# spiraldb/vortex

Hardware: AMD Instinct MI355X
Metric: decoded GB/s/GPU (device-resident) per encoding; % HBM roofline (higher is better)
Workload: dtype u32

## Files before the change

include/vortex_gpu.h:

```cpp
#ifndef VORTEX_GPU_H
#define VORTEX_GPU_H

#include <stddef.h>
#include <stdint.h>

#ifdef __cplusplus
extern "C" {
#endif

#define VXG_ABI_VERSION 9

typedef enum vxg_status {
    VXG_OK = 0,
    VXG_ERR_OUT_OF_BOUNDS = 1,
    VXG_ERR_COMPUTE = 2,
    VXG_ERR_INVALID_ARGUMENT = 3,
    VXG_ERR_INVALID_SERDE = 4,
    VXG_ERR_NOT_IMPLEMENTED = 5,
    VXG_ERR_MISMATCHED_TYPES = 6,
    VXG_ERR_ASSERTION_FAILED = 7,
    VXG_ERR_HIP = 8,
    VXG_ERR_OUT_OF_MEMORY = 9
} vxg_status;

enum {
    VXG_ENC_BOOL = 2, VXG_ENC_PRIMITIVE = 3, VXG_ENC_STRUCT = 4, VXG_ENC_VARBIN = 5,
    VXG_ENC_VARBINVIEW = 6, VXG_ENC_SPARSE = 8, VXG_ENC_CONSTANT = 9, VXG_ENC_CHUNKED = 10,
    VXG_ENC_ALP = 17, VXG_ENC_BYTE_BOOL = 18, VXG_ENC_DICT = 20, VXG_ENC_FL_BITPACKED = 21,
    VXG_ENC_FL_DELTA = 22, VXG_ENC_FL_FOR = 23, VXG_ENC_FSST = 24, VXG_ENC_ROARING_BOOL = 25, VXG_ENC_RUN_END = 27,
    VXG_ENC_RUN_END_BOOL = 28, VXG_ENC_ZIGZAG = 29, VXG_ENC_ALP_RD = 30
};

enum {
    VXG_U8 = 0, VXG_U16 = 1, VXG_U32 = 2, VXG_U64 = 3, VXG_I8 = 4, VXG_I16 = 5, VXG_I32 = 6,
    VXG_I64 = 7, VXG_F16 = 8, VXG_F32 = 9, VXG_F64 = 10
};

enum { VXG_DTYPE_NULL = 0, VXG_DTYPE_BOOL = 1, VXG_DTYPE_PRIMITIVE = 2, VXG_DTYPE_UTF8 = 3,
       VXG_DTYPE_BINARY = 4 };

enum { VXG_VALIDITY_NON_NULLABLE = 0, VXG_VALIDITY_ALL_VALID = 1, VXG_VALIDITY_ALL_INVALID = 2,
       VXG_VALIDITY_ARRAY = 3 };

typedef struct vxg_buffer {
    const void* ptr;
    uint64_t len;
} vxg_buffer;

typedef union vxg_meta {
    struct { uint8_t bit_width; uint8_t has_patches; uint16_t offset; } bitpacked;
    struct { uint64_t reference; uint8_t shift; } for_;
    struct { uint64_t deltas_len; uint16_t offset; } delta;
    struct { uint8_t e; uint8_t f; uint8_t has_patches; } alp;
    struct { uint8_t right_bit_width; uint8_t dict_len; uint8_t left_parts_ptype;
             uint8_t has_exceptions; uint16_t dict[8]; } alprd;
    struct { uint8_t codes_ptype; uint64_t values_len; } dict;
    struct { uint64_t symbols_len; uint8_t codes_nullable; uint8_t uncompressed_lengths_ptype; } fsst;
    struct { uint8_t ends_ptype; uint64_t num_runs; uint64_t offset; } runend;
    struct { uint64_t indices_offset; uint64_t indices_len; uint8_t fill_is_null; uint8_t fill[16]; } sparse;
    struct { uint8_t is_null; uint8_t scalar[16]; } constant;
    struct { uint64_t nchunks; } chunked;
    struct { uint8_t offsets_ptype; uint64_t bytes_len; } varbin;
    struct { uint8_t first_byte_bit_offset; } boolean;
    struct { uint8_t start; uint8_t ends_ptype; uint64_t num_runs; uint64_t offset; } runendbool;
    struct { uint32_t n_buffers; } varbinview;
    uint64_t raw[5];
} vxg_meta;

typedef struct vxg_array {
    uint16_t encoding;
    uint8_t dtype;
    uint8_t ptype;
    uint8_t nullable;
    uint8_t validity;
    uint16_t reserved;
    uint64_t len;
    vxg_meta meta;
    uint32_t n_buffers;
    uint32_t n_children;
    const vxg_buffer* buffers;
    const struct vxg_array* children;
} vxg_array;

typedef struct vxg_data_buffer {
    uint64_t offset;
    uint64_t len;
} vxg_data_buffer;

typedef struct vxg_canonical {
    uint16_t kind;
    uint8_t ptype;
    uint8_t dtype;
    uint32_t reserved;
    uint64_t len;
    void* values;
    uint64_t values_bytes;
    void* views;
    void* data;
    uint64_t data_bytes;
    void* validity;
    uint32_t n_data_buffers;
    uint32_t data_buffers_cap;
    vxg_data_buffer* data_buffers;
} vxg_canonical;

typedef struct vxg_ctx vxg_ctx;

int vxg_abi_version(void);
vxg_status vxg_open(int device, vxg_ctx** out);
vxg_status vxg_close(vxg_ctx* ctx);
const char* vxg_last_error(void);
vxg_status vxg_alloc(vxg_ctx* ctx, uint64_t bytes, void** dptr);
vxg_status vxg_free(vxg_ctx* ctx, void* dptr);
vxg_status vxg_host_alloc(vxg_ctx* ctx, uint64_t bytes, void** hptr);
vxg_status vxg_host_free(vxg_ctx* ctx, void* hptr);
vxg_status vxg_memcpy_h2d(vxg_ctx* ctx, void* dst, const void* src, uint64_t bytes, void* stream);
vxg_status vxg_memcpy_d2h(vxg_ctx* ctx, void* dst, const void* src, uint64_t bytes, void* stream);
vxg_status vxg_memcpy_d2d(vxg_ctx* ctx, void* dst, const void* src, uint64_t bytes, void* stream);
vxg_status vxg_stream_sync(vxg_ctx* ctx, void* stream);

typedef enum vxg_option {
    VXG_OPT_K1W_MIN_GROUPS = 1,
    VXG_OPT_K1W_BPW = 2,
    VXG_OPT_K1_WAVE = 3
} vxg_option;
vxg_status vxg_set_option(vxg_ctx* ctx, int option, int64_t value);
vxg_status vxg_get_option(vxg_ctx* ctx, int option, int64_t* value);

typedef struct vxg_launch_stats {
    uint64_t k1w_launches;
    uint64_t k1w_last_groups;
    uint32_t k1w_last_bpw;
    uint32_t k1w_last_bpw_max;
    uint32_t k1w_min_bpw;
    uint32_t k1w_max_bpw;
} vxg_launch_stats;
vxg_status vxg_get_launch_stats(vxg_ctx* ctx, vxg_launch_stats* out, int reset);

vxg_status vxg_canonical_size(vxg_ctx* ctx, const vxg_array* a, uint64_t* values_bytes,
                              uint64_t* data_bytes);
vxg_status vxg_canonicalize(vxg_ctx* ctx, const vxg_array* a, vxg_canonical* out, void* stream);

vxg_status vxg_canonical_layout(vxg_ctx* ctx, const vxg_array* a, uint64_t* values_bytes,
                                uint64_t* data_bytes, vxg_data_buffer* bufs, uint32_t cap,
                                uint32_t* n_bufs);

typedef struct vxg_plan vxg_plan;
enum { VXG_PLAN_MEASURE = 1 };
vxg_status vxg_plan_create(vxg_ctx* ctx, const vxg_array* arrays, vxg_canonical* outs, uint32_t n,
                           vxg_plan** plan);
vxg_status vxg_plan_create_ex(vxg_ctx* ctx, const vxg_array* arrays, vxg_canonical* outs, uint32_t n,
                              uint32_t flags, vxg_plan** plan);
vxg_status vxg_plan_launch(vxg_plan* plan, void* stream);
vxg_status vxg_plan_destroy(vxg_plan* plan);

typedef struct vxg_plan_info {
    uint32_t batched;
    uint32_t branches;
    uint32_t direct_nodes;
    uint32_t n_candidates;
    uint32_t candidate_batched[2];
    float candidate_ms[2];
    float create_ms;
    uint32_t selection;
    uint32_t candidate_cost[2];
    uint32_t reserved;
} vxg_plan_info;
vxg_status vxg_plan_get_info(const vxg_plan* plan, vxg_plan_info* info);

typedef enum vxg_plan_selection {
    VXG_PLAN_SEL_SINGLE = 0,
    VXG_PLAN_SEL_FASTER = 1,
    VXG_PLAN_SEL_TIE_COST = 2,
    VXG_PLAN_SEL_UNMEASURED = 3
} vxg_plan_selection;
uint32_t vxg_plan_select(const float* ms, const uint32_t* cost, uint32_t n, uint32_t* selection);


vxg_status vxg_bitunpack(vxg_ctx* ctx, int ptype, unsigned bit_width, unsigned offset,
                         uint64_t len, const void* packed, uint64_t packed_bytes, void* out,
                         void* stream);

vxg_status vxg_bitunpack_for(vxg_ctx* ctx, int ptype, unsigned bit_width, unsigned offset,
                             uint64_t len, const void* packed, uint64_t packed_bytes,
                             uint64_t reference, unsigned shift, int zigzag, void* out,
                             void* stream);

vxg_status vxg_bitunpack_alp(vxg_ctx* ctx, int float_ptype, unsigned bit_width, unsigned offset,
                             uint64_t len, const void* packed, uint64_t packed_bytes,
                             uint64_t for_reference, unsigned for_shift, unsigned e, unsigned f,
                             void* out, void* stream);

vxg_status vxg_bitunpack_dict(vxg_ctx* ctx, int codes_ptype, unsigned bit_width,
                              unsigned offset, uint64_t len, const void* packed,
                              uint64_t packed_bytes, const void* dict_values,
                              uint64_t dict_len, unsigned value_width, void* out, void* stream);

vxg_status vxg_patch(vxg_ctx* ctx, int ptype, void* out, uint64_t out_len, int indices_ptype,
                     const void* indices, uint64_t indices_offset, const void* values,
                     uint64_t n_patches, void* stream);

vxg_status vxg_for_decode(vxg_ctx* ctx, int ptype, const void* in, uint64_t n,
                          uint64_t reference, unsigned shift, void* out, void* stream);

vxg_status vxg_zigzag_decode(vxg_ctx* ctx, int out_ptype, const void* in, uint64_t n, void* out,
                             void* stream);

// ... 104 lines not shown
```

rust/vortex-gpu/src/ffi.rs:

```rust
#![allow(non_camel_case_types, non_upper_case_globals, dead_code)]

use std::os::raw::{c_char, c_int, c_uint, c_void};

pub const VXG_ABI_VERSION: c_int = 9;
pub type vxg_status = c_int;
pub const VXG_OK: vxg_status = 0;
pub const VXG_ERR_OUT_OF_BOUNDS: vxg_status = 1;
pub const VXG_ERR_COMPUTE: vxg_status = 2;
pub const VXG_ERR_INVALID_ARGUMENT: vxg_status = 3;
pub const VXG_ERR_INVALID_SERDE: vxg_status = 4;
pub const VXG_ERR_NOT_IMPLEMENTED: vxg_status = 5;
pub const VXG_ERR_MISMATCHED_TYPES: vxg_status = 6;
pub const VXG_ERR_ASSERTION_FAILED: vxg_status = 7;
pub const VXG_ERR_HIP: vxg_status = 8;
pub const VXG_ERR_OUT_OF_MEMORY: vxg_status = 9;
pub const VXG_ENC_BOOL: c_int = 2;
pub const VXG_ENC_PRIMITIVE: c_int = 3;
pub const VXG_ENC_STRUCT: c_int = 4;
pub const VXG_ENC_VARBIN: c_int = 5;
pub const VXG_ENC_VARBINVIEW: c_int = 6;
pub const VXG_ENC_SPARSE: c_int = 8;
pub const VXG_ENC_CONSTANT: c_int = 9;
pub const VXG_ENC_CHUNKED: c_int = 10;
pub const VXG_ENC_ALP: c_int = 17;
pub const VXG_ENC_BYTE_BOOL: c_int = 18;
pub const VXG_ENC_DICT: c_int = 20;
pub const VXG_ENC_FL_BITPACKED: c_int = 21;
pub const VXG_ENC_FL_DELTA: c_int = 22;
pub const VXG_ENC_FL_FOR: c_int = 23;
pub const VXG_ENC_FSST: c_int = 24;
pub const VXG_ENC_ROARING_BOOL: c_int = 25;
pub const VXG_ENC_RUN_END: c_int = 27;
pub const VXG_ENC_RUN_END_BOOL: c_int = 28;
pub const VXG_ENC_ZIGZAG: c_int = 29;
pub const VXG_ENC_ALP_RD: c_int = 30;
pub const VXG_U8: c_int = 0;
pub const VXG_U16: c_int = 1;
pub const VXG_U32: c_int = 2;
pub const VXG_U64: c_int = 3;
pub const VXG_I8: c_int = 4;
pub const VXG_I16: c_int = 5;
pub const VXG_I32: c_int = 6;
pub const VXG_I64: c_int = 7;
pub const VXG_F16: c_int = 8;
pub const VXG_F32: c_int = 9;
pub const VXG_F64: c_int = 10;
pub const VXG_DTYPE_NULL: c_int = 0;
pub const VXG_DTYPE_BOOL: c_int = 1;
pub const VXG_DTYPE_PRIMITIVE: c_int = 2;
pub const VXG_DTYPE_UTF8: c_int = 3;
pub const VXG_DTYPE_BINARY: c_int = 4;
pub const VXG_VALIDITY_NON_NULLABLE: c_int = 0;
pub const VXG_VALIDITY_ALL_VALID: c_int = 1;
pub const VXG_VALIDITY_ALL_INVALID: c_int = 2;
pub const VXG_VALIDITY_ARRAY: c_int = 3;

#[repr(C)]
#[derive(Copy, Clone, Debug)]
pub struct vxg_buffer {
    pub ptr: *const c_void,
    pub len: u64,
}

#[repr(C)]
#[derive(Copy, Clone, Debug)]
pub struct vxg_meta_bitpacked {
    pub bit_width: u8,
    pub has_patches: u8,
    pub offset: u16,
}

#[repr(C)]
#[derive(Copy, Clone, Debug)]
pub struct vxg_meta_for_ {
    pub reference: u64,
    pub shift: u8,
}

#[repr(C)]
#[derive(Copy, Clone, Debug)]
pub struct vxg_meta_delta {
    pub deltas_len: u64,
    pub offset: u16,
}

#[repr(C)]
#[derive(Copy, Clone, Debug)]
// ... 78 lines not shown
    pub ends_ptype: u8,
    pub num_runs: u64,
    pub offset: u64,
}

#[repr(C)]
#[derive(Copy, Clone, Debug)]
pub struct vxg_meta_varbinview {
    pub n_buffers: u32,
}

#[repr(C)]
#[derive(Copy, Clone)]
pub union vxg_meta {
    pub bitpacked: vxg_meta_bitpacked,
    pub for_: vxg_meta_for_,
    pub delta: vxg_meta_delta,
    pub alp: vxg_meta_alp,
    pub alprd: vxg_meta_alprd,
    pub dict: vxg_meta_dict,
    pub fsst: vxg_meta_fsst,
    pub runend: vxg_meta_runend,
    pub sparse: vxg_meta_sparse,
    pub constant: vxg_meta_constant,
    pub chunked: vxg_meta_chunked,
    pub varbin: vxg_meta_varbin,
    pub boolean: vxg_meta_boolean,
    pub runendbool: vxg_meta_runendbool,
    pub varbinview: vxg_meta_varbinview,
    pub raw: [u64; 5],
}

#[repr(C)]
#[derive(Copy, Clone, Debug)]
pub struct vxg_array {
    pub encoding: u16,
    pub dtype: u8,
    pub ptype: u8,
    pub nullable: u8,
    pub validity: u8,
    pub reserved: u16,
    pub len: u64,
    pub meta: vxg_meta,
    pub n_buffers: u32,
    pub n_children: u32,
    pub buffers: *const vxg_buffer,
    pub children: *const vxg_array,
}

#[repr(C)]
#[derive(Copy, Clone, Debug)]
pub struct vxg_data_buffer {
    pub offset: u64,
    pub len: u64,
}

#[repr(C)]
#[derive(Copy, Clone, Debug)]
pub struct vxg_canonical {
    pub kind: u16,
    pub ptype: u8,
    pub dtype: u8,
    pub reserved: u32,
    pub len: u64,
    pub values: *mut c_void,
    pub values_bytes: u64,
    pub views: *mut c_void,
    pub data: *mut c_void,
    pub data_bytes: u64,
    pub validity: *mut c_void,
    pub n_data_buffers: u32,
    pub data_buffers_cap: u32,
    pub data_buffers: *mut vxg_data_buffer,
}

#[repr(C)]
pub struct vxg_ctx {
    _private: [u8; 0],
}
pub type vxg_option = c_int;
pub const VXG_OPT_K1W_MIN_GROUPS: vxg_option = 1;
pub const VXG_OPT_K1W_BPW: vxg_option = 2;
pub const VXG_OPT_K1_WAVE: vxg_option = 3;

#[repr(C)]
#[derive(Copy, Clone, Debug)]
pub struct vxg_launch_stats {
    pub k1w_launches: u64,
    pub k1w_last_groups: u64,
    pub k1w_last_bpw: u32,
    pub k1w_last_bpw_max: u32,
    pub k1w_min_bpw: u32,
    pub k1w_max_bpw: u32,
}

#[repr(C)]
pub struct vxg_plan {
    _private: [u8; 0],
}
pub const VXG_PLAN_MEASURE: c_int = 1;

#[repr(C)]
#[derive(Copy, Clone, Debug)]
pub struct vxg_plan_info {
    pub batched: u32,
    pub branches: u32,
    pub direct_nodes: u32,
    pub n_candidates: u32,
    pub candidate_batched: [u32; 2],
    pub candidate_ms: [f32; 2],
    pub create_ms: f32,
    pub selection: u32,
    pub candidate_cost: [u32; 2],
    pub reserved: u32,
}
pub type vxg_plan_selection = c_int;
pub const VXG_PLAN_SEL_SINGLE: vxg_plan_selection = 0;
pub const VXG_PLAN_SEL_FASTER: vxg_plan_selection = 1;
pub const VXG_PLAN_SEL_TIE_COST: vxg_plan_selection = 2;
pub const VXG_PLAN_SEL_UNMEASURED: vxg_plan_selection = 3;
pub type vxg_cmp_op = c_int;
pub const VXG_CMP_EQ: vxg_cmp_op = 0;
pub const VXG_CMP_NOT_EQ: vxg_cmp_op = 1;
pub const VXG_CMP_GT: vxg_cmp_op = 2;
pub const VXG_CMP_GTE: vxg_cmp_op = 3;
pub const VXG_CMP_LT: vxg_cmp_op = 4;
pub const VXG_CMP_LTE: vxg_cmp_op = 5;
pub const VXG_CMP_NULL_AS_FALSE: c_int = 1;

#[repr(C)]
#[derive(Copy, Clone, Debug)]
pub struct vxg_compare_info {
    pub fused_launches: u32,
    pub fused_chunks: u32,
    pub fallback_arrays: u32,
    pub patch_launches: u32,
}

#[repr(C)]
#[derive(Copy, Clone, Debug)]
pub struct vxg_int_stats {
    pub n: u64,
    pub min_bits: u64,
    pub max_bits: u64,
    pub trailing_zeros: u32,
    pub reserved: u32,
    pub bit_width_freq: [u64; 65],
}

#[repr(C)]
#[derive(Copy, Clone, Debug)]
pub struct vxg_dict_chunk {
    pub packed: *const c_void,
    pub dict_values: *const c_void,
    pub out: *mut c_void,
    pub n_blocks: u64,
    pub len: u64,
    pub dict_len: u64,
}

#[repr(C)]
pub struct vxg_file {
    _private: [u8; 0],
}

#[repr(C)]
// ... 87 lines not shown
```

vortex_amd/_lib.py:

```python
from __future__ import annotations

import ctypes as C
import os
from pathlib import Path

_HERE = Path(__file__).resolve().parent
GPU_LIB_PATH = Path(os.environ["VXG_GPU_LIB"]) if os.environ.get("VXG_GPU_LIB") else _HERE / "libvortex_gpu.so"
ENC_LIB_PATH = _HERE / "libvortex_enc.so"

ENC = dict(BOOL=2, PRIMITIVE=3, STRUCT=4, VARBIN=5, VARBINVIEW=6, SPARSE=8, CONSTANT=9,
           CHUNKED=10, ALP=17, BYTE_BOOL=18, DICT=20, FL_BITPACKED=21, FL_DELTA=22, FL_FOR=23,
           FSST=24, ROARING_BOOL=25, RUN_END=27, RUN_END_BOOL=28, ZIGZAG=29, ALP_RD=30)
PTYPES = ["u8", "u16", "u32", "u64", "i8", "i16", "i32", "i64", "f16", "f32", "f64"]
PTYPE = {n: i for i, n in enumerate(PTYPES)}
DTYPE = dict(NULL=0, BOOL=1, PRIMITIVE=2, UTF8=3, BINARY=4)
VALIDITY = dict(NON_NULLABLE=0, ALL_VALID=1, ALL_INVALID=2, ARRAY=3)
ABI_VERSION = 9
STATUS = {0: "OK", 1: "OutOfBounds", 2: "ComputeError", 3: "InvalidArgument", 4: "InvalidSerde",
          5: "NotImplemented", 6: "MismatchedTypes", 7: "AssertionFailed", 8: "HipError",
          9: "OutOfMemory"}


class VortexGpuError(RuntimeError):

    def __init__(self, status: int, msg: str):
        super().__init__(f"{STATUS.get(status, status)}: {msg}")
        self.status = status
        self.kind = STATUS.get(status, str(status))


class VxgBuffer(C.Structure):
    _fields_ = [("ptr", C.c_void_p), ("len", C.c_uint64)]


class _MBitPacked(C.Structure):
    _fields_ = [("bit_width", C.c_uint8), ("has_patches", C.c_uint8), ("offset", C.c_uint16)]


class _MFoR(C.Structure):
    _fields_ = [("reference", C.c_uint64), ("shift", C.c_uint8)]


class _MDelta(C.Structure):
    _fields_ = [("deltas_len", C.c_uint64), ("offset", C.c_uint16)]


class _MAlp(C.Structure):
    _fields_ = [("e", C.c_uint8), ("f", C.c_uint8), ("has_patches", C.c_uint8)]


class _MAlpRd(C.Structure):
    _fields_ = [("right_bit_width", C.c_uint8), ("dict_len", C.c_uint8),
                ("left_parts_ptype", C.c_uint8), ("has_exceptions", C.c_uint8),
                ("dict", C.c_uint16 * 8)]


class _MDict(C.Structure):
    _fields_ = [("codes_ptype", C.c_uint8), ("values_len", C.c_uint64)]


class _MFsst(C.Structure):
    _fields_ = [("symbols_len", C.c_uint64), ("codes_nullable", C.c_uint8),
                ("uncompressed_lengths_ptype", C.c_uint8)]


class _MRunEnd(C.Structure):
    _fields_ = [("ends_ptype", C.c_uint8), ("num_runs", C.c_uint64), ("offset", C.c_uint64)]


class _MSparse(C.Structure):
    _fields_ = [("indices_offset", C.c_uint64), ("indices_len", C.c_uint64),
                ("fill_is_null", C.c_uint8), ("fill", C.c_uint8 * 16)]


class _MConstant(C.Structure):
    _fields_ = [("is_null", C.c_uint8), ("scalar", C.c_uint8 * 16)]


class _MChunked(C.Structure):
    _fields_ = [("nchunks", C.c_uint64)]


class _MVarBin(C.Structure):
    _fields_ = [("offsets_ptype", C.c_uint8), ("bytes_len", C.c_uint64)]


class _MBool(C.Structure):
    _fields_ = [("first_byte_bit_offset", C.c_uint8)]


class _MRunEndBool(C.Structure):
    _fields_ = [("start", C.c_uint8), ("ends_ptype", C.c_uint8), ("num_runs", C.c_uint64),
                ("offset", C.c_uint64)]


class _MVarBinView(C.Structure):
    _fields_ = [("n_buffers", C.c_uint32)]


class VxgMeta(C.Union):
    _fields_ = [("bitpacked", _MBitPacked), ("for_", _MFoR), ("delta", _MDelta), ("alp", _MAlp),
                ("alprd", _MAlpRd), ("dict", _MDict), ("fsst", _MFsst), ("runend", _MRunEnd),
                ("sparse", _MSparse), ("constant", _MConstant), ("chunked", _MChunked),
                ("varbin", _MVarBin), ("boolean", _MBool), ("runendbool", _MRunEndBool),
                ("varbinview", _MVarBinView), ("raw", C.c_uint64 * 5)]


class VxgArray(C.Structure):
    pass


VxgArray._fields_ = [("encoding", C.c_uint16), ("dtype", C.c_uint8), ("ptype", C.c_uint8),
                     ("nullable", C.c_uint8), ("validity", C.c_uint8), ("reserved", C.c_uint16),
                     ("len", C.c_uint64), ("meta", VxgMeta), ("n_buffers", C.c_uint32),
                     ("n_children", C.c_uint32), ("buffers", C.POINTER(VxgBuffer)),
                     ("children", C.POINTER(VxgArray))]


class VxgDataBuffer(C.Structure):
    _fields_ = [("offset", C.c_uint64), ("len", C.c_uint64)]


class VxgCanonical(C.Structure):
    _fields_ = [("kind", C.c_uint16), ("ptype", C.c_uint8), ("dtype", C.c_uint8),
                ("reserved", C.c_uint32), ("len", C.c_uint64), ("values", C.c_void_p),
                ("values_bytes", C.c_uint64), ("views", C.c_void_p), ("data", C.c_void_p),
                ("data_bytes", C.c_uint64), ("validity", C.c_void_p),
                ("n_data_buffers", C.c_uint32), ("data_buffers_cap", C.c_uint32),
                ("data_buffers", C.POINTER(VxgDataBuffer))]


PLAN_MEASURE = 1


class VxgPlanInfo(C.Structure):
    _fields_ = [("batched", C.c_uint32), ("branches", C.c_uint32), ("direct_nodes", C.c_uint32),
                ("n_candidates", C.c_uint32), ("candidate_batched", C.c_uint32 * 2),
                ("candidate_ms", C.c_float * 2), ("create_ms", C.c_float), ("selection", C.c_uint32),
                ("candidate_cost", C.c_uint32 * 2), ("reserved", C.c_uint32)]


PLAN_SELECTION = {0: "single", 1: "faster", 2: "tie_fewer_nodes", 3: "unmeasured"}


OPT_K1W_MIN_GROUPS, OPT_K1W_BPW, OPT_K1_WAVE = 1, 2, 3


class VxgLaunchStats(C.Structure):
    _fields_ = [("k1w_launches", C.c_uint64), ("k1w_last_groups", C.c_uint64), ("k1w_last_bpw", C.c_uint32),
                ("k1w_last_bpw_max", C.c_uint32), ("k1w_min_bpw", C.c_uint32), ("k1w_max_bpw", C.c_uint32)]


CMP_OP = {"==": 0, "!=": 1, ">": 2, ">=": 3, "<": 4, "<=": 5}
CMP_NULL_AS_FALSE = 1


class VxgCompareInfo(C.Structure):
    _fields_ = [("fused_launches", C.c_uint32), ("fused_chunks", C.c_uint32), ("fallback_arrays", C.c_uint32),
                ("patch_launches", C.c_uint32)]


class VxgIntStats(C.Structure):
    _fields_ = [("n", C.c_uint64), ("min_bits", C.c_uint64), ("max_bits", C.c_uint64), ("trailing_zeros", C.c_uint32),
                ("reserved", C.c_uint32), ("bit_width_freq", C.c_uint64 * 65)]


class VxgDictChunk(C.Structure):
    _fields_ = [("packed", C.c_void_p), ("dict_values", C.c_void_p), ("out", C.c_void_p),
                ("n_blocks", C.c_uint64), ("len", C.c_uint64), ("dict_len", C.c_uint64)]


assert C.sizeof(VxgMeta) == 40, C.sizeof(VxgMeta)
assert C.sizeof(VxgArray) == 80, C.sizeof(VxgArray)

VP, U64, U32, INT, UINT = C.c_void_p, C.c_uint64, C.c_uint32, C.c_int, C.c_uint
ST = C.c_int

GPU_SIGNATURES = {
    "vxg_abi_version": (C.c_int, []),
    "vxg_open": (ST, [INT, C.POINTER(VP)]),
    "vxg_close": (ST, [VP]),
    "vxg_last_error": (C.c_char_p, []),
    "vxg_alloc": (ST, [VP, U64, C.POINTER(VP)]),
    "vxg_free": (ST, [VP, VP]),
    "vxg_host_alloc": (ST, [VP, U64, C.POINTER(VP)]),
    "vxg_host_free": (ST, [VP, VP]),
    "vxg_memcpy_h2d": (ST, [VP, VP, VP, U64, VP]),
    "vxg_memcpy_d2h": (ST, [VP, VP, VP, U64, VP]),
    "vxg_memcpy_d2d": (ST, [VP, VP, VP, U64, VP]),
    "vxg_stream_sync": (ST, [VP, VP]),
    "vxg_set_option": (ST, [VP, INT, C.c_int64]),
    "vxg_get_option": (ST, [VP, INT, C.POINTER(C.c_int64)]),
    "vxg_get_launch_stats": (ST, [VP, C.POINTER(VxgLaunchStats), INT]),
    "vxg_canonical_size": (ST, [VP, C.POINTER(VxgArray), C.POINTER(U64), C.POINTER(U64)]),
    "vxg_canonicalize": (ST, [VP, C.POINTER(VxgArray), C.POINTER(VxgCanonical), VP]),
    "vxg_plan_create": (ST, [VP, C.POINTER(VxgArray), C.POINTER(VxgCanonical), U32, C.POINTER(VP)]),
    "vxg_plan_create_ex": (ST, [VP, C.POINTER(VxgArray), C.POINTER(VxgCanonical), U32, U32, C.POINTER(VP)]),
    "vxg_plan_get_info": (ST, [VP, C.c_void_p]),
    "vxg_plan_select": (U32, [C.POINTER(C.c_float), C.POINTER(U32), U32, C.POINTER(U32)]),
    "vxg_plan_launch": (ST, [VP, VP]),
    "vxg_plan_destroy": (ST, [VP]),
    "vxg_canonical_layout": (ST, [VP, C.POINTER(VxgArray), C.POINTER(U64), C.POINTER(U64),
                                  C.POINTER(VxgDataBuffer), U32, C.POINTER(U32)]),
    "vxg_bitunpack": (ST, [VP, INT, UINT, UINT, U64, VP, U64, VP, VP]),
    "vxg_bitunpack_for": (ST, [VP, INT, UINT, UINT, U64, VP, U64, U64, UINT, INT, VP, VP]),
    "vxg_bitunpack_alp": (ST, [VP, INT, UINT, UINT, U64, VP, U64, U64, UINT, UINT, UINT, VP, VP]),
    "vxg_bitunpack_dict": (ST, [VP, INT, UINT, UINT, U64, VP, U64, VP, U64, UINT, VP, VP]),
    "vxg_bitunpack_dict_chunks": (ST, [VP, INT, UINT, UINT, C.POINTER(VxgDictChunk), U32, VP]),
    "vxg_patch": (ST, [VP, INT, VP, U64, INT, VP, U64, VP, U64, VP]),
    "vxg_for_decode": (ST, [VP, INT, VP, U64, U64, UINT, VP, VP]),
    "vxg_zigzag_decode": (ST, [VP, INT, VP, U64, VP, VP]),
    "vxg_alp_decode": (ST, [VP, INT, VP, U64, UINT, UINT, VP, VP]),
    "vxg_alprd_decode": (ST, [VP, INT, VP, VP, UINT, UINT, VP, U64, VP, VP, U64, VP, VP]),
    "vxg_take": (ST, [VP, UINT, VP, U64, INT, VP, U64, VP, VP]),
    "vxg_delta_decode": (ST, [VP, INT, VP, U64, VP, U64, U64, U64, VP, VP]),
    "vxg_runend_decode": (ST, [VP, UINT, VP, INT, VP, U64, U64, U64, VP, VP]),
    "vxg_runend_bool_decode": (ST, [VP, INT, VP, U64, U64, INT, U64, VP, U64, VP]),
    "vxg_bytebool_to_bits": (ST, [VP, VP, U64, VP, U64, VP]),
    "vxg_take_array": (ST, [VP, VP, INT, VP, U64, VP, VP]),
    "vxg_filter_array": (ST, [VP, VP, VP, VP, VP]),
    "vxg_compare_scalar": (ST, [VP, VP, INT, VP, U32, VP, C.POINTER(VxgCompareInfo), VP]),
    "vxg_fsst_scratch_bytes": (U64, [U64]),
    "vxg_fsst_decode": (ST, [VP, VP, VP, UINT, VP, INT, VP, INT, VP, U64, VP, VP, VP, VP, VP]),
    "vxg_fill": (ST, [VP, UINT, VP, U64, VP, VP]),
    "vxg_compute_int_stats": (ST, [VP, INT, VP, U64, C.POINTER(VxgIntStats), VP]),
    "vxg_bitpack": (ST, [VP, INT, UINT, VP, U64, VP, U64, VP]),
    "vxg_for_encode": (ST, [VP, INT, VP, U64, U64, UINT, VP, VP]),
    "vxg_for_bitpack": (ST, [VP, INT, U64, UINT, UINT, VP, U64, VP, U64, VP]),
# ... 89 lines not shown
```

vortex_amd/arrays.py:

```python
from __future__ import annotations

import ctypes as C
from dataclasses import dataclass, field
from typing import Any, Optional, Sequence

import numpy as np

from . import _lib
from ._lib import DTYPE, ENC, PTYPE, PTYPES, VALIDITY, VortexGpuError

NP_OF_PTYPE = {"u8": np.uint8, "u16": np.uint16, "u32": np.uint32, "u64": np.uint64,
               "i8": np.int8, "i16": np.int16, "i32": np.int32, "i64": np.int64,
               "f16": np.float16, "f32": np.float32, "f64": np.float64}
PTYPE_OF_NP = {np.dtype(v): k for k, v in NP_OF_PTYPE.items()}


def ptype_width(p: str) -> int:
    return np.dtype(NP_OF_PTYPE[p]).itemsize


def unsigned_of(p: str) -> str:
    return "u" + p[1:] if p[0] == "i" else p


# ... 351 lines not shown
        m.sparse.indices_len = md["indices_len"]
        m.sparse.fill_is_null = int(md["fill_is_null"])
        for i, b in enumerate(md["fill"][:16]):
            m.sparse.fill[i] = b
    elif e == ENC["CONSTANT"]:
        m.constant.is_null = int(md["is_null"])
        for i, b in enumerate(md["scalar"][:16]):
            m.constant.scalar[i] = b
    elif e == ENC["CHUNKED"]:
        m.chunked.nchunks = md["nchunks"]
    elif e == ENC["VARBIN"]:
        m.varbin.offsets_ptype, m.varbin.bytes_len = md["offsets_ptype"], md["bytes_len"]
    elif e == ENC["BOOL"]:
        m.boolean.first_byte_bit_offset = md.get("first_byte_bit_offset", 0)
    elif e == ENC["RUN_END_BOOL"]:
        m.runendbool.start, m.runendbool.ends_ptype = int(md["start"]), md["ends_ptype"]
        m.runendbool.num_runs, m.runendbool.offset = md["num_runs"], md["offset"]
    elif e == ENC["VARBINVIEW"]:
        m.varbinview.n_buffers = md["n_buffers"]


def _buf_ptr(b) -> tuple[int, int]:
    import torch
    if not isinstance(b, torch.Tensor) or not b.is_cuda:
        raise VortexError(3, "array buffers must be device tensors: call Array.to(device) first")
    return b.data_ptr(), b.numel() * b.element_size()


def flatten(a: Array, keep: list) -> _lib.VxgArray:
    node = _lib.VxgArray()
    node.encoding = a.encoding
    node.dtype = a.dtype
    node.ptype = PTYPE[a.ptype]
    node.nullable = int(a.nullable)
    node.validity = a.validity
    node.len = a.len
    _fill_meta(node.meta, a)
    if a.buffers:
        bufs = (_lib.VxgBuffer * len(a.buffers))()
        for i, b in enumerate(a.buffers):
            bufs[i].ptr, bufs[i].len = _buf_ptr(b)
            keep.append(b)
        keep.append(bufs)
        node.buffers = C.cast(bufs, C.POINTER(_lib.VxgBuffer))
        node.n_buffers = len(a.buffers)
    if a.children:
        kids = (_lib.VxgArray * len(a.children))()
        for i, c in enumerate(a.children):
            kids[i] = flatten(c, keep)
        keep.append(kids)
        node.children = C.cast(kids, C.POINTER(_lib.VxgArray))
        node.n_children = len(a.children)
    return node


class Context:

    def __init__(self, device: int = 0):
        self.lib = _lib.gpu_lib()
        self.device = device
        h = C.c_void_p()
        _lib.check(self.lib.vxg_open(device, C.byref(h)))
        self.handle = h

    def close(self):
        if self.handle:
            self.lib.vxg_close(self.handle)
            self.handle = None

    def __del__(self):
        try:
            self.close()
        except Exception:
            pass

    def stream_ptr(self):
        import torch
        return C.c_void_p(torch.cuda.current_stream(self.device).cuda_stream)

    def sync(self):
        _lib.check(self.lib.vxg_stream_sync(self.handle, self.stream_ptr()))

    _OPTIONS = {"k1w_min_groups": _lib.OPT_K1W_MIN_GROUPS, "k1w_bpw": _lib.OPT_K1W_BPW,
                "k1_wave": _lib.OPT_K1_WAVE}

    def set_option(self, name: str, value: int):
        _lib.check(self.lib.vxg_set_option(self.handle, self._OPTIONS[name], int(value)))

    def get_option(self, name: str) -> int:
        v = C.c_int64()
        _lib.check(self.lib.vxg_get_option(self.handle, self._OPTIONS[name], C.byref(v)))
        return v.value

    def launch_stats(self, reset: bool = False) -> dict:
        st = _lib.VxgLaunchStats()
        _lib.check(self.lib.vxg_get_launch_stats(self.handle, C.byref(st), int(reset)))
        return {f: getattr(st, f) for f, _ in st._fields_}


@dataclass
class Canonical:
    kind: str
    len: int
    ptype: str
    values: Any = None
    views: Any = None
    data: Any = None
    validity: Any = None
    data_buffers: Any = None
    binary: bool = False
    info: Any = None

    def to_arrow(self):
        import pyarrow as pa
        validity = None if self.validity is None else pa.py_buffer(self.validity.cpu().numpy()[: (self.len + 7) // 8].copy())
        nulls = -1 if validity is not None else 0
        if self.kind == "primitive":
            t = {"u8": pa.uint8(), "u16": pa.uint16(), "u32": pa.uint32(), "u64": pa.uint64(), "i8": pa.int8(),
                 "i16": pa.int16(), "i32": pa.int32(), "i64": pa.int64(), "f16": pa.float16(), "f32": pa.float32(),
                 "f64": pa.float64()}[self.ptype]
            return pa.Array.from_buffers(t, self.len, [validity, pa.py_buffer(self.values.cpu().numpy().copy())],
                                         null_count=nulls)
        if self.kind == "bool":
            bits = self.values.cpu().numpy()[: (self.len + 7) // 8].copy()
            return pa.Array.from_buffers(pa.bool_(), self.len, [validity, pa.py_buffer(bits)], null_count=nulls)
        data = self.data.cpu().numpy()
        bufs = [pa.py_buffer(data[o: o + n].copy()) for o, n in self.data_buffers]
        views = pa.py_buffer(self.views.cpu().numpy()[: 16 * self.len].copy())
        return pa.Array.from_buffers(pa.binary_view() if self.binary else pa.string_view(), self.len,
                                     [validity, views] + bufs, null_count=nulls)

    def numpy(self):
        if self.kind == "primitive":
            return self.values.cpu().numpy().view(NP_OF_PTYPE[self.ptype])
        if self.kind == "bool":
            return np.unpackbits(self.values.cpu().numpy(), bitorder="little")[: self.len].astype(bool)
        return self.views.cpu().numpy().reshape(-1, 16), self.data.cpu().numpy()

    def buffers(self):
        d = self.data.cpu().numpy()
        return [d[o: o + n] for o, n in self.data_buffers]

    def validity_mask(self):
        if self.validity is None:
            return None
        bits = self.validity.cpu().numpy()
        return np.unpackbits(bits, bitorder="little")[: self.len].astype(bool)


def _kind(a: Array) -> str:
    return {DTYPE["PRIMITIVE"]: "primitive", DTYPE["BOOL"]: "bool"}.get(a.dtype, "varbinview")


def canonicalize(a: Array, ctx: Context, out_values=None, sync: bool = True) -> Canonical:
    import torch
    keep: list = []
    node = flatten(a, keep)
    dev = torch.device("cuda", ctx.device)
    vb, db, nb = C.c_uint64(), C.c_uint64(), C.c_uint32()
    cap = 256
    while True:
        table = (_lib.VxgDataBuffer * cap)()
        st = ctx.lib.vxg_canonical_layout(ctx.handle, C.byref(node), C.byref(vb), C.byref(db), table, cap,
                                          C.byref(nb))
        if st == 3 and cap < (1 << 24):
            cap *= 16
            continue
# ... 245 lines not shown
```

vortex_amd/csrc/capi.hip:

```cpp
#include <hip/hip_runtime.h>

#include <algorithm>
#include <memory>
#include <chrono>
#include <cstdio>
#include <cstdlib>
#include <cstring>
#include <mutex>
#include <string>
#include <tuple>
#include <vector>

#include "compare.hpp"
#include "encode_gpu.hpp"
#include "filter.hpp"
#include "k1g.hpp"
#include "take.hpp"
#include "vxg_internal.hpp"

struct vxg_ctx {
    vxg::Ctx c;
};

static_assert(sizeof(vxg::ChunkTable) <= 4096, "ChunkTable exceeds the kernarg limit");
static_assert(sizeof(vxg::FsstTable) <= 4096, "FsstTable exceeds the kernarg limit");
static_assert(sizeof(vxg::RunEndTable) <= 4096, "RunEndTable exceeds the kernarg limit");
static_assert(sizeof(vxg::VarBinTable) <= 4096, "VarBinTable exceeds the kernarg limit");
static_assert(sizeof(vxg::CmpTable) + 32 <= 4096, "CmpTable and the compare arguments exceed the kernarg limit");

namespace vxg {

const float kF10f[11] = {1.0f, 10.0f, 100.0f, 1000.0f, 10000.0f, 100000.0f, 1000000.0f,
                         10000000.0f, 100000000.0f, 1000000000.0f, 10000000000.0f};
const float kIF10f[11] = {1.0f, 0.1f, 0.01f, 0.001f, 0.0001f, 0.00001f, 0.000001f,
                          0.0000001f, 0.00000001f, 0.000000001f, 0.0000000001f};
const double kF10d[24] = {
    1.0, 10.0, 100.0, 1000.0, 10000.0, 100000.0, 1000000.0, 10000000.0, 100000000.0,
    1000000000.0, 10000000000.0, 100000000000.0, 1000000000000.0, 10000000000000.0,
    100000000000000.0, 1000000000000000.0, 10000000000000000.0, 100000000000000000.0,
    1000000000000000000.0, 10000000000000000000.0, 100000000000000000000.0,
    1000000000000000000000.0, 10000000000000000000000.0, 100000000000000000000000.0};
const double kIF10d[24] = {
    1.0, 0.1, 0.01, 0.001, 0.0001, 0.00001, 0.000001, 0.0000001, 0.00000001, 0.000000001,
    0.0000000001, 0.00000000001, 0.000000000001, 0.0000000000001, 0.00000000000001,
    0.000000000000001, 0.0000000000000001, 0.00000000000000001, 0.000000000000000001,
    0.0000000000000000001, 0.00000000000000000001, 0.000000000000000000001,
    0.0000000000000000000001, 0.00000000000000000000001};

static thread_local std::string g_last_error;

vxg_status set_error(vxg_status s, const std::string& msg) {
    if (s != VXG_OK) g_last_error = msg;
    return s;
}

vxg_status hip_check(hipError_t e, const char* what) {
    if (e == hipSuccess) return VXG_OK;
    return set_error(e == hipErrorOutOfMemory ? VXG_ERR_OUT_OF_MEMORY : VXG_ERR_HIP,
                     std::string(what) + ": " + hipGetErrorString(e));
}

static bool dict_rows_enabled() {
    static const bool on = [] {
        const char* e = std::getenv("VXG_DICT_ROWS");
        return !(e && e[0] == '0');
    }();
    return on;
}

static bool plan_vb_k1g() {
    const char* e = std::getenv("VXG_PLAN_VB_K1G");
    return !(e && e[0] == '0');
}

static bool fused_patches_enabled() {
    const char* e = std::getenv("VXG_FUSED_PATCHES");
    return !(e && e[0] == '0');
}

thread_local bool g_k1w_wrote_patches = false;
thread_local Ctx* g_cur_ctx = nullptr;

Options default_options() {
    static const Options d = [] {
        Options o;
        if (const char* e = std::getenv("VXG_K1W_MIN_GROUPS")) o.k1w_min_groups = int64_t(std::strtoll(e, nullptr, 10));
        return o;
    }();
    return d;
}

void note_k1w_launch(uint32_t bpw, uint32_t bpw_max, uint64_t groups) {
    if (!g_cur_ctx) return;
    std::lock_guard<std::mutex> lk(g_cur_ctx->mu);
    LaunchStats& st = g_cur_ctx->st;
    st.k1w_min_bpw = st.k1w_launches == 0 ? bpw : std::min(st.k1w_min_bpw, bpw);
    st.k1w_max_bpw = st.k1w_launches == 0 ? bpw : std::max(st.k1w_max_bpw, bpw);
    st.k1w_launches++;
    st.k1w_last_bpw = bpw;
    st.k1w_last_bpw_max = bpw_max;
    st.k1w_last_groups = groups;
}

bool k1_takes_wave(int T, int W, Epi epi, uint64_t groups32) {
    const int mode = k1_wave_mode();
    const bool split = (T == 32 || T == 64) && W > 0 && groups32 < split_below_groups();
    return groups32 > 0 && (mode == 2 || (mode == 1 && !split && epi != Epi::Dict));
}

vxg_status launch_fl_unpack(int T, int W, Epi epi, int vw, const ChunkTable& t, uint64_t g, hipStream_t s) {
    if (W < 0 || W > T) return set_error(VXG_ERR_INVALID_ARGUMENT, "bit width out of range");
    switch (epi) {
    case Epi::Plain:
    case Epi::For:
    case Epi::ForZigZag:
        switch (T) {
        case 8: return fl_plain_8(W, epi, t, g, s);
        case 16: return fl_plain_16(W, epi, t, g, s);
        case 32: return fl_plain_32(W, epi, t, g, s);
        case 64: return fl_plain_64(W, epi, t, g, s);
        }
        return set_error(VXG_ERR_INVALID_ARGUMENT, "bad FastLanes width");
    case Epi::AlpF32:
    case Epi::AlpF64:
        return fl_alp(T, W, epi, t, g, s);
    case Epi::Dict:
        if (W > kDictFusedMaxW) return VXG_ERR_NOT_IMPLEMENTED;
        if (vw == 16 && dict_rows_enabled()) return launch_dict_rows(T, W, vw, t, s);
        switch (vw) {
        case 1: return fl_dict_1(T, W, t, g, s);
        case 2: return fl_dict_2(T, W, t, g, s);
        case 4: return fl_dict_4(T, W, t, g, s);
        case 8: return fl_dict_8(T, W, t, g, s);
        case 16: return fl_dict_16(T, W, t, g, s);
        }
        return set_error(VXG_ERR_INVALID_ARGUMENT, "bad dictionary value width");
    }
    return VXG_ERR_INVALID_ARGUMENT;
}

}

using namespace vxg;

namespace {

#define VXG_TRY_S(expr)                       \
    do {                                      \
        vxg_status _s = (expr);               \
        if (_s != VXG_OK) return _s;          \
    } while (0)

struct K1Job {
    int T, W;
    Epi epi;
    int vw;
    ChunkDev d;
    bool vb = false;
    VarBinChunk vbc{};
};

bool same_kernel(const K1Job& a, const K1Job& b) {
    return a.T == b.T && a.W == b.W && a.epi == b.epi && a.vw == b.vw && a.vb == b.vb;
}

static uint64_t k1g_max_bytes() {
    static const uint64_t v = [] {
        const char* e = std::getenv("VXG_K1G_MAX_BYTES");
        return e ? uint64_t(std::strtoull(e, nullptr, 10)) : uint64_t(20) << 20;
    }();
    return v;
}

static int k1_out_width(const K1Job& j) {
    return j.epi == Epi::Dict ? j.vw : (j.epi == Epi::AlpF32 ? 4 : (j.epi == Epi::AlpF64 ? 8 : j.T / 8));
}

vxg_status launch_k1_jobs(std::vector<K1Job>& jobs, uint32_t* err, hipStream_t s, DevTables* dt = nullptr,
                          bool generic_small = false,
                          const std::vector<std::pair<int, RunEndChunk>>* gen_runs = nullptr,
                          const PatchCol* patch = nullptr, const FsstFused* fuse = nullptr) {
    std::stable_sort(jobs.begin(), jobs.end(), [](const K1Job& a, const K1Job& b) {
        return std::make_tuple(a.T, a.W, int(a.epi), a.vw, a.vb) < std::make_tuple(b.T, b.W, int(b.epi), b.vw, b.vb);
    });
    std::vector<const K1Job*> gen;
    const char* kf = std::getenv("VXG_PLAN_K1G_FIRST");
    const bool k1g_first = generic_small && dt && kf && kf[0] == '1';
    std::vector<std::pair<size_t, size_t>> deferred;
    auto launch_group = [&](size_t i, size_t j) -> vxg_status {
        size_t live = 0;
        for (size_t k = i; k < j; k++) live += jobs[k].d.n_blocks != 0;
        ChunkTable tab{};
        tab.err = err;
        if (patch && jobs.size() == 1) tab.patch = *patch;
        ChunkDev* cs = tab.c;
        if (live > size_t(kArgChunks)) {
            if (live > 0xFFFFFFFFull) return set_error(VXG_ERR_INVALID_ARGUMENT, "too many chunks");
            VXG_TRY_S(dt->table(live, &tab.host, &tab.ext));
            cs = tab.host;
        }
        uint64_t groups = 0;
        for (size_t k = i; k < j; k++) {
            if (jobs[k].d.n_blocks == 0) continue;
            ChunkDev& c = cs[tab.n++];
            c = jobs[k].d;
            c.first_group = groups;
            groups += (c.n_blocks + 31) / 32;
        }
        if (groups > 0xFFFFFFFFull) return set_error(VXG_ERR_INVALID_ARGUMENT, "array too long for one launch");
        if (tab.n) return launch_fl_unpack(jobs[i].T, jobs[i].W, jobs[i].epi, jobs[i].vw, tab, groups, s);
        return VXG_OK;
    };
    size_t i = 0;
    while (i < jobs.size()) {
        size_t j = i, live = 0;
        uint64_t out_bytes = 0;
        while (j < jobs.size() && (dt || j - i < size_t(kArgChunks)) && same_kernel(jobs[i], jobs[j])) {
            live += jobs[j].d.n_blocks != 0;
            out_bytes += jobs[j].d.len * uint64_t(k1_out_width(jobs[j]));
            j++;
        }
        if (jobs[i].vb || (dt && generic_small && out_bytes < k1g_max_bytes() &&
                           gen_kind(jobs[i].T, int(jobs[i].epi), jobs[i].vw) >= 0)) {
            if (!dt) return set_error(VXG_ERR_INVALID_ARGUMENT, "VarBin-dictionary K1 jobs need a plan");
            for (size_t k = i; k < j; k++)
                if (jobs[k].d.n_blocks) gen.push_back(&jobs[k]);
            i = j;
            continue;
        }
        (void)live;
        if (k1g_first) deferred.emplace_back(i, j);
        else VXG_TRY_S(launch_group(i, j));
        i = j;
    }
    const size_t n_runs = gen_runs ? gen_runs->size() : 0;
    if (!gen.empty() || n_runs || (fuse && fuse->valid)) {
        if (!dt) return set_error(VXG_ERR_INVALID_ARGUMENT, "internal: K1g launch outside a plan");
        if (gen.size() + n_runs > 0xFFFFFFFFull) return set_error(VXG_ERR_INVALID_ARGUMENT, "too many chunks");
        GenChunk* host;
        const GenChunk* ext;
        VXG_TRY_S(dt->table(gen.size() + n_runs, &host, &ext));
        uint64_t groups = 0;
        bool dict_lds = true;
        uint32_t packed_bytes = 0, dict_bytes = 0, runs_bytes = 0;
        const bool vb_alone = n_runs == 0 && !(fuse && fuse->valid) &&
                              std::all_of(gen.begin(), gen.end(), [](const K1Job* jp) { return jp->vb; });
        uint64_t gen_blocks = 0;
        for (const K1Job* jp : gen) gen_blocks += jp->d.n_blocks;
        const uint32_t bpw_cap = gen_bpw_cap(gen_blocks);
        for (size_t k = 0; k < gen.size(); k++) {
            const K1Job& jb = *gen[k];
            GenChunk& g = host[k];
            g.d = jb.d;
            g.kind = uint32_t(gen_kind(jb.T, int(jb.epi), jb.vw, jb.vb));
            g.W = uint32_t(jb.W);
            g.bpw = jb.vb ? gen_vb_bpw(jb.T, jb.W, vb_alone, bpw_cap) : gen_bpw(jb.T, jb.W, bpw_cap);
            g.d.first_group = groups;
            groups += (jb.d.n_blocks + g.bpw - 1) / g.bpw;
            packed_bytes = std::max(packed_bytes, g.bpw * 128u * uint32_t(jb.W));
            if (jb.vb) {
                dict_bytes = std::max(dict_bytes, gen_vb_stage_bytes(jb.d.dict_len, jb.vbc.bytes));
                g.vb_src = jb.vbc.src;
                g.vb_offs = jb.vbc.offsets;
                g.vb_offs_width = jb.vbc.offs_width;
                g.vb_dst = jb.vbc.dst;
                g.vb_bytes = jb.vbc.bytes;
                g.vb_bidx = jb.vbc.bidx;
            } else if (jb.epi == Epi::Dict) {
                dict_lds = dict_lds && jb.d.dict_len * uint64_t(jb.vw) <= uint64_t(kDictLdsBytes) &&
                           (reinterpret_cast<uintptr_t>(jb.d.dict) & 15) == 0;
            }
        }
        if (dict_lds)
            for (const K1Job* jp : gen)
                if (jp->epi == Epi::Dict && !jp->vb)
                    dict_bytes = std::max(dict_bytes, uint32_t((jp->d.dict_len * uint64_t(jp->vw) + 15) & ~15ull));
        for (size_t k = 0; k < n_runs; k++) {
            const auto& [w, r] = (*gen_runs)[k];
            GenChunk& g = host[gen.size() + k];
            g.kind = uint32_t(gen_runs_kind(w));
            g.re = r;
            g.d.first_group = groups;
            g.d.n_blocks = r.n_runs;
            groups += (r.n_runs + kRunEndRunsPerGroup - 1) / kRunEndRunsPerGroup;
            runs_bytes = std::max(runs_bytes, gen_runs_lds_bytes(w));
        }
        std::vector<uint64_t> cnt(gen.size() + n_runs);
        for (size_t k = 0; k < cnt.size(); k++)
            cnt[k] = (k + 1 < cnt.size() ? host[k + 1].d.first_group : groups) - host[k].d.first_group;
        uint64_t gpe = common_groups(cnt.data(), cnt.size());
        const char* pe = std::getenv("VXG_K1G_PAD");
        if (!gpe && cnt.size() > 1 && !(pe && pe[0] == '0')) {
            const uint64_t m = *std::max_element(cnt.begin(), cnt.end());
            if (m * cnt.size() - groups <= groups / 10) {
                for (size_t k = 0; k < cnt.size(); k++) host[k].d.first_group = k * m;
                groups = m * cnt.size();
                gpe = m;
            }
        }
        VXG_TRY_S(launch_k1_generic(ext, uint32_t(gen.size() + n_runs), groups, dict_lds, packed_bytes, dict_bytes,
                                    runs_bytes, err, s, gpe, fuse));
    }
    for (const auto& [a, b] : deferred) VXG_TRY_S(launch_group(a, b));
    return VXG_OK;
}

#define VXG_TRY(expr)                         \
    do {                                      \
        vxg_status _s = (expr);               \
        if (_s != VXG_OK) return _s;          \
    } while (0)

inline hipStream_t S(void* s) { return static_cast<hipStream_t>(s); }

vxg_status use_device(vxg_ctx* ctx) {
    if (!ctx) return set_error(VXG_ERR_INVALID_ARGUMENT, "null vxg_ctx");
    g_cur_ctx = &ctx->c;
    return hip_check(hipSetDevice(ctx->c.device), "hipSetDevice");
}

vxg_status make_k1_job(int T, unsigned W, unsigned offset, uint64_t len, const void* packed, uint64_t packed_bytes,
                       Epi epi, int vw, const UnpackArgs& a, void* out, K1Job& j) {
    if (offset > 1023) return set_error(VXG_ERR_INVALID_ARGUMENT, "Offset must be less than full block, i.e. 1024");
    if (W > unsigned(T)) return set_error(VXG_ERR_INVALID_ARGUMENT, "Unsupported bit width");
    const uint64_t nblk = (len + offset + 1023) / 1024;
    if (W > 0 && packed_bytes != nblk * 128ull * W)
        return set_error(VXG_ERR_INVALID_ARGUMENT, "Expected " + std::to_string(nblk * 128ull * W) +
                                                       " packed bytes, got " + std::to_string(packed_bytes));
    if (W > 0 && (reinterpret_cast<uintptr_t>(packed) & 15))
        return set_error(VXG_ERR_INVALID_ARGUMENT, "packed buffer must be 16-byte aligned");
    const int ow = epi == Epi::Dict ? vw : (epi == Epi::AlpF32 ? 4 : (epi == Epi::AlpF64 ? 8 : T / 8));
    if (reinterpret_cast<uintptr_t>(out) % uint64_t(ow))
        return set_error(VXG_ERR_INVALID_ARGUMENT, "output buffer must be aligned to the value width");
    if (epi == Epi::Dict && W > unsigned(kDictFusedMaxW)) return VXG_ERR_NOT_IMPLEMENTED;
    if (epi == Epi::Dict && a.dict_len == 0 && len > 0)
        return set_error(VXG_ERR_OUT_OF_BOUNDS, "take: index out of bounds");
    j.T = T;
    j.W = int(W);
    j.epi = epi;
    j.vw = epi == Epi::Dict ? vw : 0;
    j.d = ChunkDev{};
    j.d.packed = static_cast<const uint8_t*>(packed);
    j.d.out = out;
    j.d.n_blocks = len ? nblk : 0;
    j.d.len = len;
    j.d.reference = a.reference;
    j.d.alp_a = a.alp_a;
    j.d.alp_b = a.alp_b;
    j.d.dict = a.dict;
    j.d.dict_len = a.dict_len;
    j.d.offset = offset;
    j.d.shift = a.shift;
    return VXG_OK;
}

vxg_status bitunpack_common(vxg_ctx* ctx, int T, unsigned W, unsigned offset, uint64_t len,
                            const void* packed, uint64_t packed_bytes, Epi epi, int vw,
                            UnpackArgs a, void* out, void* stream) {
    std::vector<K1Job> jobs(1);
    VXG_TRY(make_k1_job(T, W, offset, len, packed, packed_bytes, epi, vw, a, out, jobs[0]));
    return launch_k1_jobs(jobs, ctx->c.err_word, S(stream));
}

vxg_status launch_runs(std::vector<RunEndChunk> runs, int w, uint32_t* err, hipStream_t s, DevTables* dt) {
    runs.erase(std::remove_if(runs.begin(), runs.end(), [](const RunEndChunk& r) { return r.len == 0; }), runs.end());
    std::vector<RunEndChunk> short_runs, long_runs;
    for (const RunEndChunk& r : runs) (r.len <= kRunEndShortRun * r.n_runs ? short_runs : long_runs).push_back(r);
    for (int pass = 0; pass < 2; pass++) {
        std::vector<RunEndChunk>& rs = pass == 0 ? short_runs : long_runs;
        const size_t per = dt && rs.size() > size_t(kRunEndArgChunks) ? rs.size() : size_t(kRunEndArgChunks);
        for (size_t i = 0; i < rs.size(); i += per) {
            RunEndTable tab{};
            tab.err = err;
            RunEndChunk* cs = tab.c;
            RunEndChunk* host = nullptr;
            if (per > size_t(kRunEndArgChunks)) {
                VXG_TRY_S(dt->table(rs.size(), &host, &tab.ext));
                cs = host;
            }
            uint64_t groups = 0;
            for (size_t k = i; k < rs.size() && k - i < per; k++) {
                RunEndChunk& r = cs[tab.n++];
                r = rs[k];
                r.first_group = groups;
                groups += pass == 0 ? (r.n_runs + kRunEndRunsPerGroup - 1) / kRunEndRunsPerGroup
                                    : (r.len + kRunEndSpan - 1) / kRunEndSpan;
            }
            VXG_TRY_S(pass == 0 ? launch_runend_runs(w, tab, groups, s) : launch_runend_chunks(w, tab, groups, s));
        }
    }
    return VXG_OK;
}

struct PlanBatch {
    struct Run {
        int w;
        RunEndChunk c;
        bool indep;
    };
    std::vector<VarBinChunk> dicts;
    std::vector<K1Job> jobs;
    std::vector<Run> runs;
    std::vector<FsstChunk> fssts;
    bool empty() const { return dicts.empty() && jobs.empty() && runs.empty() && fssts.empty(); }
};

static bool plan_fuse_enabled() {
    const char* e = std::getenv("VXG_PLAN_FUSE");
    return !(e && e[0] == '0');
}

vxg_status launch_varbin_dicts(const std::vector<VarBinChunk>& dicts, uint32_t* err, hipStream_t s, DevTables* dt) {
    const size_t per = dt && dicts.size() > size_t(kVarBinArgChunks) ? dicts.size() : size_t(kVarBinArgChunks);
    for (size_t i = 0; i < dicts.size(); i += per) {
        VarBinTable tab{};
        tab.err = err;
        VarBinChunk* cs = tab.c;
        if (per > size_t(kVarBinArgChunks)) {
            VarBinChunk* host;
            VXG_TRY_S(dt->table(dicts.size(), &host, &tab.ext));
            cs = host;
        }
        uint64_t groups = 0;
        for (size_t j = i; j < dicts.size() && j - i < per; j++) {
            VarBinChunk& d = cs[tab.n++];
            d = dicts[j];
            d.first_group = groups;
            groups += d.n ? (d.n + 255) / 256 : 1;
        }
        VXG_TRY_S(launch_varbin_chunks(tab, groups, s));
    }
    return VXG_OK;
}

vxg_status flush_plan_batch(PlanBatch& b, uint32_t* err, hipStream_t s, DevTables* dt) {
    FsstFused ff;
    if (!b.fssts.empty()) {
        void* scratch = nullptr;
        VXG_TRY_S(hip_check(hipMalloc(&scratch, (fsst_batch_scratch_bytes(b.fssts.data(), b.fssts.size()) + 15) & ~15ull),
                            "hipMalloc (plan FSST scratch)"));
        dt->allocs.push_back(scratch);
        VXG_TRY_S(launch_fsst_batch(b.fssts, scratch, err, s, dt, plan_fuse_enabled() ? &ff : nullptr));
    }
    VXG_TRY_S(launch_varbin_dicts(b.dicts, err, s, dt));
    std::vector<std::pair<int, RunEndChunk>> gen_runs;
    std::vector<PlanBatch::Run> rest;
    for (const PlanBatch::Run& r : b.runs) {
        if (r.c.len == 0) continue;
        if (r.indep && r.c.len <= kRunEndShortRun * r.c.n_runs && gen_runs_kind(r.w) >= 0) gen_runs.emplace_back(r.w, r.c);
        else rest.push_back(r);
    }
    VXG_TRY_S(launch_k1_jobs(b.jobs, err, s, dt, true, &gen_runs, nullptr, &ff));
    std::vector<int> widths;
    for (const auto& r : rest) widths.push_back(r.w);
    std::sort(widths.begin(), widths.end());
    widths.erase(std::unique(widths.begin(), widths.end()), widths.end());
    for (int w : widths) {
        std::vector<RunEndChunk> rs;
        for (const auto& r : rest)
            if (r.w == w) rs.push_back(r.c);
        VXG_TRY_S(launch_runs(rs, w, err, s, dt));
    }
    return VXG_OK;
}

class Planner {
  public:
    Planner(vxg_ctx* ctx, hipStream_t s, DevTables* plan = nullptr, PlanBatch* batch = nullptr)
        : ctx_(ctx), s_(s), plan_(plan), batch_(batch) {}
    ~Planner() {
        for (void* p : temps_) (void)hipFreeAsync(p, s_);
    }

    vxg_status canonical(const vxg_array& a, vxg_canonical& out);
    vxg_status take(const vxg_array& a, const void* idx, int iw, bool isg, uint64_t n, vxg_canonical& out);
    vxg_status filter(const vxg_array& a, const vxg_array& pred, vxg_canonical& out);
    vxg_status compare(const vxg_array& a, int op, uint64_t scalar_bits, uint32_t flags, vxg_canonical& out,
                       vxg_compare_info& info);
    vxg_status canonical_size(const vxg_array& a, uint64_t& vb, uint64_t& db);
    vxg_status string_layout(const vxg_array& a, std::vector<vxg_data_buffer>& bufs, uint64_t& extent);
    static vxg_status string_buffer_count(const vxg_array& a, uint32_t& n);

  private:
    vxg_ctx* ctx_;
    hipStream_t s_;
    std::vector<void*> temps_;
    DevTables* plan_ = nullptr;
    PlanBatch* batch_ = nullptr;
    const vxg_array* root_ = nullptr;
    bool defer(const vxg_array& a) const { return batch_ && &a == root_; }
    struct PatchJob {
        const vxg_array* sp;
        int T;
        Epi epi;
        int vw;
        UnpackArgs a;
        void* dst;
        uint64_t out_len;
    };
    std::vector<K1Job>* k1_batch_ = nullptr;
    std::vector<PatchJob>* patch_batch_ = nullptr;
    const PatchCol* fused_patch_ = nullptr;
    std::vector<FsstChunk>* fsst_batch_ = nullptr;
    bool k1_fusable(const vxg_array& c) const;

    vxg_status temp(uint64_t bytes, void** p) {
        if (bytes == 0) bytes = 16;
        if (plan_) {
            VXG_TRY(hip_check(hipMalloc(p, (bytes + 15) & ~15ull), "hipMalloc (plan temporary)"));
            plan_->allocs.push_back(*p);
            return VXG_OK;
        }
        VXG_TRY(hip_check(hipMallocAsync(p, (bytes + 15) & ~15ull, s_), "hipMallocAsync"));
        temps_.push_back(*p);
        return VXG_OK;
    }

    static bool is_primitive_dtype(const vxg_array& a) { return a.dtype == VXG_DTYPE_PRIMITIVE; }
    static int width(const vxg_array& a) { return ptype_width(a.ptype); }

    const vxg_buffer* buf(const vxg_array& a, uint32_t i) const {
        return i < a.n_buffers ? &a.buffers[i] : nullptr;
    }
    const vxg_array* child(const vxg_array& a, uint32_t i) const {
        return i < a.n_children ? &a.children[i] : nullptr;
    }

    vxg_status decode_into(const vxg_array& a, void* dst);
    vxg_status view_primitive(const vxg_array& a, const void** p);
    vxg_status int_column(const vxg_array& a, IntCol& c);
    vxg_status packed_column(const vxg_array& a, IntCol& c, bool* packed);
    vxg_status runend_column(const vxg_array& a, bool in_place, IntCol& c);

    vxg_status decode_bitpacked(const vxg_array& bp, Epi epi, int vw, UnpackArgs a, void* dst);
    bool patch_fusable(const vxg_array& sparse, int value_width) const;
    vxg_status sparse_patch_col(const vxg_array& sparse, PatchCol& pc);
    vxg_status apply_sparse_patches(const vxg_array& sparse, int T, Epi epi, int vw, const UnpackArgs& a,
                                    void* dst, uint64_t out_len);
    vxg_status decode_alp(const vxg_array& a, void* dst);
    vxg_status decode_dict_primitive(const vxg_array& a, void* dst);
    vxg_status decode_chunked_primitive(const vxg_array& a, void* dst);
    vxg_status decode_alprd(const vxg_array& a, void* dst);
    vxg_status decode_sparse_values(const vxg_array& a, void* dst);

    vxg_status take_values(const vxg_array& a, const void* idx, int iw, bool isg, uint64_t n, void* dst);
    vxg_status take_patches(const vxg_array& sp, TakePatches& p);
    struct CmpFused {
        const vxg_array* arr;
        const vxg_array* bp;
        const vxg_array* outer;
        int T, ck;
        Epi epi;
        EpiParams ep;
        CmpChunk d;
        bool excl;
    };
    vxg_status compare_shape(const vxg_array& a, uint64_t out_bit, CmpFused& f, bool* fused);
    vxg_status launch_compare_group(std::vector<CmpFused*>& group, void* out, uint64_t scalar_bits, int op);
    vxg_status validity_into(const vxg_array& a, void** bitmap);
    vxg_status bools_into(const vxg_array& a, void* bits, uint64_t off);
    vxg_status validity_source(const vxg_array& a, const vxg_array** node, int* kind);
    vxg_status string_canonical(const vxg_array& a, vxg_canonical& out);
    vxg_status string_lens(const vxg_array& a, std::vector<uint64_t>& lens,
                           std::vector<std::pair<size_t, const vxg_array*>>& fsst) const;
    vxg_status strings_into(const vxg_array& a, uint8_t* views, uint8_t* data, const vxg_data_buffer* bufs,
                            uint32_t bidx, const uint8_t* validity);
};

vxg_status Planner::view_primitive(const vxg_array& a, const void** p) {
    if (a.encoding == VXG_ENC_PRIMITIVE) {
// ... 31 lines not shown
vxg_status Planner::packed_column(const vxg_array& a, IntCol& c, bool* packed) {
    *packed = false;
    c = IntCol{};
    c.width = width(a);
    c.sgn = ptype_is_signed(a.ptype);
    const vxg_array* bp = nullptr;
    if (a.encoding == VXG_ENC_FL_FOR && child(a, 0) && child(a, 0)->encoding == VXG_ENC_FL_BITPACKED) {
        bp = child(a, 0);
        c.reference = a.meta.for_.reference;
        c.shift = a.meta.for_.shift;
    } else if (a.encoding == VXG_ENC_FL_BITPACKED) {
        bp = &a;
    }
    if (bp && !bp->meta.bitpacked.has_patches && width(*bp) == c.width && (c.width == 4 || c.width == 8) &&
        bp->len == a.len) {
        const vxg_buffer* pk = buf(*bp, 0);
        const unsigned W = bp->meta.bitpacked.bit_width, off = bp->meta.bitpacked.offset;
        const uint64_t nblk = (bp->len + off + 1023) / 1024;
        if (off > 1023) return set_error(VXG_ERR_INVALID_ARGUMENT, "Offset must be less than full block, i.e. 1024");
        if (W > unsigned(8 * c.width)) return set_error(VXG_ERR_INVALID_ARGUMENT, "Unsupported bit width");
        const uint64_t have = pk ? pk->len : 0;
        if (W > 0 && have != nblk * 128ull * W)
            return set_error(VXG_ERR_INVALID_ARGUMENT, "Expected " + std::to_string(nblk * 128ull * W) +
                                                           " packed bytes, got " + std::to_string(have));
        c.packed = true;
        c.p = pk ? pk->ptr : nullptr;
        c.W = W;
        c.offset = off;
        *packed = true;
    }
    return VXG_OK;
}

vxg_status Planner::apply_sparse_patches(const vxg_array& sp, int T, Epi epi, int vw, const UnpackArgs& a,
                                         void* dst, uint64_t out_len) {
    if (sp.encoding != VXG_ENC_SPARSE)
        return set_error(VXG_ERR_INVALID_ARGUMENT, "Can't patch with a non-Sparse array");
    const vxg_array* idx = child(sp, 0);
    const vxg_array* val = child(sp, 1);
    if (!idx || !val) return set_error(VXG_ERR_INVALID_ARGUMENT, "Sparse patches need indices and values");
    if (idx->len != val->len) return set_error(VXG_ERR_INVALID_ARGUMENT, "Sparse indices/values length mismatch");
    PatchCol pc;
    VXG_TRY(int_column(*idx, pc.idx));
    VXG_TRY(view_primitive(*val, &pc.vals));
    return launch_patch(vw, pc.idx, epi, T, dst, out_len, sp.meta.sparse.indices_offset, pc.vals, idx->len, a, s_);
}

bool Planner::patch_fusable(const vxg_array& sp, int value_width) const {
    const vxg_array* idx = child(sp, 0);
    const vxg_array* val = child(sp, 1);
    return sp.encoding == VXG_ENC_SPARSE && idx && val && idx->len == val->len && idx->len > 0 &&
           width(*val) == value_width && width(*idx) == 8 && ptype_is_int(idx->ptype);
}

vxg_status Planner::sparse_patch_col(const vxg_array& sp, PatchCol& pc) {
    const vxg_array* idx = child(sp, 0);
    VXG_TRY(int_column(*idx, pc.idx));
    VXG_TRY(view_primitive(*child(sp, 1), &pc.vals));
    pc.n = idx->len;
    pc.idx_off = sp.meta.sparse.indices_offset;
    return VXG_OK;
}

vxg_status Planner::decode_bitpacked(const vxg_array& bp, Epi epi, int vw, UnpackArgs a, void* dst) {
    const int T = 8 * width(bp);
    if (!ptype_is_int(bp.ptype)) return set_error(VXG_ERR_MISMATCHED_TYPES, "BitPacked needs an integer ptype");
    const vxg_buffer* packed = buf(bp, 0);
    const unsigned W = bp.meta.bitpacked.bit_width;
    a.err = ctx_->c.err_word;
    K1Job j;
    VXG_TRY(make_k1_job(T, W, bp.meta.bitpacked.offset, bp.len, packed ? packed->ptr : nullptr,
                        packed ? packed->len : 0, epi, vw, a, dst, j));
    const vxg_array* p = nullptr;
    if (bp.meta.bitpacked.has_patches) {
        p = child(bp, 0);
        if (!p) return set_error(VXG_ERR_INVALID_ARGUMENT, "BitPackedArray: patches child missing");
    }
    if (k1_batch_) {
        k1_batch_->push_back(j);
        if (p) patch_batch_->push_back(PatchJob{p, T, epi, vw, a, dst, bp.len});
        return VXG_OK;
    }
    std::vector<K1Job> one{j};
    VXG_TRY(launch_k1_jobs(one, ctx_->c.err_word, s_, plan_, false, nullptr, fused_patch_));
    if (p) VXG_TRY(apply_sparse_patches(*p, T, epi, vw, a, dst, bp.len));
    return VXG_OK;
}

vxg_status Planner::decode_alp(const vxg_array& a, void* dst) {
    const vxg_array* enc = child(a, 0);
    if (!enc) return set_error(VXG_ERR_INVALID_ARGUMENT, "ALPArray: encoded child missing");
    const bool f32 = a.ptype == VXG_F32;
    if (!f32 && a.ptype != VXG_F64) return set_error(VXG_ERR_MISMATCHED_TYPES, "ALP can only encode f32 and f64");
    const unsigned e = a.meta.alp.e, f = a.meta.alp.f;
    if ((f32 && (e > 10 || f > 10)) || (!f32 && (e > 23 || f > 23)))
        return set_error(VXG_ERR_INVALID_ARGUMENT, "ALP exponents out of range");
    UnpackArgs ua{};
    ua.alp_a = f32 ? double(kF10f[f]) : kF10d[f];
    ua.alp_b = f32 ? double(kIF10f[e]) : kIF10d[e];
    const Epi epi = f32 ? Epi::AlpF32 : Epi::AlpF64;
    const vxg_array* bp = nullptr;
    if (enc->encoding == VXG_ENC_FL_FOR && child(*enc, 0) &&
        child(*enc, 0)->encoding == VXG_ENC_FL_BITPACKED) {
        ua.reference = enc->meta.for_.reference;
        ua.shift = enc->meta.for_.shift;
        bp = child(*enc, 0);
    } else if (enc->encoding == VXG_ENC_FL_BITPACKED) {
        bp = enc;
    }
    bool fused = false;
    if (bp && width(*bp) == (f32 ? 4 : 8)) {
        PatchCol pc{};
        const vxg_array* p = a.meta.alp.has_patches ? child(a, 1) : nullptr;
        if (p && !k1_batch_ && !patch_batch_ && !bp->meta.bitpacked.has_patches && bp->len == a.len &&
            patch_fusable(*p, f32 ? 4 : 8) && fused_patches_enabled()) {
            const uint64_t nblk = (bp->len + bp->meta.bitpacked.offset + 1023) / 1024;
            if (k1_takes_wave(f32 ? 32 : 64, int(bp->meta.bitpacked.bit_width), epi, (nblk + 31) / 32)) {
                VXG_TRY(sparse_patch_col(*p, pc));
                fused = !pc.idx.packed || pc.idx.W > 0;
            }
        }
        fused_patch_ = fused ? &pc : nullptr;
        g_k1w_wrote_patches = false;
        const vxg_status st = decode_bitpacked(*bp, epi, 0, ua, dst);
        fused_patch_ = nullptr;
        VXG_TRY(st);
        fused = fused && g_k1w_wrote_patches;
    } else {
        const void* penc;
        VXG_TRY(view_primitive(*enc, &penc));
        VXG_TRY(launch_alp(a.ptype, penc, a.len, ua.alp_a, ua.alp_b, dst, s_));
    }
    if (a.meta.alp.has_patches && !fused) {
        const vxg_array* p = child(a, 1);
        if (!p) return set_error(VXG_ERR_INVALID_ARGUMENT, "ALPArray: patches child missing");
        UnpackArgs plain{};
        plain.err = ctx_->c.err_word;
        if (patch_batch_) {
            patch_batch_->push_back(PatchJob{p, f32 ? 32 : 64, Epi::Plain, 0, plain, dst, a.len});
            return VXG_OK;
        }
        VXG_TRY(apply_sparse_patches(*p, f32 ? 32 : 64, Epi::Plain, 0, plain, dst, a.len));
    }
    return VXG_OK;
}

vxg_status Planner::decode_dict_primitive(const vxg_array& a, void* dst) {
    const vxg_array* values = child(a, 0);
    const vxg_array* codes = child(a, 1);
    if (!values || !codes) return set_error(VXG_ERR_INVALID_ARGUMENT, "DictArray needs values and codes");
    if (!ptype_is_unsigned(codes->ptype) || codes->nullable)
        return set_error(VXG_ERR_MISMATCHED_TYPES, "Dict codes must be non-nullable unsigned int");
    const void* pv;
    VXG_TRY(view_primitive(*values, &pv));
    const int vw = width(*values);
    if (codes->encoding == VXG_ENC_FL_BITPACKED && codes->meta.bitpacked.bit_width <= kDictFusedMaxW) {
        UnpackArgs ua{};
        ua.dict = pv;
        ua.dict_len = values->len;
        return decode_bitpacked(*codes, Epi::Dict, vw, ua, dst);
    }
    const void* pc;
    VXG_TRY(view_primitive(*codes, &pc));
    return launch_take(vw, pv, values->len, width(*codes), false, pc, a.len, dst, ctx_->c.err_word, s_);
}

bool Planner::k1_fusable(const vxg_array& c) const {
// ... 42 lines not shown
    std::vector<uint8_t> is_inplace(2 * n, 0);
    uint64_t tmp_bytes = 0;
    for (uint64_t i = 0; i < n; i++) {
        const vxg_array& c = a.children[i + 1];
        if (!batch_runend(c)) continue;
        const vxg_array* e = child(c, 0);
        const vxg_array* v = child(c, 1);
        const bool short_runs = c.len <= kRunEndShortRun * e->len;
        const vxg_array* xs[2] = {e, v};
        for (int k = 0; k < 2; k++) {
            bool pk = false;
            if (short_runs && ptype_is_int(xs[k]->ptype)) VXG_TRY(packed_column(*xs[k], inplace[2 * i + k], &pk));
            is_inplace[2 * i + k] = pk;
            if (!pk && xs[k]->encoding != VXG_ENC_PRIMITIVE) tmp_bytes += (xs[k]->len * width(*xs[k]) + 15) & ~15ull;
        }
    }
    uint8_t* tmp = nullptr;
    if (tmp_bytes) {
        void* t;
        VXG_TRY(temp(tmp_bytes, &t));
        tmp = static_cast<uint8_t*>(t);
    }
    auto level0 = [&](const vxg_array& x, const void** p) -> vxg_status {
        if (x.encoding == VXG_ENC_PRIMITIVE) return view_primitive(x, p);
        *p = tmp;
        tmp += (x.len * width(x) + 15) & ~15ull;
        k1_batch_ = &jobs;
        patch_batch_ = &patches;
        const vxg_status st = decode_into(x, const_cast<void*>(*p));
        k1_batch_ = nullptr;
        patch_batch_ = nullptr;
        return st;
    };
    uint64_t off = 0;
    for (uint64_t i = 0; i < n; i++) {
        const vxg_array& c = a.children[i + 1];
        if (c.ptype != a.ptype || c.dtype != a.dtype)
            return set_error(VXG_ERR_MISMATCHED_TYPES, "Chunks must have the ChunkedArray's dtype");
        uint8_t* slice = static_cast<uint8_t*>(dst) + off * w;
        if (k1_fusable(c)) {
            k1_batch_ = &jobs;
            patch_batch_ = &patches;
            const vxg_status st = decode_into(c, slice);
            k1_batch_ = nullptr;
            patch_batch_ = nullptr;
            VXG_TRY(st);
        } else if (batch_runend(c)) {
            const vxg_array& e = *child(c, 0);
            const vxg_array& v = *child(c, 1);
            RunEndChunk r{};
            IntCol* cols[2] = {&r.ends, &r.values};
            const vxg_array* xs[2] = {&e, &v};
            for (int k = 0; k < 2; k++) {
                if (is_inplace[2 * i + k]) {
                    *cols[k] = inplace[2 * i + k];
                } else {
                    cols[k]->width = width(*xs[k]);
                    cols[k]->sgn = ptype_is_signed(xs[k]->ptype);
                    VXG_TRY(level0(*xs[k], &cols[k]->p));
                }
            }
            r.out = slice;
            r.n_runs = e.len;
            r.offset = c.meta.runend.offset;
            r.len = c.len;
            runs.push_back(r);
            runs_indep.push_back(uint8_t((is_inplace[2 * i] || e.encoding == VXG_ENC_PRIMITIVE) &&
                                         (is_inplace[2 * i + 1] || v.encoding == VXG_ENC_PRIMITIVE)));
        } else if ((reinterpret_cast<uintptr_t>(slice) & 15) == 0) {
            VXG_TRY(decode_into(c, slice));
        } else {
            const void* p;
            VXG_TRY(view_primitive(c, &p));
            VXG_TRY(launch_copy_bytes(slice, p, c.len * w, s_));
        }
        off += c.len;
    }
    if (off != a.len) return set_error(VXG_ERR_INVALID_ARGUMENT, "Chunked len != sum of chunk lens");
    if (defer(a) && patches.empty()) {
        batch_->jobs.insert(batch_->jobs.end(), jobs.begin(), jobs.end());
        for (size_t k = 0; k < runs.size(); k++) batch_->runs.push_back(PlanBatch::Run{w, runs[k], runs_indep[k] != 0});
        return VXG_OK;
    }
    VXG_TRY(launch_k1_jobs(jobs, ctx_->c.err_word, s_, plan_));
    for (const PatchJob& p : patches) VXG_TRY(apply_sparse_patches(*p.sp, p.T, p.epi, p.vw, p.a, p.dst, p.out_len));
    return launch_runs(runs, w, ctx_->c.err_word, s_, plan_);
}

vxg_status Planner::decode_alprd(const vxg_array& a, void* dst) {
    const vxg_array* left = child(a, 0);
    const vxg_array* right = child(a, 1);
    if (!left || !right) return set_error(VXG_ERR_INVALID_ARGUMENT, "ALPRDArray needs left/right parts");
    if (left->ptype != VXG_U16) return set_error(VXG_ERR_MISMATCHED_TYPES, "ALP-RD left parts must be u16");
    const void *pl, *pr;
    VXG_TRY(view_primitive(*left, &pl));
    VXG_TRY(view_primitive(*right, &pr));
    const void* pos = nullptr;
    const void* exc = nullptr;
    uint64_t n_exc = 0, pos_off = 0;
    int pw = 8;
    bool psg = false;
    if (a.meta.alprd.has_exceptions) {
        const vxg_array* sp = child(a, 2);
        if (!sp || sp->encoding != VXG_ENC_SPARSE)
            return set_error(VXG_ERR_INVALID_ARGUMENT, "left_parts_exceptions must be SparseArray encoded");
        const vxg_array* si = child(*sp, 0);
        const vxg_array* sv = child(*sp, 1);
        VXG_TRY(view_primitive(*si, &pos));
        VXG_TRY(view_primitive(*sv, &exc));
        n_exc = si->len;
        pos_off = sp->meta.sparse.indices_offset;
        pw = width(*si);
        psg = ptype_is_signed(si->ptype);
    }
    return launch_alprd(a.ptype, static_cast<const uint16_t*>(pl), a.meta.alprd.dict, a.meta.alprd.dict_len,
                        a.meta.alprd.right_bit_width, pr, a.len, pos, pw, psg, pos_off,
                        static_cast<const uint16_t*>(exc), n_exc, dst, ctx_->c.err_word, s_);
}

vxg_status Planner::decode_sparse_values(const vxg_array& a, void* dst) {
    uint8_t fill[16] = {0};
    if (!a.meta.sparse.fill_is_null) std::memcpy(fill, a.meta.sparse.fill, 16);
    VXG_TRY(launch_fill(width(a), fill, a.len, dst, s_));
    UnpackArgs plain{};
    plain.err = ctx_->c.err_word;
    return apply_sparse_patches(a, 8 * width(a), Epi::Plain, 0, plain, dst, a.len);
}

vxg_status Planner::decode_into(const vxg_array& a, void* dst) {
    if (!is_primitive_dtype(a)) return set_error(VXG_ERR_MISMATCHED_TYPES, "expected a primitive dtype");
    const int w = width(a);
    if (w == 0) return set_error(VXG_ERR_NOT_IMPLEMENTED, "unsupported ptype");
    switch (a.encoding) {
    case VXG_ENC_PRIMITIVE: {
        const void* p;
        VXG_TRY(view_primitive(a, &p));
        if (p != dst && a.len)
            VXG_TRY(launch_copy_bytes(dst, p, a.len * w, s_));
        return VXG_OK;
    }
    case VXG_ENC_FL_BITPACKED:
        return decode_bitpacked(a, Epi::Plain, 0, UnpackArgs{}, dst);
    case VXG_ENC_FL_FOR: {
        const vxg_array* enc = child(a, 0);
        if (!enc) return set_error(VXG_ERR_INVALID_ARGUMENT, "FoRArray is missing encoded child array");
        if (!ptype_is_int(a.ptype)) return set_error(VXG_ERR_MISMATCHED_TYPES, "FoR needs an integer ptype");
        if (enc->encoding == VXG_ENC_FL_BITPACKED && width(*enc) == w) {
            UnpackArgs ua{};
            ua.reference = a.meta.for_.reference;
            ua.shift = a.meta.for_.shift;
            return decode_bitpacked(*enc, Epi::For, 0, ua, dst);
        }
        VXG_TRY(decode_into(*enc, dst));
        return launch_for(w, dst, a.len, a.meta.for_.reference, a.meta.for_.shift, false, dst, s_);
    }
    case VXG_ENC_ZIGZAG: {
        const vxg_array* enc = child(a, 0);
        if (!enc) return set_error(VXG_ERR_INVALID_ARGUMENT, "ZigZagArray is missing encoded child");
        if (!ptype_is_signed(a.ptype)) return set_error(VXG_ERR_MISMATCHED_TYPES, "ZigZag decodes to signed ints");
        if (enc->encoding == VXG_ENC_FL_BITPACKED && width(*enc) == w)
            return decode_bitpacked(*enc, Epi::ForZigZag, 0, UnpackArgs{}, dst);
        VXG_TRY(decode_into(*enc, dst));
        return launch_zigzag(w, dst, a.len, dst, s_);
    }
    case VXG_ENC_ALP:
        return decode_alp(a, dst);
    case VXG_ENC_ALP_RD:
        return decode_alprd(a, dst);
    case VXG_ENC_DICT:
// ... 753 lines not shown
    if (!fsst.empty()) {
        void* d;
        VXG_TRY(temp(8 * fsst.size(), &d));
        for (size_t k = 0; k < fsst.size(); k++) {
            const vxg_array& ul = *child(*fsst[k].second, 3);
            const void* pul;
            VXG_TRY(view_primitive(ul, &pul));
            VXG_TRY(launch_sum(pul, width(ul), ptype_is_signed(ul.ptype), ul.len, static_cast<uint64_t*>(d) + k, s_));
        }
        std::vector<uint64_t> h(fsst.size());
        VXG_TRY(hip_check(hipMemcpyAsync(h.data(), d, 8 * h.size(), hipMemcpyDeviceToHost, s_), "sum readback"));
        VXG_TRY(hip_check(hipStreamSynchronize(s_), "sum sync"));
        for (size_t k = 0; k < fsst.size(); k++) lens[fsst[k].first] = h[k];
    }
    bufs.resize(lens.size());
    uint64_t off = 0;
    for (size_t b = 0; b < lens.size(); b++) {
        bufs[b] = vxg_data_buffer{off, lens[b]};
        off = (off + lens[b] + 15) & ~15ull;
    }
    extent = lens.empty() ? 0 : bufs.back().offset + bufs.back().len;
    return VXG_OK;
}

vxg_status Planner::strings_into(const vxg_array& a, uint8_t* views, uint8_t* data, const vxg_data_buffer* bufs,
                                 uint32_t bidx, const uint8_t* validity) {
    switch (a.encoding) {
    case VXG_ENC_VARBIN: {
        const vxg_array* offs = child(a, 0);
        const vxg_array* bytes = child(a, 1);
        const void *po, *pb;
        VXG_TRY(view_primitive(*offs, &po));
        VXG_TRY(view_primitive(*bytes, &pb));
        uint8_t* heap = data + bufs[0].offset;
        if (bufs[0].len)
            VXG_TRY(launch_copy_bytes(heap, pb, bufs[0].len, s_));
        return launch_varbin_views(heap, bufs[0].len, width(*offs), po, a.len, validity, bidx, views, ctx_->c.err_word, s_);
    }
    case VXG_ENC_VARBINVIEW: {
        const vxg_array* vw = child(a, 0);
        const void* pv;
        VXG_TRY(view_primitive(*vw, &pv));
        if (vw->len < 16 * a.len) return set_error(VXG_ERR_INVALID_ARGUMENT, "VarBinView views shorter than 16 * len");
        VXG_TRY(launch_views_rebase(static_cast<const uint8_t*>(pv), a.len, bidx, views, s_));
        for (uint32_t b = 0; b < a.meta.varbinview.n_buffers; b++) {
            const void* pb;
            VXG_TRY(view_primitive(a.children[1 + b], &pb));
            if (bufs[b].len)
                VXG_TRY(launch_copy_bytes(data + bufs[b].offset, pb, bufs[b].len, s_));
        }
        return VXG_OK;
    }
    case VXG_ENC_FSST: {
        const vxg_array* sym = child(a, 0);
        const vxg_array* slen = child(a, 1);
        const vxg_array* codes = child(a, 2);
        const vxg_array* ulen = child(a, 3);
        if (!sym || !slen || !codes || !ulen || codes->encoding != VXG_ENC_VARBIN)
            return set_error(VXG_ERR_INVALID_ARGUMENT, "FSSTArray needs symbols, lengths, VarBin codes, lengths");
        const void *psym, *pslen, *pcb;
        VXG_TRY(view_primitive(*sym, &psym));
        VXG_TRY(view_primitive(*slen, &pslen));
        VXG_TRY(view_primitive(*child(*codes, 1), &pcb));
        FsstChunk f{};
        f.symbols = static_cast<const uint64_t*>(psym);
        f.sym_lens = static_cast<const uint8_t*>(pslen);
        f.n_symbols = unsigned(sym->len);
        f.codes = static_cast<const uint8_t*>(pcb);
        VXG_TRY(int_column(*child(*codes, 0), f.offs));
        VXG_TRY(int_column(*ulen, f.lens));
        f.n = a.len;
        f.validity = validity;
        f.heap = data + bufs[0].offset;
        f.heap_len = bufs[0].len;
        f.views = views;
        f.bidx = bidx;
        if (fsst_batch_) {
            fsst_batch_->push_back(f);
            return VXG_OK;
        }
        std::vector<FsstChunk> one{f};
        void* scratch;
        VXG_TRY(temp(fsst_batch_scratch_bytes(one.data(), 1), &scratch));
        return launch_fsst_batch(one, scratch, ctx_->c.err_word, s_, plan_);
    }
    case VXG_ENC_DICT: {
        const vxg_array* values = child(a, 0);
        const vxg_array* codes = child(a, 1);
        if (!values || !codes) return set_error(VXG_ERR_INVALID_ARGUMENT, "DictArray needs values and codes");
        const vxg_array* vn;
        int vk;
        VXG_TRY(validity_source(*values, &vn, &vk));
        void* vbits = nullptr;
        if (vk != 0) {
            VXG_TRY(temp(((values->len + 31) / 32) * 4, &vbits));
            VXG_TRY(validity_into(*values, &vbits));
        }
        void* vviews;
        VXG_TRY(temp(16 * values->len, &vviews));
        VXG_TRY(strings_into(*values, static_cast<uint8_t*>(vviews), data, bufs, bidx,
                             static_cast<const uint8_t*>(vbits)));
        if (codes->encoding == VXG_ENC_FL_BITPACKED && codes->meta.bitpacked.bit_width <= kDictFusedMaxW) {
            UnpackArgs ua{};
            ua.dict = vviews;
            ua.dict_len = values->len;
            return decode_bitpacked(*codes, Epi::Dict, 16, ua, views);
        }
        const void* pc;
        VXG_TRY(view_primitive(*codes, &pc));
        return launch_take(16, vviews, values->len, width(*codes), false, pc, a.len, views, ctx_->c.err_word, s_);
    }
    case VXG_ENC_CHUNKED: {
        const uint64_t n = a.meta.chunked.nchunks;
        if (a.n_children != n + 1) return set_error(VXG_ERR_INVALID_ARGUMENT, "Chunked child count != nchunks + 1");
        auto dict_batchable = [&](const vxg_array& c) {
            if (c.encoding != VXG_ENC_DICT || c.n_children < 2) return false;
            const vxg_array& v = c.children[0];
            const vxg_array& k = c.children[1];
            return v.encoding == VXG_ENC_VARBIN && v.validity != VXG_VALIDITY_ARRAY &&
                   v.validity != VXG_VALIDITY_ALL_INVALID && v.n_children >= 2 &&
                   v.children[0].encoding == VXG_ENC_PRIMITIVE && v.children[1].encoding == VXG_ENC_PRIMITIVE &&
                   k.encoding == VXG_ENC_FL_BITPACKED && ptype_is_unsigned(k.ptype) && !k.nullable &&
                   k.meta.bitpacked.bit_width <= kDictFusedMaxW;
        };
        uint64_t dict_rows = 0;
        for (uint64_t i = 0; i < n; i++)
            if (dict_batchable(a.children[i + 1])) dict_rows += a.children[i + 1].children[0].len;
        uint8_t* dviews = nullptr;
        if (dict_rows) {
            void* t;
            VXG_TRY(temp(16 * dict_rows, &t));
            dviews = static_cast<uint8_t*>(t);
        }
        std::vector<VarBinChunk> dicts;
        std::vector<K1Job> jobs;
        std::vector<PatchJob> patches;
        std::vector<FsstChunk> fssts;
        uint64_t row = 0;
        uint32_t b = 0;
        for (uint64_t i = 0; i < n; i++) {
            const vxg_array& c = a.children[i + 1];
            if (c.dtype != a.dtype) return set_error(VXG_ERR_MISMATCHED_TYPES, "Chunks must have the ChunkedArray's dtype");
            uint32_t k;
            VXG_TRY(string_buffer_count(c, k));
            if (dict_batchable(c)) {
                const vxg_array& v = c.children[0];
                const void *po, *pb;
                VXG_TRY(view_primitive(v.children[0], &po));
                VXG_TRY(view_primitive(v.children[1], &pb));
                VarBinChunk d{};
                d.src = static_cast<const uint8_t*>(pb);
                d.dst = data + bufs[b].offset;
                d.offsets = po;
                d.views = dviews;
                d.bytes = bufs[b].len;
                d.n = v.len;
                d.offs_width = uint32_t(width(v.children[0]));
                d.bidx = bidx + b;
                const vxg_array& codes = c.children[1];
                const bool vb = (defer(a) || (plan_ && plan_vb_k1g())) && v.len <= kGenVarBinDictMax && v.len > 0 &&
                                codes.len > 0 && !codes.meta.bitpacked.has_patches;
                if (!vb) dicts.push_back(d);
                UnpackArgs ua{};
                ua.dict = vb ? nullptr : dviews;
                ua.dict_len = v.len;
                dviews += 16 * v.len;
                k1_batch_ = &jobs;
                patch_batch_ = &patches;
                const size_t nj = jobs.size(), np = patches.size();
                const vxg_status st = decode_bitpacked(c.children[1], Epi::Dict, 16, ua, views + 16 * row);
                k1_batch_ = nullptr;
                patch_batch_ = nullptr;
                VXG_TRY(st);
                if (vb) {
                    if (jobs.size() != nj + 1 || patches.size() != np)
                        return set_error(VXG_ERR_INVALID_ARGUMENT, "internal: VarBin-dictionary job shape");
                    jobs.back().vb = true;
                    jobs.back().vbc = d;
                }
            } else {
                void* cv = nullptr;
                const vxg_array* vn;
                int vk;
                VXG_TRY(validity_source(c, &vn, &vk));
                if (vk != 0) {
                    VXG_TRY(temp(((c.len + 31) / 32) * 4, &cv));
                    VXG_TRY(validity_into(c, &cv));
                }
                if (c.encoding == VXG_ENC_FSST) fsst_batch_ = &fssts;
                const vxg_status st =
                    strings_into(c, views + 16 * row, data, bufs + b, bidx + b, static_cast<const uint8_t*>(cv));
                fsst_batch_ = nullptr;
                VXG_TRY(st);
            }
            row += c.len;
            b += k;
        }
        if (row != a.len) return set_error(VXG_ERR_INVALID_ARGUMENT, "Chunked len != sum of chunk lens");
        if (!fssts.empty() && defer(a)) {
            batch_->fssts.insert(batch_->fssts.end(), fssts.begin(), fssts.end());
        } else if (!fssts.empty()) {
            void* scratch;
            VXG_TRY(temp(fsst_batch_scratch_bytes(fssts.data(), fssts.size()), &scratch));
            VXG_TRY(launch_fsst_batch(fssts, scratch, ctx_->c.err_word, s_, plan_));
        }
        if (defer(a) && patches.empty()) {
            batch_->dicts.insert(batch_->dicts.end(), dicts.begin(), dicts.end());
            batch_->jobs.insert(batch_->jobs.end(), jobs.begin(), jobs.end());
            return VXG_OK;
        }
        VXG_TRY(launch_varbin_dicts(dicts, ctx_->c.err_word, s_, plan_));
        VXG_TRY(launch_k1_jobs(jobs, ctx_->c.err_word, s_, plan_));
        for (const PatchJob& p : patches) VXG_TRY(apply_sparse_patches(*p.sp, p.T, p.epi, p.vw, p.a, p.dst, p.out_len));
        return VXG_OK;
    }
    default:
        return set_error(VXG_ERR_NOT_IMPLEMENTED, "string canonicalize for encoding id " + std::to_string(a.encoding));
    }
}

vxg_status Planner::string_canonical(const vxg_array& a, vxg_canonical& out) {
    out.kind = VXG_ENC_VARBINVIEW;
    out.len = a.len;
    out.dtype = a.dtype;
    uint32_t nb;
    VXG_TRY(string_buffer_count(a, nb));
    std::vector<vxg_data_buffer> bufs;
    if (out.views && out.data) {
        if (nb == 1) {
            bufs.push_back(vxg_data_buffer{0, out.data_bytes});
        } else {
            if (!out.data_buffers || out.n_data_buffers != nb)
                return set_error(VXG_ERR_INVALID_ARGUMENT, "caller-provided data needs the vxg_canonical_layout buffer table (" +
                                                               std::to_string(nb) + " buffers)");
            bufs.assign(out.data_buffers, out.data_buffers + nb);
        }
    } else {
        uint64_t extent;
        VXG_TRY(string_layout(a, bufs, extent));
        if (nb > 1 && (!out.data_buffers || out.data_buffers_cap < nb))
            return set_error(VXG_ERR_INVALID_ARGUMENT, "data_buffers must have room for " + std::to_string(nb) + " buffers");
        if (!out.views) VXG_TRY(hip_check(hipMalloc(&out.views, a.len ? 16 * a.len : 16), "views alloc"));
        if (!out.data) VXG_TRY(hip_check(hipMalloc(&out.data, extent + 16), "data alloc"));
        out.data_bytes = extent;
    }
    out.n_data_buffers = nb;
    if (out.data_buffers && out.data_buffers_cap >= nb && out.data_buffers != bufs.data())
        std::copy(bufs.begin(), bufs.end(), out.data_buffers);
    VXG_TRY(validity_into(a, &out.validity));
    return strings_into(a, static_cast<uint8_t*>(out.views), static_cast<uint8_t*>(out.data), bufs.data(), 0,
                        static_cast<const uint8_t*>(out.validity));
}

vxg_status Planner::canonical_size(const vxg_array& a, uint64_t& vb, uint64_t& db) {
    vb = db = 0;
    if (a.dtype == VXG_DTYPE_PRIMITIVE) {
        vb = a.len * width(a);
        return VXG_OK;
    }
    if (a.dtype == VXG_DTYPE_BOOL) {
        vb = ((a.len + 31) / 32) * 4;
        return VXG_OK;
    }
    if (a.dtype != VXG_DTYPE_UTF8 && a.dtype != VXG_DTYPE_BINARY)
        return set_error(VXG_ERR_NOT_IMPLEMENTED, "canonical size for this dtype");
    vb = a.len * 16;
    std::vector<vxg_data_buffer> bufs;
    return string_layout(a, bufs, db);
}

vxg_status Planner::canonical(const vxg_array& a, vxg_canonical& out) {
    root_ = &a;
    out.len = a.len;
    out.dtype = a.dtype;
    out.ptype = a.ptype;
    if (a.dtype == VXG_DTYPE_UTF8 || a.dtype == VXG_DTYPE_BINARY) return string_canonical(a, out);
    if (a.dtype == VXG_DTYPE_BOOL) {
        out.kind = VXG_ENC_BOOL;
        out.values_bytes = ((a.len + 31) / 32) * 4;
        if (!out.values)
            VXG_TRY(hip_check(hipMalloc(&out.values, out.values_bytes ? out.values_bytes : 4), "bool values alloc"));
        if (out.values_bytes)
            VXG_TRY(launch_copy_bytes(out.values, nullptr, out.values_bytes, s_));
        VXG_TRY(bools_into(a, out.values, 0));
        return validity_into(a, &out.validity);
    }
    if (a.dtype != VXG_DTYPE_PRIMITIVE)
        return set_error(VXG_ERR_NOT_IMPLEMENTED, "canonicalize supports primitive, bool and utf8/binary dtypes");
    out.kind = VXG_ENC_PRIMITIVE;
    out.values_bytes = a.len * width(a);
    if (!out.values)
        VXG_TRY(hip_check(hipMalloc(&out.values, out.values_bytes ? out.values_bytes : 16), "values alloc"));
    VXG_TRY(decode_into(a, out.values));
    return validity_into(a, &out.validity);
}

}

static vxg_status status_of_err_word(uint32_t err) {
    if (err & kErrTakeOOB) return set_error(VXG_ERR_OUT_OF_BOUNDS, "take: index out of bounds");
    if (err & kErrPatchOOB) return set_error(VXG_ERR_OUT_OF_BOUNDS, "patch index out of bounds");
    if (err & kErrPatchOrder) return set_error(VXG_ERR_INVALID_ARGUMENT, "patch indices are not sorted");
    if (err & kErrRunEnd) return set_error(VXG_ERR_INVALID_ARGUMENT, "RunEnd ends do not cover the array");
    if (err & kErrFsst) return set_error(VXG_ERR_INVALID_ARGUMENT, "FSST codes do not decode to uncompressed_lengths");
    if (err & kErrRoaring) return set_error(VXG_ERR_INVALID_SERDE, "RoaringBool buffer is not a croaring Native bitmap");
    if (err & kErrVarBin) return set_error(VXG_ERR_INVALID_ARGUMENT, "VarBin offsets out of range of the bytes");
    if (err & kErrPlanSync)
        return set_error(VXG_ERR_ASSERTION_FAILED, "plan launch: in-grid pre-pass records never published "
                                                   "(overlapping replays of one plan?)");
    return set_error(VXG_ERR_ASSERTION_FAILED, "unknown device error bit");
}

extern "C" {

int vxg_abi_version(void) { return VXG_ABI_VERSION; }

const char* vxg_last_error(void) { return g_last_error.c_str(); }

vxg_status vxg_open(int device, vxg_ctx** out) {
    if (!out) return set_error(VXG_ERR_INVALID_ARGUMENT, "null out");
    int n = 0;
    VXG_TRY(hip_check(hipGetDeviceCount(&n), "hipGetDeviceCount"));
    if (device < 0 || device >= n) return set_error(VXG_ERR_INVALID_ARGUMENT, "no such device");
    VXG_TRY(hip_check(hipSetDevice(device), "hipSetDevice"));
    auto* c = new vxg_ctx();
    c->c.device = device;
    c->c.opt = default_options();
    hipError_t e = hipMalloc(&c->c.err_word, 16);
    if (e == hipSuccess) e = hipMemset(c->c.err_word, 0, 16);
    if (e == hipSuccess) {
        hipMemPool_t pool;
        uint64_t keep = ~0ull;
        if (hipDeviceGetDefaultMemPool(&pool, device) == hipSuccess)
            (void)hipMemPoolSetAttribute(pool, hipMemPoolAttrReleaseThreshold, &keep);
    }
    if (e == hipSuccess) e = fsst_diag_init();
    if (e != hipSuccess) {
        vxg_close(c);
        return hip_check(e, "context setup");
    }
    *out = c;
    return VXG_OK;
}

vxg_status vxg_set_option(vxg_ctx* ctx, int option, int64_t value) {
    if (!ctx) return set_error(VXG_ERR_INVALID_ARGUMENT, "null vxg_ctx");
    Options& o = ctx->c.opt;
    switch (option) {
    case VXG_OPT_K1W_MIN_GROUPS:
        if (value < 0 || value > (int64_t(1) << 31)) return set_error(VXG_ERR_INVALID_ARGUMENT, "K1W_MIN_GROUPS out of range");
        o.k1w_min_groups = value;
        return VXG_OK;
    case VXG_OPT_K1W_BPW:
        if (value < 0 || value > 32) return set_error(VXG_ERR_INVALID_ARGUMENT, "K1W_BPW must be in [0, 32]");
        o.k1w_bpw = value;
        return VXG_OK;
    case VXG_OPT_K1_WAVE:
        if (value < -1 || value > 2) return set_error(VXG_ERR_INVALID_ARGUMENT, "K1_WAVE must be -1, 0, 1 or 2");
        o.k1_wave = value;
        return VXG_OK;
    }
    return set_error(VXG_ERR_INVALID_ARGUMENT, "unknown option " + std::to_string(option));
}

vxg_status vxg_get_option(vxg_ctx* ctx, int option, int64_t* value) {
    if (!ctx || !value) return set_error(VXG_ERR_INVALID_ARGUMENT, "null argument");
    const Options& o = ctx->c.opt;
    switch (option) {
    case VXG_OPT_K1W_MIN_GROUPS: *value = o.k1w_min_groups; return VXG_OK;
    case VXG_OPT_K1W_BPW: *value = o.k1w_bpw; return VXG_OK;
    case VXG_OPT_K1_WAVE: *value = o.k1_wave; return VXG_OK;
    }
    return set_error(VXG_ERR_INVALID_ARGUMENT, "unknown option " + std::to_string(option));
}

vxg_status vxg_get_launch_stats(vxg_ctx* ctx, vxg_launch_stats* out, int reset) {
    if (!ctx || !out) return set_error(VXG_ERR_INVALID_ARGUMENT, "null argument");
    std::lock_guard<std::mutex> lk(ctx->c.mu);
    const LaunchStats& st = ctx->c.st;
    *out = vxg_launch_stats{};
    out->k1w_launches = st.k1w_launches;
    out->k1w_last_groups = st.k1w_last_groups;
    out->k1w_last_bpw = st.k1w_last_bpw;
    out->k1w_min_bpw = st.k1w_min_bpw;
    out->k1w_max_bpw = st.k1w_max_bpw;
    out->k1w_last_bpw_max = st.k1w_last_bpw_max;
    if (reset) ctx->c.st = LaunchStats{};
    return VXG_OK;
}

vxg_status vxg_close(vxg_ctx* ctx) {
    if (!ctx) return VXG_OK;
    if (g_cur_ctx == &ctx->c) g_cur_ctx = nullptr;
    (void)hipSetDevice(ctx->c.device);
    (void)hipDeviceSynchronize();
    if (ctx->c.err_word) (void)hipFree(ctx->c.err_word);
    delete ctx;
    return VXG_OK;
}

vxg_status vxg_alloc(vxg_ctx* ctx, uint64_t bytes, void** dptr) {
    VXG_TRY(use_device(ctx));
    return hip_check(hipMalloc(dptr, bytes ? bytes : 16), "hipMalloc");
}

vxg_status vxg_free(vxg_ctx* ctx, void* dptr) {
    VXG_TRY(use_device(ctx));
    return hip_check(hipFree(dptr), "hipFree");
}

vxg_status vxg_host_alloc(vxg_ctx* ctx, uint64_t bytes, void** hptr) {
    VXG_TRY(use_device(ctx));
    return hip_check(hipHostMalloc(hptr, bytes ? bytes : 16, hipHostMallocDefault), "hipHostMalloc");
}

vxg_status vxg_host_free(vxg_ctx* ctx, void* hptr) {
    VXG_TRY(use_device(ctx));
    return hip_check(hipHostFree(hptr), "hipHostFree");
}

vxg_status vxg_memcpy_h2d(vxg_ctx* ctx, void* dst, const void* src, uint64_t bytes, void* stream) {
    VXG_TRY(use_device(ctx));
    return hip_check(hipMemcpyAsync(dst, src, bytes, hipMemcpyHostToDevice, S(stream)), "h2d");
}

vxg_status vxg_memcpy_d2h(vxg_ctx* ctx, void* dst, const void* src, uint64_t bytes, void* stream) {
    VXG_TRY(use_device(ctx));
    return hip_check(hipMemcpyAsync(dst, src, bytes, hipMemcpyDeviceToHost, S(stream)), "d2h");
}

vxg_status vxg_memcpy_d2d(vxg_ctx* ctx, void* dst, const void* src, uint64_t bytes, void* stream) {
    VXG_TRY(use_device(ctx));
    return hip_check(hipMemcpyAsync(dst, src, bytes, hipMemcpyDeviceToDevice, S(stream)), "d2d");
}

vxg_status vxg_stream_sync(vxg_ctx* ctx, void* stream) {
    VXG_TRY(use_device(ctx));
    VXG_TRY(hip_check(hipStreamSynchronize(S(stream)), "hipStreamSynchronize"));
    uint32_t err = 0;
    VXG_TRY(hip_check(hipMemcpy(&err, ctx->c.err_word, 4, hipMemcpyDeviceToHost), "error word readback"));
    if (err) {
        VXG_TRY(hip_check(hipMemset(ctx->c.err_word, 0, 4), "error word reset"));
        return status_of_err_word(err);
    }
    return VXG_OK;
}

vxg_status vxg_canonical_size(vxg_ctx* ctx, const vxg_array* a, uint64_t* values_bytes, uint64_t* data_bytes) {
    VXG_TRY(use_device(ctx));
    if (!a) return set_error(VXG_ERR_INVALID_ARGUMENT, "null array");
    Planner p(ctx, nullptr);
    uint64_t vb = 0, db = 0;
    VXG_TRY(p.canonical_size(*a, vb, db));
    if (values_bytes) *values_bytes = vb;
    if (data_bytes) *data_bytes = db;
    return VXG_OK;
}

vxg_status vxg_canonical_layout(vxg_ctx* ctx, const vxg_array* a, uint64_t* values_bytes, uint64_t* data_bytes,
                                vxg_data_buffer* bufs, uint32_t cap, uint32_t* n_bufs) {
    VXG_TRY(use_device(ctx));
    if (!a) return set_error(VXG_ERR_INVALID_ARGUMENT, "null array");
    Planner p(ctx, nullptr);
    uint64_t vb = 0, db = 0;
    uint32_t n = 0;
    if (a->dtype == VXG_DTYPE_UTF8 || a->dtype == VXG_DTYPE_BINARY) {
        std::vector<vxg_data_buffer> v;
        VXG_TRY(p.string_layout(*a, v, db));
        vb = 16 * a->len;
        n = uint32_t(v.size());
        if (bufs && cap < n) return set_error(VXG_ERR_INVALID_ARGUMENT, "buffer table too small");
        if (bufs) std::copy(v.begin(), v.end(), bufs);
    } else {
        VXG_TRY(p.canonical_size(*a, vb, db));
    }
    if (values_bytes) *values_bytes = vb;
    if (data_bytes) *data_bytes = db;
    if (n_bufs) *n_bufs = n;
    return VXG_OK;
}

vxg_status vxg_canonicalize(vxg_ctx* ctx, const vxg_array* a, vxg_canonical* out, void* stream) {
    VXG_TRY(use_device(ctx));
    if (!a || !out) return set_error(VXG_ERR_INVALID_ARGUMENT, "null array/out");
    Planner p(ctx, S(stream));
    return p.canonical(*a, *out);
}

}

static uint64_t tree_bytes(const vxg_array& a) {
    uint64_t b = 0;
    for (uint32_t i = 0; i < a.n_buffers; i++) b += a.buffers[i].len;
    for (uint32_t i = 0; i < a.n_children; i++) b += tree_bytes(a.children[i]);
    return b;
}

static uint16_t leading_encoding(const vxg_array& a) {
    return a.encoding == VXG_ENC_CHUNKED && a.n_children ? leading_encoding(a.children[0]) : a.encoding;
}

static uint64_t plan_cost(const vxg_array& a) {
    const bool str = a.dtype == VXG_DTYPE_UTF8 || a.dtype == VXG_DTYPE_BINARY;
    const uint64_t out = a.dtype == VXG_DTYPE_BOOL ? a.len / 8 : a.len * (str ? 16 : ptype_width(a.ptype));
    const uint64_t bytes = tree_bytes(a) + out;
    const uint16_t e = leading_encoding(a);
    const uint64_t pct = e == VXG_ENC_FSST ? 45 : e == VXG_ENC_RUN_END ? 34 : str ? 55 : 70;
    return bytes * 100 / pct;
}

static uint32_t plan_branches_env() {
    static const uint32_t nb = [] {
        const char* e = std::getenv("VXG_PLAN_BRANCHES");
        const long v = e ? std::strtol(e, nullptr, 10) : 0;
        return v >= 1 && v <= 16 ? uint32_t(v) : 0u;
    }();
    return nb;
}

enum class BatchMode { Auto, Off, On, Mixed, Strings };
static BatchMode plan_batch_mode() {
    const char* e = std::getenv("VXG_PLAN_BATCH");
    if (!e || !*e) return BatchMode::Auto;
    if (e[0] == '0') return BatchMode::Off;
    if (e[0] == '1') return BatchMode::On;
    if (e[0] == 'm') return BatchMode::Mixed;
    if (e[0] == 's') return BatchMode::Strings;
    return BatchMode::Auto;
}
static bool dict_string_column(const vxg_array& a) {
    const bool str = a.dtype == VXG_DTYPE_UTF8 || a.dtype == VXG_DTYPE_BINARY;
    if (!str) return false;
    if (a.encoding == VXG_ENC_CHUNKED) {
        for (uint32_t i = 1; i < a.n_children; i++)
            if (a.children[i].encoding != VXG_ENC_DICT) return false;
        return a.n_children > 1;
    }
    return a.encoding == VXG_ENC_DICT;
}
static uint64_t env_bytes(const char* name, uint64_t dflt) {
    const char* e = std::getenv(name);
    return e ? uint64_t(std::strtoull(e, nullptr, 10)) : dflt;
}
static uint64_t plan_batch_max_bytes() { return env_bytes("VXG_PLAN_BATCH_MAX_BYTES", uint64_t(64) << 20); }

static uint64_t canonical_out_bytes(const vxg_array& a) {
    const bool str = a.dtype == VXG_DTYPE_UTF8 || a.dtype == VXG_DTYPE_BINARY;
    return a.dtype == VXG_DTYPE_BOOL ? a.len / 8 : a.len * (str ? 16 : ptype_width(a.ptype));
}

struct FusedNode {
    FsstFusedArgs fa;
    const GenChunk* gtab;
    uint32_t gn, dict_off;
    bool dict_lds;
    uint32_t* err;
    uint64_t gpe;
    void* args[7];
    hipGraphNode_t node = nullptr;
    hipKernelNodeParams p{};
    explicit FusedNode(void** a) {
        fa = *static_cast<const FsstFusedArgs*>(a[0]);
        gtab = *static_cast<const GenChunk* const*>(a[1]);
        gn = *static_cast<const uint32_t*>(a[2]);
        dict_off = *static_cast<const uint32_t*>(a[3]);
        dict_lds = *static_cast<const bool*>(a[4]);
        err = *static_cast<uint32_t* const*>(a[5]);
        gpe = *static_cast<const uint64_t*>(a[6]);
// ... 722 lines not shown
```

vortex_amd/csrc/dict_rows.hip:

```cpp
#include "fl_unpack_impl.hpp"

namespace vxg {

namespace {

constexpr int kRowsThreads = 256;
constexpr int kRowsMaxW = 16;

template <int VW> struct DVal;
template <> struct DVal<8> { using t = uint64_t; };
template <> struct DVal<16> { using t = uint4; };

template <int T, int VW, int BPW, bool LDSD, bool EXT>
__global__ __launch_bounds__(kRowsThreads) void dict_rows_kernel(ChunkTable tab, unsigned W) {
    using E = typename Fl<T>::E;
    using V = typename DVal<VW>::t;
    constexpr unsigned LANES = 1024 / T;
    const uint64_t g = blockIdx.x;
    uint32_t ci;
    if constexpr (EXT) {
        ci = ext_chunk_index(tab.ext, tab.n, g, [](const ChunkDev& d) { return d.first_group; });
    } else {
        uint32_t lo = 0, hi = tab.n;
        while (hi - lo > 1) {
            const uint32_t mid = (lo + hi) >> 1;
            if (tab.c[mid].first_group <= g) lo = mid; else hi = mid;
        }
        ci = lo;
    }
    const ChunkDev& c = EXT ? tab.ext[ci] : tab.c[ci];
    __shared__ __attribute__((aligned(16))) E s_packed[BPW * 128 * kRowsMaxW / sizeof(E)];
    __shared__ __attribute__((aligned(16))) uint8_t s_dict[LDSD ? kDictLdsBytes : 16];
    const unsigned tid = threadIdx.x;
    const uint64_t blk0 = (g - c.first_group) * BPW;
    const unsigned nb = unsigned(c.n_blocks - blk0 < uint64_t(BPW) ? c.n_blocks - blk0 : uint64_t(BPW));
    const unsigned q16 = nb * 8 * W;
    for (unsigned q = tid; q < q16; q += kRowsThreads)
        reinterpret_cast<uint4*>(s_packed)[q] = reinterpret_cast<const uint4*>(c.packed + blk0 * (128ull * W))[q];
    const V* dict = static_cast<const V*>(c.dict);
    if constexpr (LDSD) {
        const unsigned n16 = unsigned((c.dict_len * VW + 15) / 16);
        for (unsigned q = tid; q < n16; q += kRowsThreads)
            reinterpret_cast<uint4*>(s_dict)[q] = static_cast<const uint4*>(c.dict)[q];
        dict = reinterpret_cast<const V*>(s_dict);
    }
    __syncthreads();
    V* __restrict__ out = static_cast<V*>(c.out);
    const RtRows<T> rows(W);
    bool oob = false;
    for (unsigned b = 0; b < nb; b++) {
        const E* __restrict__ pw = s_packed + b * (LANES * W);
        const int64_t base = int64_t((blk0 + b) * 1024) - int64_t(c.offset);
        const bool whole = base >= 0 && uint64_t(base) + 1024 <= c.len;
#pragma unroll
        for (unsigned k = 0; k < 4; k++) {
            const int64_t o = base + int64_t(k * kRowsThreads + tid);
            if (!whole && (o < 0 || uint64_t(o) >= c.len)) continue;
            const uint64_t code = W ? uint64_t(rows.get(pw, k)) : 0;
            const bool bad = code >= c.dict_len;
            oob |= bad;
            nt_store(out + o, dict[bad ? 0 : code]);
        }
    }
    if (oob) __hip_atomic_fetch_or(tab.err, kErrTakeOOB, __ATOMIC_RELAXED, __HIP_MEMORY_SCOPE_AGENT);
}

template <int T, int VW, int BPW, bool LDSD, bool EXT>
vxg_status launch_rows(ChunkTable tab, unsigned W, hipStream_t s) {
    ChunkDev* cs = tab.ext ? tab.host : tab.c;
    uint64_t groups = 0;
    for (uint32_t k = 0; k < tab.n; k++) {
        cs[k].first_group = groups;
        groups += (cs[k].n_blocks + BPW - 1) / BPW;
    }
    if (groups == 0) return VXG_OK;
    if (groups > 0xFFFFFFFFull) return set_error(VXG_ERR_INVALID_ARGUMENT, "array too long for one launch");
    hipLaunchKernelGGL((dict_rows_kernel<T, VW, BPW, LDSD, EXT>), dim3(unsigned(groups)), dim3(kRowsThreads), 0, s,
                       tab, W);
    return hip_check(hipGetLastError(), "dict_rows_kernel launch");
}

template <int T, int VW, int BPW>
vxg_status launch_rows_b(const ChunkTable& tab, unsigned W, bool lds, hipStream_t s) {
    if (tab.ext) return lds ? launch_rows<T, VW, BPW, true, true>(tab, W, s) : launch_rows<T, VW, BPW, false, true>(tab, W, s);
    return lds ? launch_rows<T, VW, BPW, true, false>(tab, W, s) : launch_rows<T, VW, BPW, false, false>(tab, W, s);
}

template <int T, int VW>
vxg_status launch_rows_t(const ChunkTable& tab, unsigned W, hipStream_t s) {
    const ChunkDev* cs = tab.ext ? tab.host : tab.c;
    bool lds = true;
    uint64_t max_dict = 0;
    for (uint32_t k = 0; k < tab.n; k++) {
        lds = lds && cs[k].dict_len * VW <= uint64_t(kDictLdsBytes) && (reinterpret_cast<uintptr_t>(cs[k].dict) & 15) == 0;
        max_dict = cs[k].dict_len * VW > max_dict ? cs[k].dict_len * VW : max_dict;
    }
    if (lds && max_dict > 1024) return launch_rows_b<T, VW, 8>(tab, W, lds, s);
    return launch_rows_b<T, VW, 1>(tab, W, lds, s);
}

}

vxg_status launch_dict_rows(int T, int W, int vw, const ChunkTable& tab, hipStream_t s) {
    if (W < 0 || W > kRowsMaxW || W > T) return VXG_ERR_NOT_IMPLEMENTED;
    const unsigned w = unsigned(W);
#define VXG_ROWS(TT, VV) \
    if (T == TT && vw == VV) return launch_rows_t<TT, VV>(tab, w, s);
    VXG_ROWS(8, 8) VXG_ROWS(16, 8) VXG_ROWS(32, 8) VXG_ROWS(64, 8)
    VXG_ROWS(8, 16) VXG_ROWS(16, 16) VXG_ROWS(32, 16) VXG_ROWS(64, 16)
#undef VXG_ROWS
    return VXG_ERR_NOT_IMPLEMENTED;
}

}
```

vortex_amd/csrc/fl_unpack_impl.hpp:

```cpp
#pragma once

#include <hip/hip_runtime.h>

#include <cstdint>
#include <cstdlib>
#include <type_traits>
#include <utility>

#include "vxg_internal.hpp"
#include "intcol.hpp"

namespace vxg {

template <int T> struct Fl;
template <> struct Fl<8> {
    using E = uint8_t;  using U = uint32_t;
    static constexpr uint32_t rep(uint32_t m) { return m * 0x01010101u; }
};
template <> struct Fl<16> {
    using E = uint16_t; using U = uint32_t;
    static constexpr uint32_t rep(uint32_t m) { return m * 0x00010001u; }
};
template <> struct Fl<32> {
    using E = uint32_t; using U = uint32_t;
// ... 567 lines not shown
                __hip_atomic_fetch_or(err, kErrPatchOOB, __ATOMIC_RELAXED, __HIP_MEMORY_SCOPE_AGENT);
        }
        __builtin_amdgcn_s_waitcnt(0);
        __syncthreads();
        if (s_pscr[0] && s_pscr[1]) {
            if (pin) gstore(out + pkey, pval);
        } else {
            const uint64_t ps = patch_lower_bound(pc, olo, s_pscr + 4);
            const uint64_t pe = patch_lower_bound(pc, ohi, s_pscr + 4);
            bool bad = false;
            for (uint64_t i = ps + threadIdx.x; i < pe; i += 256) {
                const uint64_t key = uint64_t(intcol_get(pc.idx, i)) - pc.idx_off;
                if (key >= olo && key < ohi) gstore(out + key, gload(static_cast<const O*>(pc.vals) + i));
                else bad = true;
            }
            if (bad) __hip_atomic_fetch_or(err, kErrPatchOrder, __ATOMIC_RELAXED, __HIP_MEMORY_SCOPE_AGENT);
        }
    }
}

template <int T, int W, Epi EPI, int VW, bool LDSD, bool EXT>
__global__ __launch_bounds__(256) void fl_unpack_w_kernel(ChunkTable tab) {
    const uint64_t g = blockIdx.x;
    if constexpr (EXT) {
        const ChunkDev& c =
            tab.ext[ext_chunk_index(tab.ext, tab.n, g, [](const ChunkDev& d) { return d.first_group; })];
        unpack_chunk_w<T, W, EPI, VW, LDSD>(c, g, tab.err, PatchCol{}, tab.bpw);
    } else {
        uint32_t lo = 0, hi = tab.n;
        while (hi - lo > 1) {
            const uint32_t mid = (lo + hi) >> 1;
            if (tab.c[mid].first_group <= g) lo = mid; else hi = mid;
        }
        unpack_chunk_w<T, W, EPI, VW, LDSD>(tab.c[lo], g, tab.err, tab.patch, tab.bpw);
    }
}

template <int T, int W, Epi EPI, int VW, bool LDSD = false, int S = 1, bool EXT = false>
__global__ __launch_bounds__(256) void fl_unpack_kernel(ChunkTable tab) {
    const uint64_t g = blockIdx.x;
    if constexpr (EXT) {
        const ChunkDev& c =
            tab.ext[ext_chunk_index(tab.ext, tab.n, g, [](const ChunkDev& d) { return d.first_group; })];
        unpack_chunk<T, W, EPI, VW, LDSD, S>(c, g, tab.err);
    } else {
        uint32_t lo = 0, hi = tab.n;
        while (hi - lo > 1) {
            const uint32_t mid = (lo + hi) >> 1;
            if (tab.c[mid].first_group <= g) lo = mid; else hi = mid;
        }
        unpack_chunk<T, W, EPI, VW, LDSD, S>(tab.c[lo], g, tab.err);
    }
}


inline int k1w_pick_bpw(uint64_t blocks, int bpw_max, int64_t min_groups, int64_t forced) {
    if (forced > 0) return int(forced < bpw_max ? forced : bpw_max);
    if (min_groups <= 0 || blocks >= uint64_t(min_groups) * uint64_t(bpw_max)) return bpw_max;
    const uint64_t b = blocks / uint64_t(min_groups);
    const int bpw = int(b < 4 ? 4 : (b / 4) * 4);
    return bpw > bpw_max ? bpw_max : bpw;
}

template <int T, int W, Epi EPI, int VW, bool LDSD, bool EXT>
vxg_status launch_w(ChunkTable tab, hipStream_t s) {
    constexpr int BPW_MAX = kw_bpw(W, LDSD);
    ChunkDev* cs = tab.ext ? tab.host : tab.c;
    uint64_t blocks = 0;
    for (uint32_t k = 0; k < tab.n; k++) blocks += cs[k].n_blocks;
    const Options o = cur_options();
    const int BPW = k1w_pick_bpw(blocks, BPW_MAX, o.k1w_min_groups, o.k1w_bpw);
    tab.bpw = uint32_t(BPW);
    uint64_t groups = 0, dict_bytes = 0;
    for (uint32_t k = 0; k < tab.n; k++) {
        cs[k].first_group = groups;
        groups += (cs[k].n_blocks + BPW - 1) / BPW;
        const uint64_t db = (cs[k].dict_len * uint64_t(VW > 0 ? VW : 1) + 15) & ~15ull;
        dict_bytes = db > dict_bytes ? db : dict_bytes;
    }
    if (groups == 0) return VXG_OK;
    if (groups > 0xFFFFFFFFull) return set_error(VXG_ERR_INVALID_ARGUMENT, "array too long for one launch");
    const size_t shm = LDSD ? size_t(kw_packed_lds<W, LDSD>()) + size_t(dict_bytes)
                            : size_t(W > 0 ? BPW * 128 * W : 0) + 128;
    hipLaunchKernelGGL((fl_unpack_w_kernel<T, W, EPI, VW, LDSD, EXT>), dim3(unsigned(groups)), dim3(256), shm, s, tab);
    note_k1w_launch(uint32_t(BPW), uint32_t(BPW_MAX), groups);
    if constexpr (!EXT) {
        if (tab.patch.n) g_k1w_wrote_patches = true;
    }
    return hip_check(hipGetLastError(), "fl_unpack_w_kernel launch");
}


template <int T, int W, Epi EPI, int VW, bool LDSD, int S, bool EXT = false>
vxg_status launch_s(ChunkTable tab, hipStream_t s) {
    ChunkDev* cs = tab.ext ? tab.host : tab.c;
    uint64_t groups = 0;
    for (uint32_t k = 0; k < tab.n; k++) {
        cs[k].first_group = groups;
        groups += (cs[k].n_blocks + (32 / S) - 1) / (32 / S);
    }
    if (groups == 0) return VXG_OK;
    if (groups > 0xFFFFFFFFull) return set_error(VXG_ERR_INVALID_ARGUMENT, "array too long for one launch");
    hipLaunchKernelGGL((fl_unpack_kernel<T, W, EPI, VW, LDSD, S, EXT>), dim3(unsigned(groups)), dim3(256), 0, s, tab);
    return hip_check(hipGetLastError(), "fl_unpack_kernel launch");
}

template <int T, int W, Epi EPI, int VW>
vxg_status launch_one(const ChunkTable& tab, uint64_t groups32, hipStream_t s) {
    if (groups32 == 0) return VXG_OK;
    constexpr bool kSplit = (T == 32 || T == 64) && W > 0;
    const bool split = kSplit && groups32 < split_below_groups();
    bool lds = false;
    if constexpr (EPI == Epi::Dict) {
        const ChunkDev* cs = tab.ext ? tab.host : tab.c;
        lds = true;
        for (uint32_t k = 0; k < tab.n; k++)
            lds = lds && cs[k].dict_len * VW <= uint64_t(kDictLdsBytes) &&
                  (reinterpret_cast<uintptr_t>(cs[k].dict) & 15) == 0;
    }
    constexpr uint64_t kExtWaveGroups = 128;
    const int mode = k1_wave_mode();
    const bool big = !split || (tab.ext && groups32 >= kExtWaveGroups);
    const bool wave = mode == 2 || (mode == 1 && big && EPI != Epi::Dict);
    if (tab.ext) {
        if (wave) {
            if constexpr (EPI == Epi::Dict) {
                if (lds) return launch_w<T, W, EPI, VW, true, true>(tab, s);
            }
            return launch_w<T, W, EPI, VW, false, true>(tab, s);
        }
        constexpr int SX = kSplit ? 4 : 1;
        if constexpr (EPI == Epi::Dict) {
            if (lds) return launch_s<T, W, EPI, VW, true, SX, true>(tab, s);
        }
        return launch_s<T, W, EPI, VW, false, SX, true>(tab, s);
    }
    if constexpr (kSplit) {
        if (split && !wave) return lds ? launch_s<T, W, EPI, VW, true, 4>(tab, s) : launch_s<T, W, EPI, VW, false, 4>(tab, s);
    }
    if (wave) {
        if constexpr (EPI == Epi::Dict) {
            if (lds) return launch_w<T, W, EPI, VW, true, false>(tab, s);
        }
        return launch_w<T, W, EPI, VW, false, false>(tab, s);
    }
    if constexpr (EPI == Epi::Dict) {
        if (lds) return launch_s<T, W, EPI, VW, true, 1>(tab, s);
    }
    return launch_s<T, W, EPI, VW, false, 1>(tab, s);
}

template <int T, Epi EPI, int VW, int... Ws>
vxg_status dispatch_w_impl(int W, const ChunkTable& tab, uint64_t groups, hipStream_t s,
                           std::integer_sequence<int, Ws...>) {
    using Fn = vxg_status (*)(const ChunkTable&, uint64_t, hipStream_t);
    static constexpr Fn table[] = {&launch_one<T, Ws, EPI, VW>...};
    if (W < 0 || W >= int(sizeof...(Ws))) return VXG_ERR_NOT_IMPLEMENTED;
    return table[W](tab, groups, s);
}

template <int T, Epi EPI, int VW, int WMAX>
vxg_status dispatch_w(int W, const ChunkTable& tab, uint64_t groups, hipStream_t s) {
    return dispatch_w_impl<T, EPI, VW>(W, tab, groups, s, std::make_integer_sequence<int, WMAX + 1>{});
}

}
```

vortex_amd/csrc/fsst.hip:

```cpp
#include <algorithm>
#include <tuple>

#include "fl_unpack_impl.hpp"
#include "intcol.hpp"
#include "k1g_impl.hpp"

namespace vxg {


namespace {

constexpr int kTile = 256;
constexpr int kTS = kTile;
constexpr int kCodeLds = 6 * 1024;
constexpr int kHeapLds = 10 * 1024;
constexpr int kTPB = 1024 / kTS;
constexpr int kScanTiles = 32 * kTPB;

__device__ __forceinline__ int64_t wave_sum(int64_t x) {
#pragma unroll
    for (int d = 32; d > 0; d >>= 1) x += __shfl_xor(x, d, 64);
    return x;
}

// ... 921 lines not shown
                           int64_t* codes, std::integer_sequence<int, Ws...>) {
    using Fn = void (*)(FsstTable, int64_t*, int64_t*, int64_t*);
    static constexpr Fn table[] = {&fsst_tile_scan_fl32<Ws, false>...};
    static constexpr Fn table_ext[] = {&fsst_tile_scan_fl32<Ws, true>...};
    hipLaunchKernelGGL((t.ext ? table_ext : table)[W], grid, dim3(kScanThreads), 0, s, t, tiles, blocks, codes);
}

template <class F>
bool with_acc(int kind, F&& f) {
    switch (kind) {
    case 1: f(static_cast<PlainCol<1>*>(nullptr)); return true;
    case 2: f(static_cast<PlainCol<2>*>(nullptr)); return true;
    case 4: f(static_cast<PlainCol<4>*>(nullptr)); return true;
    case 8: f(static_cast<PlainCol<8>*>(nullptr)); return true;
    case 32: f(static_cast<PackedCol<32>*>(nullptr)); return true;
    case 64: f(static_cast<PackedCol<64>*>(nullptr)); return true;
    default: return false;
    }
}

}

static size_t fsst_pad_lds() {
    static const size_t v = [] {
        const char* e = std::getenv("VXG_FSST_PAD_LDS");
        const long x = e ? std::strtol(e, nullptr, 10) : 0;
        return size_t(x > 0 && x <= 65536 ? x : 0);
    }();
    return v;
}

hipError_t fsst_diag_init() {
    static const uint32_t m = [] {
        const char* e = std::getenv("VXG_FSST_ABL");
        return e ? uint32_t(std::strtoul(e, nullptr, 10)) : 0u;
    }();
    return m ? hipMemcpyToSymbol(HIP_SYMBOL(g_fsst_abl), &m, sizeof m) : hipSuccess;
}

static bool fused_acc(int oa, int la) { return (oa == 32 && la == 32) || (oa == 4 && la == 4); }

static uint64_t fused_mix_pct() {
    static const uint64_t v = [] {
        const char* e = std::getenv("VXG_FUSED_MIX");
        const long x = e ? std::strtol(e, nullptr, 10) : 100;
        return uint64_t(x >= 0 && x <= 100 ? x : 100);
    }();
    return v;
}

static uint64_t fused_prepass_max_tiles() {
    const char* e = std::getenv("VXG_FUSED_PREPASS_MAX_TILES");
    return e ? uint64_t(std::strtoull(e, nullptr, 10)) : uint64_t(8192);
}
static int64_t fused_delay() {
    static const int64_t v = [] {
        const char* e = std::getenv("VXG_FUSED_DELAY");
        return e ? int64_t(std::strtoull(e, nullptr, 10)) : int64_t(-1);
    }();
    return v;
}

vxg_status launch_fsst_k1g(const FsstFused& fuse, const GenChunk* ext, uint32_t n, uint64_t groups, uint32_t dict_off,
                           bool dict_lds, size_t shm, uint32_t* err, hipStream_t s, uint64_t gpe) {
    if (!fuse.valid || !fused_acc(fuse.oa, fuse.la)) return set_error(VXG_ERR_INVALID_ARGUMENT, "internal: fused FSST group");
    if (n == 0) groups = 0;
    FsstFusedArgs a = fuse.a;
    a.delay = fused_delay() >= 0 ? std::min(uint64_t(fused_delay()), groups) : (a.prepass ? groups : 0);
    a.mix = a.tiles + (groups - a.delay) * fused_mix_pct() / 100;
    const uint64_t grid = a.prepass + a.tiles + groups;
    if (grid == 0) return VXG_OK;
    if (grid > 0xFFFFFFFFull) return set_error(VXG_ERR_INVALID_ARGUMENT, "array too long for one launch");
    shm = std::max<size_t>(shm, kDecLdsBytes + fsst_pad_lds());
    if (fuse.oa == 32)
        hipLaunchKernelGGL((fsst_k1g_kernel<PackedCol<32>, PackedCol<32>>), dim3(unsigned(grid)), dim3(kTile), shm, s, a,
                           ext, n, dict_off, dict_lds, err, gpe);
    else
        hipLaunchKernelGGL((fsst_k1g_kernel<PlainCol<4>, PlainCol<4>>), dim3(unsigned(grid)), dim3(kTile), shm, s, a, ext,
                           n, dict_off, dict_lds, err, gpe);
    return hip_check(hipGetLastError(), "fsst_k1g_kernel launch");
}

vxg_status launch_fsst_batch(std::vector<FsstChunk>& chunks, void* scratch, uint32_t* err, hipStream_t s,
                             DevTables* dt, FsstFused* fuse) {
    if (fuse) fuse->valid = false;
    for (const FsstChunk& c : chunks) {
        if (c.n_symbols > 255) return set_error(VXG_ERR_INVALID_ARGUMENT, "FSST symbol table > 255 entries");
        if ((c.n + kTS - 1) / kTS > 0xFFFFFFFFull) return set_error(VXG_ERR_INVALID_ARGUMENT, "FSST array too long");
        if (acc_kind(c.offs) == 0 || acc_kind(c.lens) == 0 || (c.offs.packed && c.offs.width != 4 && c.offs.width != 8) ||
            (c.lens.packed && c.lens.width != 4 && c.lens.width != 8))
            return set_error(VXG_ERR_MISMATCHED_TYPES, "FSST offsets/lengths must be 1/2/4/8-byte integers "
                                                        "(packed: 32/64-bit)");
    }
    std::stable_sort(chunks.begin(), chunks.end(),
                     [](const FsstChunk& a, const FsstChunk& b) { return fsst_key(a) < fsst_key(b); });
    int64_t* tiles_all = static_cast<int64_t*>(scratch);
    size_t i = 0;
    while (i < chunks.size()) {
        FsstTable tab{};
        uint64_t tiles = 0, scans = 0;
        size_t j = i, live = 0;
        while (j < chunks.size() && (dt || j - i < size_t(kFsstArgChunks)) && fsst_key(chunks[j]) == fsst_key(chunks[i]))
            live += chunks[j++].n != 0;
        const bool fusing = fuse && dt && !fuse->valid && live &&
                            fused_acc(std::get<0>(fsst_key(chunks[i])), std::get<1>(fsst_key(chunks[i])));
        uint64_t group_tiles = 0;
        for (size_t k = i; k < j; k++) group_tiles += (chunks[k].n + kTS - 1) / kTS;
        const bool ingrid = fusing && group_tiles <= fused_prepass_max_tiles();
        const uint64_t scan_tiles = ingrid ? uint64_t(kFusedScanTiles) : uint64_t(kScanTiles);
        FsstChunk* cs = tab.c;
        if (live > size_t(kFsstArgChunks) || fusing) {
            FsstChunk* host;
            const vxg_status st = dt->table(live, &host, &tab.ext);
            if (st != VXG_OK) return st;
            cs = host;
        }
        for (size_t k = i; k < j; k++) {
            if (chunks[k].n == 0) continue;
            FsstChunk& c = cs[tab.n++];
            c = chunks[k];
            const uint64_t nt = (c.n + kTS - 1) / kTS;
            c.first_tile = tiles;
            c.first_scan = scans;
            tiles += nt;
            scans += (nt + scan_tiles - 1) / scan_tiles;
        }
        if (tab.n) {
            const uint32_t* wg_chunk = nullptr;
            if (tab.ext) {
                uint32_t* host_map;
                const vxg_status st = dt->table(tiles, &host_map, &wg_chunk);
                if (st != VXG_OK) return st;
                for (uint32_t k = 0; k < tab.n; k++) {
                    const FsstChunk& c = cs[k];
                    const uint64_t nt = (c.n + kTS - 1) / kTS;
                    for (uint64_t t = 0; t < nt; t++) host_map[c.first_tile + t] = k;
                }
            }
            const auto key = fsst_key(cs[0]);
            if (ingrid) {
                int64_t* rec_host;
                const int64_t* rec;
                uint32_t* scan_host;
                const uint32_t* scan_chunk;
                vxg_status st = dt->table(2 * tiles + scans, &rec_host, &rec);
                if (st == VXG_OK) st = dt->table(scans, &scan_host, &scan_chunk);
                if (st != VXG_OK) return st;
                for (uint32_t k = 0; k < tab.n; k++) {
                    const FsstChunk& c = cs[k];
                    const uint64_t ns = ((c.n + kTS - 1) / kTS + kFusedScanTiles - 1) / kFusedScanTiles;
                    for (uint64_t b = 0; b < ns; b++) scan_host[c.first_scan + b] = k;
                }
                int64_t* r = const_cast<int64_t*>(rec);
                fuse->valid = true;
                fuse->oa = std::get<0>(key);
                fuse->la = std::get<1>(key);
                fuse->a = FsstFusedArgs{tab.ext, r, r + tiles, r + tiles + scans, wg_chunk, tiles, tiles,
                                        scans, 0, scan_chunk, 1};
                i = j;
                continue;
            }
            int64_t* tp = tiles_all;
            int64_t* bt = tiles_all + tiles;
            int64_t* tc = bt + scans;
            tiles_all += 2 * tiles + scans;
            if (std::get<2>(key) >= 0)
                launch_tile_scan_fl32(std::get<2>(key), dim3(unsigned(scans)), s, tab, tp, bt, tc,
                                      std::make_integer_sequence<int, 33>{});
            if (fusing) {
                if (std::get<2>(key) < 0) {
                    bool ok = with_acc(std::get<1>(key), [&](auto* la) {
                        using LA = std::remove_pointer_t<decltype(la)>;
                        hipLaunchKernelGGL((fsst_tile_scan<LA, true>), dim3(unsigned(scans)), dim3(kTile), 0, s, tab, tp,
                                           bt, tc);
                    });
                    if (!ok) return set_error(VXG_ERR_MISMATCHED_TYPES, "FSST accessor");
                }
                fuse->valid = true;
                fuse->oa = std::get<0>(key);
                fuse->la = std::get<1>(key);
                fuse->a = FsstFusedArgs{tab.ext, tp, bt, tc, wg_chunk, tiles, tiles, 0, 0, nullptr, 0};
                const vxg_status st = hip_check(hipGetLastError(), "fsst pre-pass");
                if (st != VXG_OK) return st;
                i = j;
                continue;
            }
            bool ok = true;
            with_acc(std::get<0>(key), [&](auto* oa) {
                ok = with_acc(std::get<1>(key), [&](auto* la) {
                    using OA = std::remove_pointer_t<decltype(oa)>;
                    using LA = std::remove_pointer_t<decltype(la)>;
                    auto go = [&](auto ext) {
                        constexpr bool X = decltype(ext)::value;
                        if (std::get<2>(key) < 0)
                            hipLaunchKernelGGL((fsst_tile_scan<LA, X>), dim3(unsigned(scans)), dim3(kTile), 0, s, tab,
                                               tp, bt, tc);
                        hipLaunchKernelGGL((fsst_decode<OA, LA, X>), dim3(unsigned(tiles)), dim3(kTile), fsst_pad_lds(), s,
                                           tab, tp, bt, tc, err, wg_chunk);
                    };
                    if (tab.ext) go(std::true_type{});
                    else go(std::false_type{});
                });
            });
            if (!ok) return set_error(VXG_ERR_MISMATCHED_TYPES, "FSST accessor");
            const vxg_status st = hip_check(hipGetLastError(), "fsst kernels");
            if (st != VXG_OK) return st;
        }
        i = j;
    }
    return VXG_OK;
}

}
```

vortex_amd/csrc/k1g.hip:

```cpp
#include <algorithm>

#include "k1g_impl.hpp"

namespace vxg {

namespace {

__global__ __launch_bounds__(kGenThreads) void k1_generic_kernel(const GenChunk* __restrict__ tab, uint32_t n,
                                                                 uint32_t dict_off, bool dict_lds, uint32_t* err,
                                                                 uint64_t gpe) {
    extern __shared__ __attribute__((aligned(16))) uint8_t lds[];
    const uint64_t g = blockIdx.x;
    const GenChunk& gc = tab[ext_chunk_index_gpe(tab, n, g, gpe, [](const GenChunk& d) { return d.d.first_group; })];
    gen_dispatch(int(gc.kind), gc, g, lds, dict_off, dict_lds, err);
}

}

int gen_runs_kind(int value_width) {
    switch (value_width) {
    case 1: return 38;
    case 2: return 39;
    case 4: return 40;
    case 8: return 41;
    case 16: return 42;
    default: return -1;
    }
}

int gen_kind(int T, int epi, int vw, bool varbin_dict) {
    const int ti = T == 8 ? 0 : T == 16 ? 1 : T == 32 ? 2 : T == 64 ? 3 : -1;
    if (ti < 0) return -1;
    if (varbin_dict) return Epi(epi) == Epi::Dict && vw == 16 ? 34 + ti : -1;
    switch (Epi(epi)) {
    case Epi::Plain: return 3 * ti;
    case Epi::For: return 3 * ti + 1;
    case Epi::ForZigZag: return 3 * ti + 2;
    case Epi::AlpF32: return T == 32 ? 12 : -1;
    case Epi::AlpF64: return T == 64 ? 13 : -1;
    case Epi::Dict: {
        const int vi = vw == 1 ? 0 : vw == 2 ? 1 : vw == 4 ? 2 : vw == 8 ? 3 : vw == 16 ? 4 : -1;
        return vi < 0 ? -1 : 14 + 5 * ti + vi;
    }
    }
    return -1;
}

static long gen_bpw_env() {
    static const long v = [] {
        const char* e = std::getenv("VXG_K1G_BPW");
        const long x = e ? std::strtol(e, nullptr, 10) : 0;
        return x >= 1 && x <= 32 ? x : 0L;
    }();
    return v;
}

constexpr uint64_t kGenWideMinGroups = 2048;
uint32_t gen_bpw_cap(uint64_t blocks) {
    if (const long v = gen_bpw_env()) return uint32_t(v);
    return blocks / 8 >= kGenWideMinGroups ? 8u : 4u;
}

uint32_t gen_bpw(int T, int W, uint32_t cap) {
    (void)T;
    const uint32_t per = 128u * uint32_t(W > 0 ? W : 1);
    const uint32_t b = kGenPackedLds / per, m = cap ? cap : (gen_bpw_env() ? uint32_t(gen_bpw_env()) : 4u);
    return b > m ? m : (b < 1 ? 1 : b);
}

uint32_t gen_vb_bpw(int T, int W, bool alone, uint32_t cap) {
    static const long v = [] {
        const char* e = std::getenv("VXG_K1G_VB_BPW");
        return e ? std::strtol(e, nullptr, 10) : 0L;
    }();
    const uint32_t b = gen_bpw(T, W, v >= 1 && uint32_t(v) > cap ? uint32_t(v) : cap);
    const uint32_t want = v >= 1 ? uint32_t(v) : (alone ? 1u : b);
    return want < b ? want : b;
}

uint32_t gen_runs_lds_bytes(int value_width) {
    switch (value_width) {
    case 1: return uint32_t(runs_lds_bytes<uint8_t>());
    case 2: return uint32_t(runs_lds_bytes<uint16_t>());
    case 4: return uint32_t(runs_lds_bytes<uint32_t>());
    case 8: return uint32_t(runs_lds_bytes<uint64_t>());
    default: return uint32_t(runs_lds_bytes<uint4>());
    }
}

vxg_status launch_k1_generic(const GenChunk* ext, uint32_t n, uint64_t groups, bool dict_lds, uint32_t packed_bytes,
                             uint32_t dict_bytes, uint32_t runs_bytes, uint32_t* err, hipStream_t s,
                             uint64_t gpe, const FsstFused* fuse) {
    static_assert(kGenVarBinDictMax * 16 <= uint64_t(kDictLdsBytes), "VarBin views must fit the dictionary stage");
    if (n == 0) groups = 0;
    if (groups == 0 && !(fuse && fuse->valid)) return VXG_OK;
    if (groups > 0xFFFFFFFFull) return set_error(VXG_ERR_INVALID_ARGUMENT, "array too long for one launch");
    if (packed_bytes > kGenPackedLds || dict_bytes > uint32_t(kDictLdsBytes))
        return set_error(VXG_ERR_INVALID_ARGUMENT, "K1g stage sizes");
    const uint32_t dict_off = (packed_bytes + 128 + 15) & ~15u;
    const size_t shm = std::max<size_t>({size_t(dict_off) + dict_bytes, size_t(runs_bytes), 16});
    if (fuse && fuse->valid) return launch_fsst_k1g(*fuse, ext, n, groups, dict_off, dict_lds, shm, err, s, gpe);
    hipLaunchKernelGGL(k1_generic_kernel, dim3(unsigned(groups)), dim3(kGenThreads), shm, s, ext, n, dict_off, dict_lds,
                       err, gpe);
    return hip_check(hipGetLastError(), "k1_generic_kernel launch");
}

}
```

vortex_amd/csrc/kernels.hip:

```cpp
#include "fl_unpack_impl.hpp"
#include "intcol.hpp"
#include "runend_runs.hpp"

namespace vxg {

namespace {

constexpr int kBlock = 256;

inline unsigned grid_for(uint64_t n_threads) {
    uint64_t g = (n_threads + kBlock - 1) / kBlock;
    const uint64_t cap = 256ull * 8 * 16;
    if (g > cap) g = cap;
    if (g == 0) g = 1;
    return unsigned(g);
}

__device__ __forceinline__ uint64_t load_uint(const void* p, int width, bool sgn, uint64_t i) {
    switch (width) {
    case 1: return sgn ? uint64_t(int64_t(gload(static_cast<const int8_t*>(p) + i))) : gload(static_cast<const uint8_t*>(p) + i);
    case 2: return sgn ? uint64_t(int64_t(gload(static_cast<const int16_t*>(p) + i))) : gload(static_cast<const uint16_t*>(p) + i);
    case 4: return sgn ? uint64_t(int64_t(gload(static_cast<const int32_t*>(p) + i))) : gload(static_cast<const uint32_t*>(p) + i);
    default: return gload(static_cast<const uint64_t*>(p) + i);
    }
// ... 511 lines not shown
        c = tab.c[lo];
    }
    const V* __restrict__ values = static_cast<const V*>(c.values.p);
    const void* ends = c.ends.p;
    V* __restrict__ out = static_cast<V*>(c.out);
    const int ew = c.ends.width, tid = threadIdx.x;
    const uint64_t j0 = (g - c.first_group) * SPAN;
    const int jn = int(c.len - j0 < uint64_t(SPAN) ? c.len - j0 : uint64_t(SPAN));
    const uint64_t jend = j0 + uint64_t(jn);
    if (tid < 64) {
        const uint64_t r0 = runend_locate(ends, ew, c.offset, c.n_runs, c.len, j0);
        if (tid == 0) s_r0 = r0;
    } else if (tid == 64) {
        s_bad = c.n_runs == 0 || load_uint(ends, ew, false, c.n_runs - 1) - c.offset < c.len;
    }
#pragma unroll
    for (int k = 0; k < PER; k++) s_head[tid + k * kBlock] = 0;
    __syncthreads();
    if (s_bad) {
        if (tid == 0) __hip_atomic_fetch_or(tab.err, kErrRunEnd, __ATOMIC_RELAXED, __HIP_MEMORY_SCOPE_AGENT);
        return;
    }
    const uint64_t r0 = s_r0;
    constexpr int Q = 4;
    for (uint64_t rb = r0;; rb += uint64_t(Q) * kBlock) {
        uint64_t st[Q];
#pragma unroll
        for (int q = 0; q < Q; q++) {
            const uint64_t r = rb + uint64_t(q) * kBlock + uint64_t(tid);
            st[q] = r + 1 < c.n_runs ? load_uint(ends, ew, false, r) - c.offset : ~0ull;
        }
#pragma unroll
        for (int q = 0; q < Q; q++)
            if (st[q] < jend) s_head[st[q] - j0] = uint32_t(rb + uint64_t(q) * kBlock + uint64_t(tid) + 1 - r0);
        if (!__syncthreads_or(st[Q - 1] < jend)) break;
    }
    __syncthreads();
    uint32_t v[PER];
    uint32_t m = 0;
#pragma unroll
    for (int k = 0; k < PER; k++) {
        m = max(m, s_head[tid * PER + k]);
        v[k] = m;
    }
    uint32_t x = m;
#pragma unroll
    for (int d = 1; d < 64; d <<= 1) {
        const uint32_t y = __shfl_up(x, d, 64);
        if ((tid & 63) >= d) x = max(x, y);
    }
    if ((tid & 63) == 63) s_wmax[tid >> 6] = x;
    __syncthreads();
    uint32_t before = __shfl_up(x, 1, 64);
    if ((tid & 63) == 0) before = 0;
#pragma unroll
    for (int w = 0; w < kBlock / 64; w++)
        if (w < (tid >> 6)) before = max(before, s_wmax[w]);
#pragma unroll
    for (int k = 0; k < PER; k++) s_head[tid * PER + k] = max(v[k], before);
    __syncthreads();
    for (int i = tid; i < jn; i += kBlock) nt_store(out + j0 + i, gload(values + r0 + s_head[i]));
}

template <typename V>
__global__ __launch_bounds__(kBlock) void runend_runs_kernel(RunEndTable tab) {
    __shared__ __attribute__((aligned(16))) uint8_t lds[runs_lds_bytes<V>()];
    const uint64_t g = blockIdx.x;
    RunEndChunk c;
    if (tab.ext) {
        c = tab.ext[ext_chunk_index(tab.ext, tab.n, g, [](RunEndChunk const& d) { return d.first_group; })];
    } else {
        uint32_t lo = 0, hi = tab.n;
        while (hi - lo > 1) {
            const uint32_t mid = (lo + hi) >> 1;
            if (tab.c[mid].first_group <= g) lo = mid; else hi = mid;
        }
        c = tab.c[lo];
    }
    runend_runs_body<V>(c, g, tab.err, lds);
}

vxg_status launch_runend_runs(int value_width, const RunEndTable& t, uint64_t groups, hipStream_t s) {
    if (groups == 0) return VXG_OK;
    switch (value_width) {
#define RR_CASE(W)                                                                                                \
    case W:                                                                                                       \
        hipLaunchKernelGGL((runend_runs_kernel<typename UInt<W>::t>), dim3(unsigned(groups)), dim3(kBlock), 0, s, t); \
        break;
        RR_CASE(1) RR_CASE(2) RR_CASE(4) RR_CASE(8) RR_CASE(16)
#undef RR_CASE
    default: return VXG_ERR_INVALID_ARGUMENT;
    }
    return hip_check(hipGetLastError(), "runend_runs_kernel");
}

vxg_status launch_runend_chunks(int value_width, const RunEndTable& t, uint64_t groups, hipStream_t s) {
    if (groups == 0) return VXG_OK;
    switch (value_width) {
#define RE_CASE(W)                                                                                  \
    case W:                                                                                         \
        hipLaunchKernelGGL((runend_chunks_kernel<typename UInt<W>::t>), dim3(unsigned(groups)), dim3(kBlock), 0, s, t); \
        break;
        RE_CASE(1) RE_CASE(2) RE_CASE(4) RE_CASE(8) RE_CASE(16)
#undef RE_CASE
    default: return VXG_ERR_INVALID_ARGUMENT;
    }
    return hip_check(hipGetLastError(), "runend_chunks_kernel");
}

vxg_status launch_runend(int value_width, const RunEndChunk& chunk, uint32_t* err, hipStream_t s) {
    if (chunk.len == 0) return VXG_OK;
    if (chunk.n_runs == 0) return set_error(VXG_ERR_INVALID_ARGUMENT, "RunEnd with len > 0 has no runs");
    RunEndTable t{};
    t.err = err;
    t.n = 1;
    t.c[0] = chunk;
    t.c[0].first_group = 0;
    if (chunk.len <= kRunEndShortRun * chunk.n_runs)
        return launch_runend_runs(value_width, t, (chunk.n_runs + kRunEndRunsPerGroup - 1) / kRunEndRunsPerGroup, s);
    if (chunk.ends.packed || chunk.values.packed)
        return set_error(VXG_ERR_INVALID_ARGUMENT, "long-run RunEnd expansion reads plain ends/values");
    return launch_runend_chunks(value_width, t, (chunk.len + kRunEndSpan - 1) / kRunEndSpan, s);
}

template <typename V>
__global__ __launch_bounds__(kBlock) void fill_kernel(V v, uint64_t n, V* __restrict__ out) {
    const uint64_t stride = uint64_t(gridDim.x) * blockDim.x;
    for (uint64_t i = uint64_t(blockIdx.x) * blockDim.x + threadIdx.x; i < n; i += stride) nt_store(out + i, v);
}

vxg_status launch_fill(int value_width, const uint8_t* scalar16, uint64_t n, void* out, hipStream_t s) {
    if (n == 0) return VXG_OK;
    const unsigned g = grid_for(n);
    switch (value_width) {
#define FILL_CASE(W)                                                                                \
    case W: {                                                                                       \
        typename UInt<W>::t v;                                                                      \
        __builtin_memcpy(&v, scalar16, W);                                                          \
        hipLaunchKernelGGL((fill_kernel<typename UInt<W>::t>), dim3(g), dim3(kBlock), 0, s, v, n,   \
                           static_cast<typename UInt<W>::t*>(out));                                 \
    } break;
        FILL_CASE(1) FILL_CASE(2) FILL_CASE(4) FILL_CASE(8) FILL_CASE(16)
#undef FILL_CASE
    default: return VXG_ERR_INVALID_ARGUMENT;
    }
    return hip_check(hipGetLastError(), "fill_kernel");
}

__device__ __forceinline__ uint32_t abyte(uint32_t hi, uint32_t lo, uint32_t sh) {
    return __builtin_amdgcn_alignbyte(hi, lo, sh);
}
template <int QD>
__device__ __forceinline__ uint4 funnel16(const uint4& lo, const uint4& hi, uint32_t rb) {
    const uint32_t w[8] = {lo.x, lo.y, lo.z, lo.w, hi.x, hi.y, hi.z, hi.w};
    return make_uint4(abyte(w[QD + 1], w[QD], rb), abyte(w[QD + 2], w[QD + 1], rb), abyte(w[QD + 3], w[QD + 2], rb),
                      abyte(w[QD + 4], w[QD + 3], rb));
}

__global__ __launch_bounds__(kBlock) void copy_bytes_kernel(uint8_t* __restrict__ dst, const uint8_t* __restrict__ src,
                                                            uint64_t n, uint64_t head, uint64_t body, uint32_t r) {
    const uint64_t stride = uint64_t(gridDim.x) * blockDim.x;
    const uint64_t t0 = uint64_t(blockIdx.x) * blockDim.x + threadIdx.x;
    uint4* const d16 = reinterpret_cast<uint4*>(dst + head);
    if (!src) {
        for (uint64_t q = t0; q < body; q += stride) gstore(d16 + q, make_uint4(0, 0, 0, 0));
    } else if (r == 0) {
        const uint4* const s16 = reinterpret_cast<const uint4*>(src + head);
        for (uint64_t q = t0; q < body; q += stride) gstore(d16 + q, gload(s16 + q));
    } else {
        const uint4* const s16 = reinterpret_cast<const uint4*>(src + head - r);
        const uint32_t qd = r >> 2, rb = r & 3;
        for (uint64_t q = t0; q < body; q += stride) {
            const uint4 lo = gload(s16 + q), hi = gload(s16 + q + 1);
            uint4 v;
            if (qd == 0) v = funnel16<0>(lo, hi, rb);
            else if (qd == 1) v = funnel16<1>(lo, hi, rb);
            else if (qd == 2) v = funnel16<2>(lo, hi, rb);
            else v = funnel16<3>(lo, hi, rb);
            gstore(d16 + q, v);
        }
// ... 18 lines not shown
}

__device__ __forceinline__ uint4 make_view(const uint8_t* __restrict__ heap, uint64_t start, uint32_t len,
                                          uint32_t bidx) {
    const uint8_t* p = heap + start;
    uint32_t w1 = 0, w2 = 0, w3 = 0;
    if (len <= 12) {
#pragma unroll
        for (int j = 0; j < 12; j++) {
            const uint32_t b = uint32_t(j) < len ? uint32_t(gload(p + j)) : 0u;
            if (j < 4) w1 |= b << (8 * j);
            else if (j < 8) w2 |= b << (8 * (j - 4));
            else w3 |= b << (8 * (j - 8));
        }
    } else {
#pragma unroll
        for (int j = 0; j < 4; j++) w1 |= uint32_t(gload(p + j)) << (8 * j);
        w2 = bidx;
        w3 = uint32_t(start);
    }
    return make_uint4(len, w1, w2, w3);
}

__device__ __forceinline__ uint4 checked_view(const uint8_t* __restrict__ heap, uint64_t heap_len, uint64_t a,
                                              uint64_t e, uint32_t bidx, uint32_t* err) {
    if (a > e || e > heap_len) {
        __hip_atomic_fetch_or(err, kErrVarBin, __ATOMIC_RELAXED, __HIP_MEMORY_SCOPE_AGENT);
        return make_uint4(0, 0, 0, 0);
    }
    return make_view(heap, a, uint32_t(e - a), bidx);
}

__global__ __launch_bounds__(kBlock) void varbin_views_kernel(const uint8_t* __restrict__ heap, uint64_t heap_len,
                                                              const void* offs, int offs_width, uint64_t n,
                                                              const uint8_t* __restrict__ validity,
                                                              uint32_t bidx, uint4* __restrict__ views, uint32_t* err) {
    const uint64_t stride = uint64_t(gridDim.x) * blockDim.x;
    for (uint64_t i = uint64_t(blockIdx.x) * blockDim.x + threadIdx.x; i < n; i += stride) {
        if (validity && !((validity[i >> 3] >> (i & 7)) & 1)) {
            views[i] = make_uint4(0, 0, 0, 0);
            continue;
        }
        const uint64_t a = load_uint(offs, offs_width, offs_width < 8, i);
        const uint64_t b = load_uint(offs, offs_width, offs_width < 8, i + 1);
        views[i] = checked_view(heap, heap_len, a, b, bidx, err);
    }
}

vxg_status launch_varbin_views(const uint8_t* heap, uint64_t heap_len, int offs_width, const void* offsets, uint64_t n,
                               const uint8_t* validity, uint32_t bidx, uint8_t* views, uint32_t* err, hipStream_t s) {
    if (n == 0) return VXG_OK;
    hipLaunchKernelGGL(varbin_views_kernel, dim3(grid_for(n)), dim3(kBlock), 0, s, heap, heap_len, offsets,
                       offs_width, n, validity, bidx, reinterpret_cast<uint4*>(views), err);
    return hip_check(hipGetLastError(), "varbin_views_kernel");
}

__global__ __launch_bounds__(kBlock) void varbin_chunks_kernel(VarBinTable tab) {
    const uint64_t g = blockIdx.x;
    VarBinChunk c;
    if (tab.ext) {
        c = tab.ext[ext_chunk_index(tab.ext, tab.n, g, [](VarBinChunk const& d) { return d.first_group; })];
    } else {
        uint32_t lo = 0, hi = tab.n;
        while (hi - lo > 1) {
            const uint32_t mid = (lo + hi) >> 1;
            if (tab.c[mid].first_group <= g) lo = mid; else hi = mid;
        }
        c = tab.c[lo];
    }
    const uint64_t lg = g - c.first_group;
    const uint64_t ng = (c.n + kBlock - 1) / kBlock > 0 ? (c.n + kBlock - 1) / kBlock : 1;
    const uint64_t per = (c.bytes + ng - 1) / ng;
    for (uint64_t b = lg * per + threadIdx.x; b < c.bytes && b < (lg + 1) * per; b += kBlock) gstore(c.dst + b, gload(c.src + b));
    const uint64_t i = lg * kBlock + threadIdx.x;
    if (i < c.n) {
        const uint64_t a = load_uint(c.offsets, int(c.offs_width), c.offs_width < 8, i);
        const uint64_t e = load_uint(c.offsets, int(c.offs_width), c.offs_width < 8, i + 1);
        gstore(reinterpret_cast<uint4*>(c.views) + i, checked_view(c.src, c.bytes, a, e, c.bidx, tab.err));
    }
}

vxg_status launch_varbin_chunks(const VarBinTable& t, uint64_t groups, hipStream_t s) {
    if (groups == 0) return VXG_OK;
    hipLaunchKernelGGL(varbin_chunks_kernel, dim3(unsigned(groups)), dim3(kBlock), 0, s, t);
    return hip_check(hipGetLastError(), "varbin_chunks_kernel");
}

__global__ __launch_bounds__(kBlock) void views_rebase_kernel(const uint4* __restrict__ src, uint64_t n, uint32_t add,
                                                              uint4* __restrict__ dst) {
    const uint64_t stride = uint64_t(gridDim.x) * blockDim.x;
    for (uint64_t i = uint64_t(blockIdx.x) * blockDim.x + threadIdx.x; i < n; i += stride) {
        uint4 v = src[i];
        if (v.x > 12) v.z += add;
        dst[i] = v;
    }
}

vxg_status launch_views_rebase(const uint8_t* src, uint64_t n, uint32_t add, uint8_t* dst, hipStream_t s) {
    if (n == 0) return VXG_OK;
    hipLaunchKernelGGL(views_rebase_kernel, dim3(grid_for(n)), dim3(kBlock), 0, s,
                       reinterpret_cast<const uint4*>(src), n, add, reinterpret_cast<uint4*>(dst));
    return hip_check(hipGetLastError(), "views_rebase_kernel");
}

__device__ __forceinline__ void put_bits(uint32_t* __restrict__ dst, uint64_t pos, uint32_t word, bool full) {
    const uint64_t w = pos >> 5;
    const int sh = int(pos & 31);
    if (full && sh == 0) {
        dst[w] = word;
        return;
    }
    if (!word) return;
    atomicOr(dst + w, word << sh);
    if (sh) {
        const uint32_t hi = word >> (32 - sh);
        if (hi) atomicOr(dst + w + 1, hi);
    }
}

constexpr int kBoolSpan = 32 * kBlock;
__global__ __launch_bounds__(kBlock) void runend_bool_kernel(const void* __restrict__ ends, int ew, uint64_t n_runs,
                                                             uint64_t offset, int start, uint64_t len,
                                                             uint32_t* __restrict__ dst, uint64_t dst_off,
                                                             uint32_t* __restrict__ err) {
    __shared__ uint32_t s_flip[kBlock];
    __shared__ uint32_t s_wpar[kBlock / 64];
    __shared__ uint64_t s_r0;
    const int tid = threadIdx.x, lane = tid & 63, wave = tid >> 6;
    const uint64_t j0 = uint64_t(blockIdx.x) * kBoolSpan;
    const uint64_t jend = len - j0 < uint64_t(kBoolSpan) ? len : j0 + kBoolSpan;
    s_flip[tid] = 0;
    if (tid < 64) {
        const uint64_t r0 = runend_first_gt(ends, ew, offset, n_runs, j0);
        if (tid == 0) s_r0 = r0;
        if (blockIdx.x == 0 && tid == 0 && load_uint(ends, ew, false, n_runs - 1) - offset < len)
            __hip_atomic_fetch_or(err, kErrRunEnd, __ATOMIC_RELAXED, __HIP_MEMORY_SCOPE_AGENT);
    }
    __syncthreads();
    const uint64_t r0 = s_r0;
    if (r0 >= n_runs) {
        return;
    }
    for (uint64_t r = r0 + tid; r < n_runs; r += kBlock) {
        const uint64_t e = load_uint(ends, ew, false, r) - offset;
        if (e >= jend) break;
        const uint32_t p = uint32_t(e - j0);
        atomicXor(&s_flip[p >> 5], 1u << (p & 31));
    }
    __syncthreads();
    const uint32_t f = s_flip[tid];
    uint32_t x = f;
    x ^= x << 1;
    x ^= x << 2;
    x ^= x << 4;
    x ^= x << 8;
    x ^= x << 16;
    const unsigned long long bal = __ballot(__popc(f) & 1);
    const uint32_t below = uint32_t(__popcll(bal & ((1ull << lane) - 1ull)) & 1);
    if (lane == 0) s_wpar[wave] = uint32_t(__popcll(bal) & 1);
    __syncthreads();
    uint32_t carry = below ^ uint32_t(start != 0) ^ uint32_t(r0 & 1);
    for (int w = 0; w < wave; w++) carry ^= s_wpar[w];
    uint32_t word = x ^ (carry ? 0xFFFFFFFFu : 0u);
    const uint64_t p0 = j0 + uint64_t(tid) * 32;
    if (p0 >= jend) return;
    const uint64_t nb = jend - p0;
// ... 99 lines not shown
```

vortex_amd/csrc/vxg_internal.hpp:

```cpp
#pragma once

#include <hip/hip_runtime.h>

#include <cstdint>
#include <cstdlib>
#include <mutex>
#include <string>
#include <type_traits>
#include <vector>

#include "../../include/vortex_gpu.h"

namespace vxg {

__host__ __device__ constexpr int fl_order(int i) {
    constexpr int o[8] = {0, 4, 2, 6, 1, 5, 3, 7};
    return o[i];
}
__host__ __device__ constexpr int fl_index(int row, int lane) {
    return fl_order(row / 8) * 16 + (row % 8) * 128 + lane;
}

template <class T>
using gptr = __attribute__((address_space(1))) T*;
template <class T>
__device__ __forceinline__ T gload(const T* p) {
    if constexpr (sizeof(T) == 16 && !std::is_scalar_v<T>) {
        using u32x4 = unsigned int __attribute__((ext_vector_type(4)));
        const u32x4 x = *(gptr<const u32x4>)p;
        T r;
        __builtin_memcpy(&r, &x, 16);
        return r;
    } else {
        return *(gptr<const T>)p;
    }
}
template <class T>
__device__ __forceinline__ void gstore(T* p, const T& v) {
    if constexpr (sizeof(T) == 16 && !std::is_scalar_v<T>) {
        using u32x4 = unsigned int __attribute__((ext_vector_type(4)));
        u32x4 x;
        __builtin_memcpy(&x, &v, 16);
        *(gptr<u32x4>)p = x;
    } else {
        *(gptr<T>)p = v;
    }
}
template <class T>
__device__ __forceinline__ T lds_load(const T* p) {
    if constexpr (sizeof(T) == 16 && !std::is_scalar_v<T>) {
        using u32x4 = unsigned int __attribute__((ext_vector_type(4)));
        const u32x4 x = *(__attribute__((address_space(3))) const u32x4*)p;
        T r;
        __builtin_memcpy(&r, &x, 16);
        return r;
    } else {
        return *(__attribute__((address_space(3))) const T*)p;
    }
}

template <typename V>
__device__ __forceinline__ void nt_store(V* p, const V& v) {
    if constexpr (sizeof(V) == 16) {
        using u32x4 = unsigned int __attribute__((ext_vector_type(4)));
        u32x4 vv;
        __builtin_memcpy(&vv, &v, 16);
        __builtin_nontemporal_store(vv, (gptr<u32x4>)p);
    } else {
        __builtin_nontemporal_store(v, (gptr<V>)p);
    }
}

inline int ptype_width(int p) {
    switch (p) {
    case VXG_U8: case VXG_I8: return 1;
    case VXG_U16: case VXG_I16: case VXG_F16: return 2;
    case VXG_U32: case VXG_I32: case VXG_F32: return 4;
    case VXG_U64: case VXG_I64: case VXG_F64: return 8;
    default: return 0;
    }
}
inline bool ptype_is_int(int p) { return p >= VXG_U8 && p <= VXG_I64; }
inline bool ptype_is_signed(int p) { return p >= VXG_I8 && p <= VXG_I64; }
inline bool ptype_is_unsigned(int p) { return p >= VXG_U8 && p <= VXG_U64; }

extern const float kF10f[11];
extern const float kIF10f[11];
extern const double kF10d[24];
extern const double kIF10d[24];

enum : uint32_t { kErrTakeOOB = 1u, kErrPatchOOB = 2u, kErrRunEnd = 4u, kErrFsst = 8u, kErrRoaring = 16u, kErrVarBin = 32u,
                  kErrPatchOrder = 64u, kErrPlanSync = 128u };

struct Options {
    int64_t k1w_min_groups = 1024;
    int64_t k1w_bpw = 0;
    int64_t k1_wave = -1;
};
struct LaunchStats {
    uint64_t k1w_launches = 0, k1w_last_groups = 0;
    uint32_t k1w_last_bpw = 0, k1w_min_bpw = 0, k1w_max_bpw = 0, k1w_last_bpw_max = 0;
};

struct Ctx {
    int device = 0;
    uint32_t* err_word = nullptr;
    Options opt;
    std::mutex mu;
    LaunchStats st;
};
extern thread_local Ctx* g_cur_ctx;
Options default_options();
inline Options cur_options() { return g_cur_ctx ? g_cur_ctx->opt : default_options(); }
inline int k1_wave_mode() {
    const int64_t o = cur_options().k1_wave;
    if (o >= 0) return int(o > 2 ? 2 : o);
    const char* e = std::getenv("VXG_K1_WAVE");
    if (!e) return 1;
    return e[0] == '0' ? 0 : (e[0] == 'f' ? 2 : 1);
}
void note_k1w_launch(uint32_t bpw, uint32_t bpw_max, uint64_t groups);

vxg_status set_error(vxg_status s, const std::string& msg);
vxg_status hip_check(hipError_t e, const char* what);

struct DevTables {
    std::vector<void*> allocs;
    std::vector<std::pair<void*, std::vector<uint8_t>>> uploads;
    template <class E>
    vxg_status table(size_t n, E** host, const E** dev) {
        void* d = nullptr;
        const hipError_t e = hipMalloc(&d, n * sizeof(E) + 16);
        if (e != hipSuccess) return hip_check(e, "hipMalloc (plan chunk table)");
        allocs.push_back(d);
        uploads.emplace_back(d, std::vector<uint8_t>(n * sizeof(E), 0));
        *host = reinterpret_cast<E*>(uploads.back().second.data());
        *dev = static_cast<const E*>(d);
        return VXG_OK;
    }
    vxg_status upload() {
        for (auto& u : uploads) {
            const hipError_t e = hipMemcpy(u.first, u.second.data(), u.second.size(), hipMemcpyHostToDevice);
            if (e != hipSuccess) return hip_check(e, "plan chunk table upload");
        }
        uploads.clear();
        return VXG_OK;
    }
};

template <class E, class Key>
__device__ __forceinline__ uint32_t ext_chunk_index(const E* __restrict__ ext, uint32_t n, uint64_t g, Key key) {
    const uint32_t lane = threadIdx.x & 63u;
    uint32_t cnt = 0;
    for (uint32_t base = 0; base < n; base += 256) {
        uint64_t kv[4];
#pragma unroll
        for (int k = 0; k < 4; k++) {
            const uint32_t i = base + 64u * uint32_t(k) + lane;
            kv[k] = uint64_t(key(ext[i < n ? i : n - 1]));
        }
#pragma unroll
        for (int k = 0; k < 4; k++) {
            const bool le = base + 64u * uint32_t(k) + lane < n && kv[k] <= g;
            cnt += uint32_t(__popcll(__ballot(le)));
        }
    }
    return cnt ? cnt - 1 : 0;
}

template <class E, class Key>
__device__ __forceinline__ uint32_t ext_chunk_index_gpe(const E* __restrict__ ext, uint32_t n, uint64_t g, uint64_t gpe,
                                                        Key key) {
    if (gpe) {
        const uint32_t q = uint32_t(g) / uint32_t(gpe);
        const uint32_t ci = __builtin_amdgcn_readfirstlane(q < n - 1 ? q : n - 1);
        const uint64_t f0 = uint64_t(key(ext[ci]));
        const uint64_t f1 = ci + 1 < n ? uint64_t(key(ext[ci + 1])) : ~0ull;
        if (f0 <= g && g < f1) return ci;
    }
    return ext_chunk_index(ext, n, g, key);
}
inline uint64_t common_groups(const uint64_t* counts, size_t n) {
    static const bool on = [] {
        const char* e = std::getenv("VXG_EXT_GPE");
        return !(e && e[0] == '0');
    }();
    if (!on || n == 0 || counts[0] == 0) return 0;
    for (size_t i = 1; i + 1 < n; i++)
        if (counts[i] != counts[0]) return 0;
    return counts[n - 1] <= counts[0] ? counts[0] : 0;
}

enum class Epi : int { Plain = 0, For = 1, ForZigZag = 2, AlpF32 = 3, AlpF64 = 4, Dict = 5 };

struct UnpackArgs {
    const uint8_t* packed;
    void* out;
    uint64_t n_blocks;
    uint32_t offset;
    uint64_t len;
    uint64_t reference;
    uint32_t shift;
    double alp_a, alp_b;
    const void* dict;
    uint64_t dict_len;
    uint32_t* err;
};

struct ChunkDev {
    const uint8_t* packed;
    void* out;
    uint64_t n_blocks;
    uint64_t len;
    uint64_t first_group;
    uint64_t reference;
    double alp_a, alp_b;
    const void* dict;
    uint64_t dict_len;
    uint32_t offset;
    uint32_t shift;
};
constexpr int kArgChunks = 32;
struct ChunkTable;

vxg_status launch_fl_unpack(int T, int W, Epi epi, int value_width, const ChunkTable& tab, uint64_t groups,
                            hipStream_t s);

struct IntCol {
    const void* p;
    int width;
    bool sgn;
// ... 87 lines not shown
};
vxg_status launch_runend(int value_width, const RunEndChunk& chunk, uint32_t* err, hipStream_t s);
constexpr uint64_t kRunEndSpan = 4096;
constexpr int kRunEndArgChunks = 32;
struct RunEndTable {
    RunEndChunk c[kRunEndArgChunks];
    uint32_t n;
    uint32_t* err;
    const RunEndChunk* ext;
};
vxg_status launch_runend_chunks(int value_width, const RunEndTable& t, uint64_t groups, hipStream_t s);
constexpr uint64_t kRunEndShortRun = 16;
constexpr uint64_t kRunEndRunsPerGroup = 1024;
vxg_status launch_runend_runs(int value_width, const RunEndTable& t, uint64_t groups, hipStream_t s);

struct VarBinChunk {
    const uint8_t* src;
    uint8_t* dst;
    const void* offsets;
    uint8_t* views;
    uint64_t bytes;
    uint64_t n;
    uint64_t first_group;
    uint32_t offs_width;
    uint32_t bidx;
};
constexpr int kVarBinArgChunks = 48;
struct VarBinTable {
    VarBinChunk c[kVarBinArgChunks];
    uint32_t n;
    const VarBinChunk* ext;
    uint32_t* err;
};
vxg_status launch_varbin_chunks(const VarBinTable& t, uint64_t groups, hipStream_t s);

vxg_status launch_copy_bytes(void* dst, const void* src, uint64_t n, hipStream_t s);
vxg_status launch_fill(int value_width, const uint8_t* scalar16, uint64_t n, void* out,
                       hipStream_t s);
struct FsstChunk {
    const uint64_t* symbols;
    const uint8_t* sym_lens;
    const uint8_t* codes;
    const uint8_t* validity;
    uint8_t* heap;
    uint8_t* views;
    IntCol offs;
    IntCol lens;
    uint64_t n;
    uint64_t heap_len;
    uint64_t first_tile;
    uint64_t first_scan;
    uint32_t n_symbols;
    uint32_t bidx;
};
constexpr int kFsstArgChunks = 24;
struct FsstTable {
    FsstChunk c[kFsstArgChunks];
    uint32_t n;
    const FsstChunk* ext;
};
uint64_t fsst_scratch_bytes(uint64_t n);
uint64_t fsst_batch_scratch_bytes(const FsstChunk* chunks, size_t n_chunks);
struct FsstFusedArgs {
    const FsstChunk* ext;
    const int64_t* tp;
    const int64_t* bt;
    const int64_t* tc;
    const uint32_t* wg_chunk;
    uint64_t tiles;
    uint64_t mix;
    uint64_t prepass;
    uint64_t delay;
    const uint32_t* scan_chunk;
    uint32_t tag;
};
bool is_fsst_fused_kernel(const void* func);
struct FsstFused {
    bool valid = false;
    int oa = 0, la = 0;
    FsstFusedArgs a{};
};
hipError_t fsst_diag_init();
vxg_status launch_fsst_batch(std::vector<FsstChunk>& chunks, void* scratch, uint32_t* err, hipStream_t s,
                             DevTables* dt = nullptr, FsstFused* fuse = nullptr);
vxg_status launch_varbin_views(const uint8_t* heap, uint64_t heap_len, int offs_width, const void* offsets, uint64_t n,
                               const uint8_t* validity, uint32_t bidx, uint8_t* views, uint32_t* err, hipStream_t s);
vxg_status launch_views_rebase(const uint8_t* src, uint64_t n, uint32_t add, uint8_t* dst, hipStream_t s);

}
```

Before: 4812.

## Add per-call pinned-memory chunk tables so unplanned decodes batch many chunks per launch

Adds a per-context pool of pinned host regions, mapped for device access, plus matching device regions. Unplanned canonicalize calls can now put chunk descriptor tables larger than the kernel-argument limit into these regions and copy them to the device on the stream before each launch, using either a copy kernel or hipMemcpyAsync. This lets K1, run-end, varbin and FSST batches cover all chunks in one launch instead of splitting at kArgChunks, which cuts launch count. Regions are recycled through events, and the feature is on by default with a new option to turn it off; it costs an extra small copy per launch and more complexity.

```diff
diff --git a/include/vortex_gpu.h b/include/vortex_gpu.h
--- a/include/vortex_gpu.h
+++ b/include/vortex_gpu.h
@@ -8,7 +8,7 @@
 extern "C" {
 #endif
 
-#define VXG_ABI_VERSION 9
+#define VXG_ABI_VERSION 10
 
 typedef enum vxg_status {
     VXG_OK = 0,
@@ -122,7 +122,8 @@
 typedef enum vxg_option {
     VXG_OPT_K1W_MIN_GROUPS = 1,
     VXG_OPT_K1W_BPW = 2,
-    VXG_OPT_K1_WAVE = 3
+    VXG_OPT_K1_WAVE = 3,
+    VXG_OPT_DIRECT_TABLES = 4
 } vxg_option;
 vxg_status vxg_set_option(vxg_ctx* ctx, int option, int64_t value);
 vxg_status vxg_get_option(vxg_ctx* ctx, int option, int64_t* value);
diff --git a/rust/vortex-gpu/src/ffi.rs b/rust/vortex-gpu/src/ffi.rs
--- a/rust/vortex-gpu/src/ffi.rs
+++ b/rust/vortex-gpu/src/ffi.rs
@@ -2,7 +2,7 @@
 
 use std::os::raw::{c_char, c_int, c_uint, c_void};
 
-pub const VXG_ABI_VERSION: c_int = 9;
+pub const VXG_ABI_VERSION: c_int = 10;
 pub type vxg_status = c_int;
 pub const VXG_OK: vxg_status = 0;
 pub const VXG_ERR_OUT_OF_BOUNDS: vxg_status = 1;
@@ -247,6 +247,7 @@
 pub const VXG_OPT_K1W_MIN_GROUPS: vxg_option = 1;
 pub const VXG_OPT_K1W_BPW: vxg_option = 2;
 pub const VXG_OPT_K1_WAVE: vxg_option = 3;
+pub const VXG_OPT_DIRECT_TABLES: vxg_option = 4;
 
 #[repr(C)]
 #[derive(Copy, Clone, Debug)]
diff --git a/vortex_amd/_lib.py b/vortex_amd/_lib.py
--- a/vortex_amd/_lib.py
+++ b/vortex_amd/_lib.py
@@ -15,7 +15,7 @@
 PTYPE = {n: i for i, n in enumerate(PTYPES)}
 DTYPE = dict(NULL=0, BOOL=1, PRIMITIVE=2, UTF8=3, BINARY=4)
 VALIDITY = dict(NON_NULLABLE=0, ALL_VALID=1, ALL_INVALID=2, ARRAY=3)
-ABI_VERSION = 9
+ABI_VERSION = 10
 STATUS = {0: "OK", 1: "OutOfBounds", 2: "ComputeError", 3: "InvalidArgument", 4: "InvalidSerde",
           5: "NotImplemented", 6: "MismatchedTypes", 7: "AssertionFailed", 8: "HipError",
           9: "OutOfMemory"}
@@ -143,7 +143,7 @@
 PLAN_SELECTION = {0: "single", 1: "faster", 2: "tie_fewer_nodes", 3: "unmeasured"}
 
 
-OPT_K1W_MIN_GROUPS, OPT_K1W_BPW, OPT_K1_WAVE = 1, 2, 3
+OPT_K1W_MIN_GROUPS, OPT_K1W_BPW, OPT_K1_WAVE, OPT_DIRECT_TABLES = 1, 2, 3, 4
 
 
 class VxgLaunchStats(C.Structure):
diff --git a/vortex_amd/arrays.py b/vortex_amd/arrays.py
--- a/vortex_amd/arrays.py
+++ b/vortex_amd/arrays.py
@@ -457,7 +457,7 @@
         _lib.check(self.lib.vxg_stream_sync(self.handle, self.stream_ptr()))
 
     _OPTIONS = {"k1w_min_groups": _lib.OPT_K1W_MIN_GROUPS, "k1w_bpw": _lib.OPT_K1W_BPW,
-                "k1_wave": _lib.OPT_K1_WAVE}
+                "k1_wave": _lib.OPT_K1_WAVE, "direct_tables": _lib.OPT_DIRECT_TABLES}
 
     def set_option(self, name: str, value: int):
         _lib.check(self.lib.vxg_set_option(self.handle, self._OPTIONS[name], int(value)))
diff --git a/vortex_amd/csrc/capi.hip b/vortex_amd/csrc/capi.hip
--- a/vortex_amd/csrc/capi.hip
+++ b/vortex_amd/csrc/capi.hip
@@ -102,6 +102,161 @@
     st.k1w_last_groups = groups;
 }
 
+thread_local CallTablesCall* g_call_tables = nullptr;
+
+static bool call_tables_memcpy() {
+    static const bool v = [] {
+        const char* e = std::getenv("VXG_CALL_TABLES_COPY");
+        return e && e[0] == 'm';
+    }();
+    return v;
+}
+
+CallTables::Region* CallTables::acquire(size_t need) {
+    int polls = 0;
+    for (Region* r : regions) {
+        if (r->in_call) continue;
+        if (r->pending) {
+            if (polls < 0 || polls == 2) continue;
+            polls++;
+            if (hipEventQuery(r->done) != hipSuccess) {
+                (void)hipGetLastError();
+                polls = -1;
+                continue;
+            }
+            r->pending = false;
+        }
+        if (r->cap < need) continue;
+        r->in_call = true;
+        return r;
+    }
+    const size_t rcap = need <= kRegionBytes ? kRegionBytes : (need + kRegionBytes - 1) / kRegionBytes * kRegionBytes;
+    const size_t nreg = need <= kRegionBytes ? kSegmentRegions : 1;
+    if (bytes + rcap * nreg > kMaxBytes) return nullptr;
+    void *h = nullptr, *hd = nullptr, *d = nullptr;
+    std::vector<hipEvent_t> evs;
+    bool ok = hipHostMalloc(&h, rcap * nreg, hipHostMallocDefault) == hipSuccess &&
+              hipHostGetDevicePointer(&hd, h, 0) == hipSuccess && hipMalloc(&d, rcap * nreg) == hipSuccess;
+    for (size_t k = 0; ok && k < nreg; k++) {
+        hipEvent_t ev;
+        ok = hipEventCreateWithFlags(&ev, hipEventDisableTiming) == hipSuccess;
+        if (ok) evs.push_back(ev);
+    }
+    if (!ok) {
+        (void)hipGetLastError();
+        for (hipEvent_t ev : evs) (void)hipEventDestroy(ev);
+        if (d) (void)hipFree(d);
+        if (h) (void)hipHostFree(h);
+        return nullptr;
+    }
+    segments.emplace_back(h, d);
+    bytes += rcap * nreg;
+    for (size_t k = 0; k < nreg; k++) {
+        Region* r = new Region();
+        r->host = static_cast<uint8_t*>(h) + k * rcap;
+        r->host_dev = static_cast<const uint8_t*>(hd) + k * rcap;
+        r->dev = static_cast<uint8_t*>(d) + k * rcap;
+        r->cap = rcap;
+        r->done = evs[k];
+        regions.push_back(r);
+    }
+    Region* r = regions[regions.size() - nreg];
+    r->in_call = true;
+    return r;
+}
+
+void CallTables::destroy() {
+    for (Region* r : regions) {
+        (void)hipEventDestroy(r->done);
+        delete r;
+    }
+    for (auto& [h, d] : segments) {
+        (void)hipFree(d);
+        (void)hipHostFree(h);
+    }
+    regions.clear();
+    segments.clear();
+    bytes = 0;
+}
+
+bool CallTablesCall::usable() {
+    if (state_ == 0) {
+        state_ = -1;
+        hipStreamCaptureStatus cs = hipStreamCaptureStatusNone;
+        if (ctx_->opt.direct_tables == 0) return false;
+        if (hipStreamIsCapturing(s_, &cs) != hipSuccess) {
+            (void)hipGetLastError();
+            return false;
+        }
+        if (cs == hipStreamCaptureStatusNone) state_ = 1;
+    }
+    return state_ > 0;
+}
+
+bool CallTablesCall::grow(size_t need) {
+    std::lock_guard<std::mutex> lk(ctx_->mu);
+    if (!ctx_->call_tables) ctx_->call_tables = new CallTables();
+    CallTables::Region* r = ctx_->call_tables->acquire(need);
+    if (!r) return false;
+    uses_.push_back(Use{r, 0, 0});
+    return true;
+}
+
+bool CallTablesCall::reserve(size_t bytes) {
+    if (!usable()) return false;
+    const size_t total = reserved_ + bytes + 256;
+    if ((uses_.empty() || uses_.back().r->cap - uses_.back().used < total) && !grow(total)) return false;
+    reserved_ = total;
+    return true;
+}
+
+vxg_status CallTablesCall::alloc(size_t bytes, void** host, const void** dev) {
+    const size_t take = (bytes + 16 + 63) & ~size_t(63);
+    if (!usable()) return set_error(VXG_ERR_INVALID_ARGUMENT, "internal: device table in a call that cannot take one");
+    if ((uses_.empty() || uses_.back().r->cap - uses_.back().used < take) && !grow(reserved_ + take))
+        return set_error(VXG_ERR_OUT_OF_MEMORY, "no room for the call's chunk table");
+    Use& u = uses_.back();
+    std::memset(u.r->host + u.used, 0, take);
+    *host = u.r->host + u.used;
+    *dev = u.r->dev + u.used;
+    u.used += take;
+    reserved_ -= std::min(reserved_, take);
+    return VXG_OK;
+}
+
+vxg_status CallTablesCall::commit(hipStream_t s) {
+    for (Use& u : uses_) {
+        if (u.committed == u.used) continue;
+        const size_t n = u.used - u.committed;
+        if (call_tables_memcpy()) {
+            const hipError_t e = hipMemcpyAsync(u.r->dev + u.committed, u.r->host + u.committed, n, hipMemcpyHostToDevice, s);
+            if (e != hipSuccess) return hip_check(e, "chunk table copy");
+        } else {
+            const vxg_status st = launch_copy_bytes(u.r->dev + u.committed, u.r->host_dev + u.committed, n, s);
+            if (st != VXG_OK) return st;
+        }
+        u.committed = u.used;
+    }
+    return VXG_OK;
+}
+
+CallTablesCall::~CallTablesCall() {
+    if (g_call_tables == this) g_call_tables = nullptr;
+    if (uses_.empty()) return;
+    std::lock_guard<std::mutex> lk(ctx_->mu);
+    for (Use& u : uses_) {
+        u.r->pending = u.committed > 0;
+        if (u.r->pending && hipEventRecord(u.r->done, s_) != hipSuccess) {
+            (void)hipGetLastError();
+            continue;
+        }
+        u.r->in_call = false;
+        auto& rs = ctx_->call_tables->regions;
+        rs.erase(std::find(rs.begin(), rs.end(), u.r));
+        rs.push_back(u.r);
+    }
+}
+
 bool k1_takes_wave(int T, int W, Epi epi, uint64_t groups32) {
     const int mode = k1_wave_mode();
     const bool split = (T == 32 || T == 64) && W > 0 && groups32 < split_below_groups();
@@ -176,7 +331,7 @@
     return j.epi == Epi::Dict ? j.vw : (j.epi == Epi::AlpF32 ? 4 : (j.epi == Epi::AlpF64 ? 8 : j.T / 8));
 }
 
-vxg_status launch_k1_jobs(std::vector<K1Job>& jobs, uint32_t* err, hipStream_t s, DevTables* dt = nullptr,
+vxg_status launch_k1_jobs(std::vector<K1Job>& jobs, uint32_t* err, hipStream_t s, Tables* dt = nullptr,
                           bool generic_small = false,
                           const std::vector<std::pair<int, RunEndChunk>>* gen_runs = nullptr,
                           const PatchCol* patch = nullptr, const FsstFused* fuse = nullptr) {
@@ -220,6 +375,8 @@
             out_bytes += jobs[j].d.len * uint64_t(k1_out_width(jobs[j]));
             j++;
         }
+        if (live > size_t(kArgChunks) && !jobs[i].vb && !dt->reserve(live * sizeof(ChunkDev)))
+            j = i + size_t(kArgChunks);
         if (jobs[i].vb || (dt && generic_small && out_bytes < k1g_max_bytes() &&
                            gen_kind(jobs[i].T, int(jobs[i].epi), jobs[i].vw) >= 0)) {
             if (!dt) return set_error(VXG_ERR_INVALID_ARGUMENT, "VarBin-dictionary K1 jobs need a plan");
@@ -362,13 +519,14 @@
     return launch_k1_jobs(jobs, ctx->c.err_word, S(stream));
 }
 
-vxg_status launch_runs(std::vector<RunEndChunk> runs, int w, uint32_t* err, hipStream_t s, DevTables* dt) {
+vxg_status launch_runs(std::vector<RunEndChunk> runs, int w, uint32_t* err, hipStream_t s, Tables* dt) {
     runs.erase(std::remove_if(runs.begin(), runs.end(), [](const RunEndChunk& r) { return r.len == 0; }), runs.end());
     std::vector<RunEndChunk> short_runs, long_runs;
     for (const RunEndChunk& r : runs) (r.len <= kRunEndShortRun * r.n_runs ? short_runs : long_runs).push_back(r);
     for (int pass = 0; pass < 2; pass++) {
         std::vector<RunEndChunk>& rs = pass == 0 ? short_runs : long_runs;
-        const size_t per = dt && rs.size() > size_t(kRunEndArgChunks) ? rs.size() : size_t(kRunEndArgChunks);
+        const size_t per = dt && rs.size() > size_t(kRunEndArgChunks) && dt->reserve(rs.size() * sizeof(RunEndChunk))
+                               ? rs.size() : size_t(kRunEndArgChunks);
         for (size_t i = 0; i < rs.size(); i += per) {
             RunEndTable tab{};
             tab.err = err;
@@ -410,8 +568,9 @@
     return !(e && e[0] == '0');
 }
 
-vxg_status launch_varbin_dicts(const std::vector<VarBinChunk>& dicts, uint32_t* err, hipStream_t s, DevTables* dt) {
-    const size_t per = dt && dicts.size() > size_t(kVarBinArgChunks) ? dicts.size() : size_t(kVarBinArgChunks);
+vxg_status launch_varbin_dicts(const std::vector<VarBinChunk>& dicts, uint32_t* err, hipStream_t s, Tables* dt) {
+    const size_t per = dt && dicts.size() > size_t(kVarBinArgChunks) && dt->reserve(dicts.size() * sizeof(VarBinChunk))
+                           ? dicts.size() : size_t(kVarBinArgChunks);
     for (size_t i = 0; i < dicts.size(); i += per) {
         VarBinTable tab{};
         tab.err = err;
@@ -466,8 +625,9 @@
 
 class Planner {
   public:
-    Planner(vxg_ctx* ctx, hipStream_t s, DevTables* plan = nullptr, PlanBatch* batch = nullptr)
-        : ctx_(ctx), s_(s), plan_(plan), batch_(batch) {}
+    Planner(vxg_ctx* ctx, hipStream_t s, DevTables* plan = nullptr, PlanBatch* batch = nullptr,
+            Tables* call_tables = nullptr)
+        : ctx_(ctx), s_(s), plan_(plan), tables_(plan ? static_cast<Tables*>(plan) : call_tables), batch_(batch) {}
     ~Planner() {
         for (void* p : temps_) (void)hipFreeAsync(p, s_);
     }
@@ -486,6 +646,7 @@
     hipStream_t s_;
     std::vector<void*> temps_;
     DevTables* plan_ = nullptr;
+    Tables* tables_ = nullptr;
     PlanBatch* batch_ = nullptr;
     const vxg_array* root_ = nullptr;
     bool defer(const vxg_array& a) const { return batch_ && &a == root_; }
@@ -683,7 +844,7 @@
         return VXG_OK;
     }
     std::vector<K1Job> one{j};
-    VXG_TRY(launch_k1_jobs(one, ctx_->c.err_word, s_, plan_, false, nullptr, fused_patch_));
+    VXG_TRY(launch_k1_jobs(one, ctx_->c.err_word, s_, tables_, false, nullptr, fused_patch_));
     if (p) VXG_TRY(apply_sparse_patches(*p, T, epi, vw, a, dst, bp.len));
     return VXG_OK;
 }
@@ -892,9 +1053,9 @@
         for (size_t k = 0; k < runs.size(); k++) batch_->runs.push_back(PlanBatch::Run{w, runs[k], runs_indep[k] != 0});
         return VXG_OK;
     }
-    VXG_TRY(launch_k1_jobs(jobs, ctx_->c.err_word, s_, plan_));
+    VXG_TRY(launch_k1_jobs(jobs, ctx_->c.err_word, s_, tables_));
     for (const PatchJob& p : patches) VXG_TRY(apply_sparse_patches(*p.sp, p.T, p.epi, p.vw, p.a, p.dst, p.out_len));
-    return launch_runs(runs, w, ctx_->c.err_word, s_, plan_);
+    return launch_runs(runs, w, ctx_->c.err_word, s_, tables_);
 }
 
 vxg_status Planner::decode_alprd(const vxg_array& a, void* dst) {
@@ -1814,7 +1975,7 @@
         std::vector<FsstChunk> one{f};
         void* scratch;
         VXG_TRY(temp(fsst_batch_scratch_bytes(one.data(), 1), &scratch));
-        return launch_fsst_batch(one, scratch, ctx_->c.err_word, s_, plan_);
+        return launch_fsst_batch(one, scratch, ctx_->c.err_word, s_, tables_);
     }
     case VXG_ENC_DICT: {
         const vxg_array* values = child(a, 0);
@@ -1855,9 +2016,15 @@
                    k.encoding == VXG_ENC_FL_BITPACKED && ptype_is_unsigned(k.ptype) && !k.nullable &&
                    k.meta.bitpacked.bit_width <= kDictFusedMaxW;
         };
-        uint64_t dict_rows = 0;
+        uint64_t dict_rows = 0, n_dict = 0;
         for (uint64_t i = 0; i < n; i++)
-            if (dict_batchable(a.children[i + 1])) dict_rows += a.children[i + 1].children[0].len;
+            if (dict_batchable(a.children[i + 1])) {
+                dict_rows += a.children[i + 1].children[0].len;
+                n_dict++;
+            }
+        const bool vb_form = defer(a) || (plan_ ? plan_vb_k1g()
+                                                : tables_ && n_dict > uint64_t(kArgChunks) && plan_vb_k1g() &&
+                                                      tables_->reserve(n_dict * sizeof(GenChunk)));
         uint8_t* dviews = nullptr;
         if (dict_rows) {
             void* t;
@@ -1890,7 +2057,7 @@
                 d.offs_width = uint32_t(width(v.children[0]));
                 d.bidx = bidx + b;
                 const vxg_array& codes = c.children[1];
-                const bool vb = (defer(a) || (plan_ && plan_vb_k1g())) && v.len <= kGenVarBinDictMax && v.len > 0 &&
+                const bool vb = vb_form && v.len <= kGenVarBinDictMax && v.len > 0 &&
                                 codes.len > 0 && !codes.meta.bitpacked.has_patches;
                 if (!vb) dicts.push_back(d);
                 UnpackArgs ua{};
@@ -1934,15 +2101,15 @@
         } else if (!fssts.empty()) {
             void* scratch;
             VXG_TRY(temp(fsst_batch_scratch_bytes(fssts.data(), fssts.size()), &scratch));
-            VXG_TRY(launch_fsst_batch(fssts, scratch, ctx_->c.err_word, s_, plan_));
+            VXG_TRY(launch_fsst_batch(fssts, scratch, ctx_->c.err_word, s_, tables_));
         }
         if (defer(a) && patches.empty()) {
             batch_->dicts.insert(batch_->dicts.end(), dicts.begin(), dicts.end());
             batch_->jobs.insert(batch_->jobs.end(), jobs.begin(), jobs.end());
             return VXG_OK;
         }
-        VXG_TRY(launch_varbin_dicts(dicts, ctx_->c.err_word, s_, plan_));
-        VXG_TRY(launch_k1_jobs(jobs, ctx_->c.err_word, s_, plan_));
+        VXG_TRY(launch_varbin_dicts(dicts, ctx_->c.err_word, s_, tables_));
+        VXG_TRY(launch_k1_jobs(jobs, ctx_->c.err_word, s_, tables_));
         for (const PatchJob& p : patches) VXG_TRY(apply_sparse_patches(*p.sp, p.T, p.epi, p.vw, p.a, p.dst, p.out_len));
         return VXG_OK;
     }
@@ -2091,6 +2258,10 @@
         if (value < -1 || value > 2) return set_error(VXG_ERR_INVALID_ARGUMENT, "K1_WAVE must be -1, 0, 1 or 2");
         o.k1_wave = value;
         return VXG_OK;
+    case VXG_OPT_DIRECT_TABLES:
+        if (value < 0 || value > 1) return set_error(VXG_ERR_INVALID_ARGUMENT, "DIRECT_TABLES must be 0 or 1");
+        o.direct_tables = value;
+        return VXG_OK;
     }
     return set_error(VXG_ERR_INVALID_ARGUMENT, "unknown option " + std::to_string(option));
 }
@@ -2102,6 +2273,7 @@
     case VXG_OPT_K1W_MIN_GROUPS: *value = o.k1w_min_groups; return VXG_OK;
     case VXG_OPT_K1W_BPW: *value = o.k1w_bpw; return VXG_OK;
     case VXG_OPT_K1_WAVE: *value = o.k1_wave; return VXG_OK;
+    case VXG_OPT_DIRECT_TABLES: *value = o.direct_tables; return VXG_OK;
     }
     return set_error(VXG_ERR_INVALID_ARGUMENT, "unknown option " + std::to_string(option));
 }
@@ -2127,6 +2299,10 @@
     (void)hipSetDevice(ctx->c.device);
     (void)hipDeviceSynchronize();
     if (ctx->c.err_word) (void)hipFree(ctx->c.err_word);
+    if (ctx->c.call_tables) {
+        ctx->c.call_tables->destroy();
+        delete ctx->c.call_tables;
+    }
     delete ctx;
     return VXG_OK;
 }
@@ -2215,7 +2391,9 @@
 vxg_status vxg_canonicalize(vxg_ctx* ctx, const vxg_array* a, vxg_canonical* out, void* stream) {
     VXG_TRY(use_device(ctx));
     if (!a || !out) return set_error(VXG_ERR_INVALID_ARGUMENT, "null array/out");
-    Planner p(ctx, S(stream));
+    CallTablesCall tables(&ctx->c, S(stream));
+    g_call_tables = &tables;
+    Planner p(ctx, S(stream), nullptr, nullptr, &tables);
     return p.canonical(*a, *out);
 }
 
diff --git a/vortex_amd/csrc/dict_rows.hip b/vortex_amd/csrc/dict_rows.hip
--- a/vortex_amd/csrc/dict_rows.hip
+++ b/vortex_amd/csrc/dict_rows.hip
@@ -75,6 +75,10 @@
     }
     if (groups == 0) return VXG_OK;
     if (groups > 0xFFFFFFFFull) return set_error(VXG_ERR_INVALID_ARGUMENT, "array too long for one launch");
+    if constexpr (EXT) {
+        const vxg_status cs = commit_call_tables(s);
+        if (cs != VXG_OK) return cs;
+    }
     hipLaunchKernelGGL((dict_rows_kernel<T, VW, BPW, LDSD, EXT>), dim3(unsigned(groups)), dim3(kRowsThreads), 0, s,
                        tab, W);
     return hip_check(hipGetLastError(), "dict_rows_kernel launch");
diff --git a/vortex_amd/csrc/fl_unpack_impl.hpp b/vortex_amd/csrc/fl_unpack_impl.hpp
--- a/vortex_amd/csrc/fl_unpack_impl.hpp
+++ b/vortex_amd/csrc/fl_unpack_impl.hpp
@@ -673,6 +673,10 @@
     if (groups > 0xFFFFFFFFull) return set_error(VXG_ERR_INVALID_ARGUMENT, "array too long for one launch");
     const size_t shm = LDSD ? size_t(kw_packed_lds<W, LDSD>()) + size_t(dict_bytes)
                             : size_t(W > 0 ? BPW * 128 * W : 0) + 128;
+    if constexpr (EXT) {
+        const vxg_status cs = commit_call_tables(s);
+        if (cs != VXG_OK) return cs;
+    }
     hipLaunchKernelGGL((fl_unpack_w_kernel<T, W, EPI, VW, LDSD, EXT>), dim3(unsigned(groups)), dim3(256), shm, s, tab);
     note_k1w_launch(uint32_t(BPW), uint32_t(BPW_MAX), groups);
     if constexpr (!EXT) {
@@ -692,6 +696,10 @@
     }
     if (groups == 0) return VXG_OK;
     if (groups > 0xFFFFFFFFull) return set_error(VXG_ERR_INVALID_ARGUMENT, "array too long for one launch");
+    if constexpr (EXT) {
+        const vxg_status cs = commit_call_tables(s);
+        if (cs != VXG_OK) return cs;
+    }
     hipLaunchKernelGGL((fl_unpack_kernel<T, W, EPI, VW, LDSD, S, EXT>), dim3(unsigned(groups)), dim3(256), 0, s, tab);
     return hip_check(hipGetLastError(), "fl_unpack_kernel launch");
 }
diff --git a/vortex_amd/csrc/fsst.hip b/vortex_amd/csrc/fsst.hip
--- a/vortex_amd/csrc/fsst.hip
+++ b/vortex_amd/csrc/fsst.hip
@@ -1027,7 +1027,7 @@
 }
 
 vxg_status launch_fsst_batch(std::vector<FsstChunk>& chunks, void* scratch, uint32_t* err, hipStream_t s,
-                             DevTables* dt, FsstFused* fuse) {
+                             Tables* dt, FsstFused* fuse) {
     if (fuse) fuse->valid = false;
     for (const FsstChunk& c : chunks) {
         if (c.n_symbols > 255) return set_error(VXG_ERR_INVALID_ARGUMENT, "FSST symbol table > 255 entries");
@@ -1047,6 +1047,15 @@
         size_t j = i, live = 0;
         while (j < chunks.size() && (dt || j - i < size_t(kFsstArgChunks)) && fsst_key(chunks[j]) == fsst_key(chunks[i]))
             live += chunks[j++].n != 0;
+        if (live > size_t(kFsstArgChunks) && !fuse) {
+            uint64_t t = 0;
+            for (size_t k = i; k < j; k++) t += (chunks[k].n + kTS - 1) / kTS;
+            if (!dt->reserve(live * sizeof(FsstChunk) + t * sizeof(uint32_t))) {
+                j = i + size_t(kFsstArgChunks);
+                live = 0;
+                for (size_t k = i; k < j; k++) live += chunks[k].n != 0;
+            }
+        }
         const bool fusing = fuse && dt && !fuse->valid && live &&
                             fused_acc(std::get<0>(fsst_key(chunks[i])), std::get<1>(fsst_key(chunks[i])));
         uint64_t group_tiles = 0;
@@ -1109,6 +1118,10 @@
             int64_t* bt = tiles_all + tiles;
             int64_t* tc = bt + scans;
             tiles_all += 2 * tiles + scans;
+            if (tab.ext) {
+                const vxg_status st = commit_call_tables(s);
+                if (st != VXG_OK) return st;
+            }
             if (std::get<2>(key) >= 0)
                 launch_tile_scan_fl32(std::get<2>(key), dim3(unsigned(scans)), s, tab, tp, bt, tc,
                                       std::make_integer_sequence<int, 33>{});
diff --git a/vortex_amd/csrc/k1g.hip b/vortex_amd/csrc/k1g.hip
--- a/vortex_amd/csrc/k1g.hip
+++ b/vortex_amd/csrc/k1g.hip
@@ -100,6 +100,8 @@
     const uint32_t dict_off = (packed_bytes + 128 + 15) & ~15u;
     const size_t shm = std::max<size_t>({size_t(dict_off) + dict_bytes, size_t(runs_bytes), 16});
     if (fuse && fuse->valid) return launch_fsst_k1g(*fuse, ext, n, groups, dict_off, dict_lds, shm, err, s, gpe);
+    const vxg_status cs = commit_call_tables(s);
+    if (cs != VXG_OK) return cs;
     hipLaunchKernelGGL(k1_generic_kernel, dim3(unsigned(groups)), dim3(kGenThreads), shm, s, ext, n, dict_off, dict_lds,
                        err, gpe);
     return hip_check(hipGetLastError(), "k1_generic_kernel launch");
diff --git a/vortex_amd/csrc/kernels.hip b/vortex_amd/csrc/kernels.hip
--- a/vortex_amd/csrc/kernels.hip
+++ b/vortex_amd/csrc/kernels.hip
@@ -617,6 +617,10 @@
 
 vxg_status launch_runend_runs(int value_width, const RunEndTable& t, uint64_t groups, hipStream_t s) {
     if (groups == 0) return VXG_OK;
+    if (t.ext) {
+        const vxg_status cs = commit_call_tables(s);
+        if (cs != VXG_OK) return cs;
+    }
     switch (value_width) {
 #define RR_CASE(W)                                                                                                \
     case W:                                                                                                       \
@@ -631,6 +635,10 @@
 
 vxg_status launch_runend_chunks(int value_width, const RunEndTable& t, uint64_t groups, hipStream_t s) {
     if (groups == 0) return VXG_OK;
+    if (t.ext) {
+        const vxg_status cs = commit_call_tables(s);
+        if (cs != VXG_OK) return cs;
+    }
     switch (value_width) {
 #define RE_CASE(W)                                                                                  \
     case W:                                                                                         \
@@ -815,6 +823,10 @@
 
 vxg_status launch_varbin_chunks(const VarBinTable& t, uint64_t groups, hipStream_t s) {
     if (groups == 0) return VXG_OK;
+    if (t.ext) {
+        const vxg_status cs = commit_call_tables(s);
+        if (cs != VXG_OK) return cs;
+    }
     hipLaunchKernelGGL(varbin_chunks_kernel, dim3(unsigned(groups)), dim3(kBlock), 0, s, t);
     return hip_check(hipGetLastError(), "varbin_chunks_kernel");
 }
diff --git a/vortex_amd/csrc/vxg_internal.hpp b/vortex_amd/csrc/vxg_internal.hpp
--- a/vortex_amd/csrc/vxg_internal.hpp
+++ b/vortex_amd/csrc/vxg_internal.hpp
@@ -96,18 +96,21 @@
     int64_t k1w_min_groups = 1024;
     int64_t k1w_bpw = 0;
     int64_t k1_wave = -1;
+    int64_t direct_tables = 1;
 };
 struct LaunchStats {
     uint64_t k1w_launches = 0, k1w_last_groups = 0;
     uint32_t k1w_last_bpw = 0, k1w_min_bpw = 0, k1w_max_bpw = 0, k1w_last_bpw_max = 0;
 };
 
+struct CallTables;
 struct Ctx {
     int device = 0;
     uint32_t* err_word = nullptr;
     Options opt;
     std::mutex mu;
     LaunchStats st;
+    CallTables* call_tables = nullptr;
 };
 extern thread_local Ctx* g_cur_ctx;
 Options default_options();
@@ -124,20 +127,36 @@
 vxg_status set_error(vxg_status s, const std::string& msg);
 vxg_status hip_check(hipError_t e, const char* what);
 
-struct DevTables {
+struct Tables {
+    virtual ~Tables() = default;
+    virtual vxg_status alloc(size_t bytes, void** host, const void** dev) = 0;
+    virtual bool reserve(size_t bytes) = 0;
+    template <class E>
+    vxg_status table(size_t n, E** host, const E** dev) {
+        void* h = nullptr;
+        const void* d = nullptr;
+        const vxg_status st = alloc(n * sizeof(E), &h, &d);
+        if (st != VXG_OK) return st;
+        *host = static_cast<E*>(h);
+        *dev = static_cast<const E*>(d);
+        return VXG_OK;
+    }
+};
+
+struct DevTables : Tables {
     std::vector<void*> allocs;
     std::vector<std::pair<void*, std::vector<uint8_t>>> uploads;
-    template <class E>
-    vxg_status table(size_t n, E** host, const E** dev) {
+    vxg_status alloc(size_t bytes, void** host, const void** dev) override {
         void* d = nullptr;
-        const hipError_t e = hipMalloc(&d, n * sizeof(E) + 16);
+        const hipError_t e = hipMalloc(&d, bytes + 16);
         if (e != hipSuccess) return hip_check(e, "hipMalloc (plan chunk table)");
         allocs.push_back(d);
-        uploads.emplace_back(d, std::vector<uint8_t>(n * sizeof(E), 0));
-        *host = reinterpret_cast<E*>(uploads.back().second.data());
-        *dev = static_cast<const E*>(d);
+        uploads.emplace_back(d, std::vector<uint8_t>(bytes, 0));
+        *host = uploads.back().second.data();
+        *dev = d;
         return VXG_OK;
     }
+    bool reserve(size_t) override { return true; }
     vxg_status upload() {
         for (auto& u : uploads) {
             const hipError_t e = hipMemcpy(u.first, u.second.data(), u.second.size(), hipMemcpyHostToDevice);
@@ -147,6 +166,50 @@
         return VXG_OK;
     }
 };
+
+struct CallTables {
+    static constexpr size_t kRegionBytes = size_t(256) << 10;
+    static constexpr size_t kSegmentRegions = 4;
+    static constexpr size_t kMaxBytes = size_t(16) << 20;
+    struct Region {
+        uint8_t* host = nullptr;
+        const uint8_t* host_dev = nullptr;
+        uint8_t* dev = nullptr;
+        size_t cap = 0;
+        hipEvent_t done = nullptr;
+        bool in_call = false;
+        bool pending = false;
+    };
+    std::vector<Region*> regions;
+    std::vector<std::pair<void*, void*>> segments;
+    size_t bytes = 0;
+    Region* acquire(size_t need);
+    void destroy();
+};
+
+class CallTablesCall : public Tables {
+  public:
+    CallTablesCall(Ctx* ctx, hipStream_t s) : ctx_(ctx), s_(s) {}
+    ~CallTablesCall() override;
+    vxg_status alloc(size_t bytes, void** host, const void** dev) override;
+    bool reserve(size_t bytes) override;
+    vxg_status commit(hipStream_t s);
+
+  private:
+    struct Use {
+        CallTables::Region* r;
+        size_t used, committed;
+    };
+    bool usable();
+    bool grow(size_t need);
+    Ctx* ctx_;
+    hipStream_t s_;
+    std::vector<Use> uses_;
+    size_t reserved_ = 0;
+    int state_ = 0;
+};
+extern thread_local CallTablesCall* g_call_tables;
+inline vxg_status commit_call_tables(hipStream_t s) { return g_call_tables ? g_call_tables->commit(s) : VXG_OK; }
 
 template <class E, class Key>
 __device__ __forceinline__ uint32_t ext_chunk_index(const E* __restrict__ ext, uint32_t n, uint64_t g, Key key) {
@@ -400,7 +463,7 @@
 };
 hipError_t fsst_diag_init();
 vxg_status launch_fsst_batch(std::vector<FsstChunk>& chunks, void* scratch, uint32_t* err, hipStream_t s,
-                             DevTables* dt = nullptr, FsstFused* fuse = nullptr);
+                             Tables* dt = nullptr, FsstFused* fuse = nullptr);
 vxg_status launch_varbin_views(const uint8_t* heap, uint64_t heap_len, int offs_width, const void* offsets, uint64_t n,
                                const uint8_t* validity, uint32_t bidx, uint8_t* views, uint32_t* err, hipStream_t s);
 vxg_status launch_views_rebase(const uint8_t* src, uint64_t n, uint32_t add, uint8_t* dst, hipStream_t s);
```

Measured after the change: 4821, median of 3. About the same (+0.2%).
